# fawnliu/TRIS

Measured on AMD Instinct MI355X. Metric: Stage-1 training images/sec @320px bs48 (TRIS clip-RN50, 3 negatives), higher is better.
Workload: dtype f32 storage/accumulate; products h2 = 2 x f16 pieces; 1 GPU; Stage-1 train step, RefCOCOg-shaped synthetic batch: 48 img/GPU 320x320, 20-token query + 3 negative queries per image, clip-RN50 trunk + frozen aux CLIP ViT-B/32, AdamW (BASELINE.json configs[2]/[3]); per_gpu_batch=48, global_batch=48, size=320, query_len=20, negative_samples=3, parallelism=dp1, sync_bn=False

## Files before the change

include/tris_hip.h:

```cpp
#ifndef TRIS_HIP_H
#define TRIS_HIP_H

#ifdef __cplusplus
extern "C" {
#endif

int tris_gemm_f32(const float* A, const float* B, float* C, int M, int N, int K, long lda, long ldb, long ldc,
                  int transA, int transB, int batch, long strideA, long strideB, long strideC, const float* bias,
                  int bias_mode, const float* resid, long ldr, long strideR, int act, float alpha, float* workspace,
                  long workspace_bytes, void* stream);

int tris_gemm_epilogue_next(float* pre_out, const float* dact_x);

int tris_splitk_tickets_next(int* tickets, int count);
long tris_splitk_fused_launches(void);

int tris_set_gemm_mode(int mode);
int tris_set_gemm_mode_thread(int mode);
int tris_set_option(const char* name, const char* value);
int tris_set_conv_direct_thread(int value);

int tris_set_autotune(int on);
int tris_get_autotune(void);
int tris_get_gemm_mode(void);
long tris_direct_launches(int kind);

int tris_conv3x3_fwd_f32(const float* X, const float* Wt, float* Y, int B, int H, int W, int Cin, int Cout, int stride,
                         void* stream);
int tris_conv3x3_dgrad_f32(const float* dY, const float* Wt, float* dX, int B, int H, int W, int Cin, int Cout,
                           void* stream);
int tris_conv3x3_wgrad_f32(const float* X, const float* dY, float* dW, int B, int H, int W, int Cin, int Cout,
                           int stride, float* workspace, long workspace_bytes, void* stream);

int tris_conv3x3_bnin_ok(int B, int H, int W, int Cin, int Cout);
int tris_conv3x3_fwd_bnin_f32(const float* X, const float* mean, const float* invstd, const float* gamma, const float* beta,
                              const float* Wt, float* Y, int B, int H, int W, int Cin, int Cout, double* stat_part,
                              int* stat_rows, void* stream);
int tris_conv3x3_wgrad_bnin_f32(const float* X, const float* mean, const float* invstd, const float* gamma, const float* beta,
                                const float* dY, float* dW, int B, int H, int W, int Cin, int Cout, float* workspace,
                                long workspace_bytes, void* stream);

int tris_gemm_bnstat_f32(const float* A, const float* B, float* C, int M, int N, int K, double* stat_part,
                         int* stat_rows, void* stream);
int tris_conv3x3_fwd_bnstat_f32(const float* X, const float* Wt, float* Y, int B, int H, int W, int Cin, int Cout,
                                int stride, double* stat_part, int* stat_rows, void* stream);
int tris_bn_finalize_f32(const double* part, int rows, long M, int C, float eps, float momentum, float* stats,
                         float* running_mean, float* running_var, void* stream);

long tris_col_workspace_bytes(long M, int C);
int tris_bn_stats_f32(const float* X, long M, int C, float eps, float momentum, float* stats, float* running_mean,
                      float* running_var, float* workspace, void* stream);
int tris_bn_sync_combine_f32(const float* gathered, int world, int C, long count_per_rank, float eps, float momentum,
                             float* stats, float* running_mean, float* running_var, void* stream);
int tris_bn_apply_f32(const float* X, const float* mean, const float* invstd, const float* gamma, const float* beta,
                      const float* resid, float* Y, long M, int C, int relu, void* stream);
int tris_gemm_bnbwd_f32(const float* dY, const float* Wt, float* dZ, int M, int N, int K, const float* resid, long ldr,
                        const float* bn_x, const float* bn_y, const float* mean, const float* invstd, const float* gamma,
                        const float* beta, double* part, int* part_rows, void* stream);
int tris_conv3x3_dgrad_bnbwd_f32(const float* dY, const float* Wt, float* dZ, int B, int H, int W, int Cin, int Cout,
                                 const float* bn_x, const float* mean, const float* invstd, const float* gamma,
                                 const float* beta, double* part, int* part_rows, void* stream);
int tris_part_finalize_f32(const double* part, int rows, int C, float* out0, float* out1, void* stream);

int tris_amax_bits_f32(const float* x, long n, unsigned* out, void* stream);
int tris_amax_segments_f32(const float* base, const long* offs, const long* sizes, int nseg, unsigned* slots, void* stream);
int tris_amax_next(unsigned* out);
int tris_h2_next(const unsigned* amaxA, const unsigned* amaxB, float scaleA, float scaleB);
int tris_bn_mask_next(unsigned char* mask);
int tris_h2_planes_f32(const float* x, float* planes_out, long n, const unsigned* word, void* stream);
int tris_h2_planes_segments_f32(const float* base, const long* offs, const long* sizes, const long* slot_index, int nseg,
                                const unsigned* slots, float* out_base, void* stream);
int tris_h2_planes_t_segments_f32(const float* base, const long* offs, const long* rows, const long* cols, const long* slot_index,
                                  int nseg, const unsigned* slots, float* out_base, void* stream);
int tris_h2_unplanes_f32(const float* planes, float* out, long n, const unsigned* word, void* stream);
int tris_h2_next_planes(const unsigned* amaxA, const unsigned* amaxB, int flags);
int tris_bn_apply_pl_f32(const float* X, const float* mean, const float* invstd, const float* gamma, const float* beta,
                         const float* resid, int resid_kind, const unsigned* resid_word, float* Ypl, const unsigned* out_word, long M,
                         int C, int relu, void* stream);
int tris_bn_bwd_reduce_pl_f32(const float* dY, const float* Ypl, const float* X, const float* mean, const float* invstd, long M, int C,
                              float* sum_dz, float* sum_dzx, float* workspace, float* dz_out, void* stream);
int tris_bn_apply_pool_pl_f32(const float* X, const float* mean, const float* invstd, const float* gamma, const float* beta,
                              float* Ypl, const unsigned* out_word, int B, int H, int W, int C, void* stream);
int tris_avgpool2_fwd_pl_f32(const float* Xpl, float* Ypl, const unsigned* word, int B, int H, int W, int C, void* stream);
int tris_bn_bwd_apply_pl_f32(const float* dY, const float* Ypl, const float* X, const float* mean, const float* invstd,
                             const float* gamma, const float* sum_dz, const float* sum_dzx, float inv_count, float* dXpl,
                             const unsigned* out_word, float* dZ, long M, int C, const float* beta_mask, void* stream);
int tris_bn_bwd_apply_pool_pl_f32(const float* dYp, const float* X, const float* mean, const float* invstd, const float* gamma,
                                  const float* beta, const float* sum_dz, const float* sum_dzx, float inv_count, float* dXpl,
                                  const unsigned* out_word, int B, int H, int W, int C, void* stream);
int tris_bn_out_bound2_f32(const float* gamma, const float* beta, int C, float xhat_max, const unsigned* add_word, unsigned* out,
                           void* stream);
int tris_bn_finalize_bound_f32(const double* part, int rows, long M, int C, float eps, float momentum, float* stats,
                               float* running_mean, float* running_var, const float* gamma, const float* beta, float xhat_max,
                               const unsigned* add_word, unsigned* bound_out, void* stream);
int tris_part_finalize_bound_f32(const double* part, int rows, int C, float* out0, float* out1, const float* gamma, const float* invstd,
                                 float inv_count, float xhat_max, const unsigned* dz_word, unsigned* bound_out, void* stream);
int tris_bn_bwd_bound_f32(const float* gamma, const float* invstd, const float* sum_dz, const float* sum_dzx, int C, float inv_count,
                          float xhat_max, const unsigned* dz_word, unsigned* out, void* stream);
int tris_bn_out_bound_f32(const float* gamma, const float* beta, int C, float xhat_max, unsigned* out, void* stream);
int tris_bn_bwd_reduce_f32(const float* dY, const float* Y, const float* X, const float* mean, const float* invstd,
                           long M, int C, float* sum_dz, float* sum_dzx, float* workspace, const float* gamma_mask,
                           const float* beta_mask, float* dz_out, void* stream);
int tris_bn_bwd_apply_f32(const float* dY, const float* Y, const float* X, const float* mean, const float* invstd,
                          const float* gamma, const float* sum_dz, const float* sum_dzx, float inv_count, float* dX,
                          float* dZ, long M, int C, const float* beta_mask, void* stream);
int tris_colsum_f32(const float* X, long M, int N, long ld, float* out, float* workspace, void* stream);

int tris_instnorm_fwd_f32(const float* X, const float* gamma, const float* beta, float* Y, float* mean, float* invstd,
                          int B, int P, int C, float eps, int relu, void* stream);
int tris_instnorm_bwd_f32(const float* dY, const float* Y, const float* X, const float* gamma, const float* mean,
                          const float* invstd, float* dX, float* dgamma_part , float* dbeta_part ,
                          int B, int P, int C, int relu, void* stream);

int tris_layernorm_fwd_f32(const float* X, const float* gamma, const float* beta, float* Y, float* mean, float* rstd,
                           long rows, int W, float eps, void* stream);
long tris_layernorm_bwd_workspace_bytes(long rows, int W);
int tris_layernorm_bwd_f32(const float* dY, const float* X, const float* gamma, const float* mean, const float* rstd,
                           float* dX, float* dgamma, float* dbeta, long rows, int W, float* workspace, const float* extra , void* stream);

int tris_bn_apply_pool_f32(const float* X, const float* mean, const float* invstd, const float* gamma, const float* beta,
                           float* Yp, int B, int H, int W, int C, void* stream);
int tris_bn_bwd_reduce_pool_f32(const float* dYp, const float* X, const float* mean, const float* invstd, int B, int H, int W,
                                int C, float* sum_dz, float* sum_dzx, float* workspace, const float* gamma, const float* beta,
                                void* stream);
int tris_bn_bwd_apply_pool_f32(const float* dYp, const float* X, const float* mean, const float* invstd, const float* gamma,
                               const float* beta, const float* sum_dz, const float* sum_dzx, float inv_count, float* dX, int B,
                               int H, int W, int C, void* stream);
int tris_avgpool2_fwd_f32(const float* X, float* Y, int B, int H, int W, int C, void* stream);
int tris_avgpool2_bwd_f32(const float* dY, float* dX, int B, int H, int W, int C, void* stream);
#define TRIS_EW_ADD 0
#define TRIS_EW_AXPY 1
#define TRIS_EW_RELU_BWD 2
#define TRIS_EW_QGELU 3
#define TRIS_EW_QGELU_BWD 4
#define TRIS_EW_MUL 5
#define TRIS_EW_SCALE 6
#define TRIS_EW_RELU 7
int tris_elementwise_f32(int op, const float* A, const float* B, float* O, long n, float s, void* stream);
int tris_elementwise_bcast_f32(int op, const float* A, const float* B, float* O, long n, long nb, float s, void* stream);
int tris_scale_exp_fwd_f32(const float* X, const float* ls, float* O, float* e_out, long n, void* stream);
long tris_scale_exp_workspace_bytes(void);
int tris_scale_exp_bwd_f32(const float* dO, const float* O, const float* ls, float* dX, float* dls, float* workspace, long n,
                           void* stream);
int tris_nchw_to_nhwc_f32(const float* X, float* Y, int B, int C, int H, int W, void* stream);

int tris_mha_fwd_f32(const float* qkv, float* out, int N, int L, int W, int heads, int causal, void* stream);
int tris_mha_bwd_f32(const float* qkv, const float* dout, float* dqkv, int N, int L, int W, int heads, int causal,
                     void* stream);
int tris_mha_mfma_fwd_f32(const float* qkv, float* out, float* lse, int N, int L, int W, int heads, int causal,
                          void* stream);
int tris_mha_mfma_bwd_f32(const float* qkv, const float* out, const float* dout, const float* lse, float* delta,
                          float* dqkv, int N, int L, int W, int heads, int causal, void* stream);
int tris_mha_h2_fwd_f32(const float* qkv, float* out, float* lse, const unsigned* amax_qkv, int N, int L, int W, int heads,
                        int causal, void* stream);
int tris_mha_h2_bwd_f32(const float* qkv, const float* out, const float* dout, const float* lse, float* delta, float* dqkv,
                        const unsigned* amax_qkv, const unsigned* amax_dout, int N, int L, int W, int heads, int causal,
                        void* stream);
int tris_text_pack_plan_i64(const long* ids, int N, int L, int* plan, void* stream);
int tris_embed_packed_fwd_f32(const long* ids, const float* tok, const float* pos, const int* plan, float* out, int N, int L, int W,
                              void* stream);
int tris_mha_packed_fwd_f32(const float* qkv, float* out, const int* plan, int N, int Lmax, int W, int heads, int causal, void* stream);
int tris_eot_gather_packed_f32(const float* x, const int* plan, float* out, int N, int W, void* stream);
int tris_rows_limit_thread(const int* limit);
int tris_embed_fwd_f32(const long* ids, const float* tok, const float* pos, float* out, int N, int L, int W,
                       void* stream);
int tris_embed_bwd_f32(const long* ids, const float* dout, float* dtok, float* dpos, int N, int L, int W, void* stream);
int tris_embed_rows_bwd_f32(const long* ids, const float* rows, float* dtok, int R, int W, float scale, void* stream);
int tris_concat_i64(const long* a, long na, const long* b, long nb, long* out, void* stream);
int tris_eot_gather_fwd_f32(const long* ids, const float* x, float* out, int N, int L, int W, void* stream);
int tris_eot_gather_bwd_f32(const long* ids, const float* dout, float* dx, int N, int L, int W, void* stream);

int tris_l2norm_fwd_f32(const float* X, float* Y, float* inv_norm, long rows, int C, void* stream);
int tris_l2norm_bwd_f32(const float* dY, const float* Y, const float* inv_norm, float* dX, long rows, int C,
                        void* stream);
int tris_softmax_fwd_f32(const float* X, float* Y, long rows, int n, float scale, void* stream);
int tris_softmax_bwd_f32(const float* dY, const float* Y, float* dX, long rows, int n, float scale, void* stream);
int tris_xattn_fwd_f32(const float* Qv, const float* Kv, const float* Vv, const float* Qt, const float* Kt,
                       const float* Vt, float* new_vis, float* new_lan, float* probs, int B, int P, int N, int C,
                       void* stream);
#define TRIS_DECLINED (-2)
long tris_xattn_fused_ws_bytes(int B, int N, int C);
long tris_xattn_fused_sync_words(int B);
int tris_xattn_fused_fwd_f32(const float* Qv, const float* Kv, const float* Vv, const float* Qt, const float* Kt,
                             const float* Vt, float* new_vis, float* new_lan, float* probs, int B, int P, int N, int C,
                             float* ws, long ws_bytes, unsigned* sync, void* stream);
long tris_xattn_px_ws_bytes(int B, int N, int C);
long tris_xattn_px_sync_words(int B);
long tris_xattn_px_bwd_ws_bytes(int B, int N, int C);
int tris_xattn_px_bwd_f32(const float* d_vis, const float* d_lan, const float* Vv, const float* Qt, const float* Kt,
                          const float* Vt, const float* probs, float* dQv, float* dKv, float* dVv, float* dS, int B, int P,
                          int N, int C, float* ws, long ws_bytes, unsigned* sync, unsigned* amax_dQv, unsigned* amax_dKv,
                          unsigned* amax_dVv, void* stream);
long tris_xattn_px_last_form(void);
int tris_xattn_amax_next(const unsigned* qv, const unsigned* kv, const unsigned* vv, const unsigned* qt, const unsigned* kt,
                         const unsigned* vt);
long tris_xattn_px_slots(int B, int P, int C, int cus);
int tris_xattn_px_fwd_f32(const float* Qv, const float* Kv, const float* Vv, const float* Qt, const float* Kt,
                          const float* Vt, float* new_vis, float* new_lan, float* probs, int B, int P, int N, int C,
                          float* ws, long ws_bytes, unsigned* sync, void* stream);
int tris_softmax_col_bwd_f32(const float* dY, const float* Y, float* dX, int B, int P, int N, float scale,
                             void* stream);
int tris_cls_head_fwd_f32(const float* score, float* cls_out, float* cls_fg, int B, int P, int N, float focal_p,
                          float focal_c, void* stream);
int tris_cls_head_bwd_f32(const float* score, const float* g_cls_out, float* dscore, int B, int P, int N, float focal_p,
                          float focal_c, void* stream);
int tris_maps_fwd_f32(const float* score, float* relu_map, float* sig_map, int B, int h, int w, int N, int S,
                      void* stream);
int tris_maps_bwd_f32(const float* score, const float* d_relu, const float* d_sig, float* dscore, int B, int h, int w,
                      int N, int S, void* stream);
int tris_resize_bilinear_fwd_f32(const float* X, float* Y, int planes, int Hi, int Wi, int Ho, int Wo,
                                 int align_corners, void* stream);
int tris_resize_bilinear_bwd_f32(const float* dY, float* dX, int planes, int Hi, int Wi, int Ho, int Wo,
                                 int align_corners, void* stream);
int tris_fg_patch_fwd_f32(const float* cam, const float* img, float* patches, int B, int C, int R, int ps,
                          void* stream);
int tris_fg_patch_bwd_f32(const float* dpatches, const float* img, float* dcam, int B, int C, int R, int ps,
                          void* stream);
int tris_vit_assemble_fwd_f32(const float* emb, const float* cls, const float* pos, float* x, int B, int T, int W,
                              void* stream);
int tris_vit_assemble_bwd_f32(const float* dx, float* demb, int B, int T, int W, void* stream);
int tris_stage1_loss_fwd_f32(const float* cls, const float* fi, const float* ft, const float* fneg, int B, int N, int E,
                             int K, float w1, float w4, float w5, float* per_img, float* rowloss, float* losses,
                             void* stream);
int tris_stage1_loss_bwd_f32(const float* cls, const float* fi, const float* ft, const float* fneg, const float* g,
                             float w1, float w4, float w5, int B, int N, int E, int K, float* dcls, float* dfi, void* stream);

int tris_adamw_f32(float* p, const float* g, float* m, float* v, long n, float lr, float beta1, float beta2, float eps,
                   float weight_decay, int step_count, void* stream);
int tris_adamw_dev_f32(float* p, const float* g, float* m, float* v, long n, const float* hyper, float beta1, float beta2,
                       float eps, float weight_decay, void* stream);

int tris_eval_post_f32(const float* relu_map, int S, const unsigned char* target, int oH, int oW, float* cam,
                       long* out_iu, float* workspace , void* stream);

int tris_resample_u8(const unsigned char* in, int Hin, int Win, int C, const int* bounds_h, const int* kk_h, int ksize_h,
                     const int* bounds_v, const int* kk_v, int ksize_v, int Hout, int Wout, unsigned char* tmp,
                     unsigned char* out, void* stream);
int tris_gather2d_u8(const unsigned char* in, int Hin, int Win, int C, const int* yidx, const int* xidx, int Hout,
                     int Wout, unsigned char* out, void* stream);
int tris_mask_sum_nearest_u8(const unsigned char* masks, int K, int Hin, int Win, const int* yidx, const int* xidx,
                             int Hout, int Wout, unsigned char* out, void* stream);
int tris_u8_gather_normalize_f32(const unsigned char* cache, const long* index, int B, long HW, const float* lut,
                                 float* out, int planar, void* stream);
int tris_gather_rows(const void* table, const long* index, long rows, long row_bytes, void* out, void* stream);

#define TRIS_MBOX_MAX_WORLD 16
long tris_mbox_bytes(int cap_floats);
int tris_mbox_alloc(void** ptr, int cap_floats);
int tris_mbox_free(void* ptr);
int tris_mbox_ipc_handle(void* ptr, void* handle64);
int tris_mbox_ipc_open(const void* handle64, void** ptr);
int tris_mbox_ipc_close(void* ptr);
int tris_mbox_exchange_f32(const float* src0, int n0, const float* src1, int n1, float* out, void* const* boxes, int world,
                           int rank, unsigned* seq, int cap_floats, int mode, long spin_limit, int* err, void* stream);
int tris_mbox_bn_combine_f32(const float* local_stats, int C, long count_per_rank, float eps, float momentum, float* stats,
                             float* running_mean, float* running_var, void* const* boxes, int world, int rank, unsigned* seq,
                             int cap_floats, long spin_limit, int* err, void* stream);
int tris_mbox_bn_combine_bound_f32(const float* local_stats, int C, long count_per_rank, float eps, float momentum, float* stats,
                                   float* running_mean, float* running_var, void* const* boxes, int world, int rank, unsigned* seq,
                                   int cap_floats, long spin_limit, int* err, const float* gamma, const float* beta, float xhat_max,
                                   const unsigned* resid_word, unsigned* bound_word, void* stream);
int tris_mbox_bn_bwd_exchange_f32(const float* sum_dz, const float* sum_dzx, int C, float* out, void* const* boxes, int world, int rank,
                                  unsigned* seq, int cap_floats, long spin_limit, int* err, const float* gamma, const float* invstd,
                                  float inv_count, float xhat_max, const unsigned* dz_word, unsigned* bound_word, void* stream);

long tris_seg_workspace_bytes(long M, int C);
int tris_bn_prelu_fwd_f32(const float* X, const float* mean, const float* invstd, const float* gamma, const float* beta,
                          const float* slope, float* Y, long M, int C, void* stream);
int tris_bn_prelu_bwd_reduce_f32(const float* dY, const float* X, const float* mean, const float* invstd, const float* gamma,
                                 const float* beta, const float* slope, long M, int C, float* sum_dz, float* sum_dzx, float* dslope,
                                 double* workspace, void* stream);
int tris_bn_prelu_bwd_apply_f32(const float* dY, const float* X, const float* mean, const float* invstd, const float* gamma,
                                const float* beta, const float* slope, const float* sum_dz, const float* sum_dzx, float inv_count,
                                float* dX, long M, int C, void* stream);
int tris_upsample_nhwc_fwd_f32(const float* X, const float* skip, float* up, float* sum, int B, int Hi, int Wi, int Ho, int Wo,
                               int C, void* stream);
int tris_upsample_nhwc_bwd_f32(const float* d_up, const float* d_sum, float* dX, int B, int Hi, int Wi, int Ho, int Wo, int C,
                               void* stream);
int tris_head1_fwd_f32(const float* X, const float* w, float* Y, long M, int C, void* stream);
int tris_head1_bwd_f32(const float* g, const float* X, const float* w, float* dX, float* dw, long M, int C, double* workspace,
                       void* stream);
long tris_bce4_workspace_bytes(long n);
int tris_bce4_fwd_f32(const float* x1, const float* x2, const float* x3, const float* x4, const void* target, int target_f32, long n,
                      float* losses, double* workspace, void* stream);
int tris_bce4_bwd_f32(const float* x1, const float* x2, const float* x3, const float* x4, const void* target, int target_f32,
                      const float* g, float* d1, float* d2, float* d3, float* d4, long n, void* stream);
int tris_eval_post_signed_f32(const float* map, int S, const unsigned char* target, int oH, int oW, float* cam, long* out_iu,
                              float* workspace, void* stream);

int tris_irn_centroids_f32(const float* dp, int h, int w, int iterations, int* centroids, void* stream);
int tris_irn_weak_mask_f32(const float* dp, int h, int w, float thres, unsigned char* mask, void* stream);
long tris_cc_workspace_bytes(int B, int H, int W);
int tris_cc_label_u8(const unsigned char* img, int B, int H, int W, int* labels, int* counts, int* workspace, void* stream);
int tris_irn_cluster_i32(const int* centroids, const int* dp_label, int n_label, int h, int w, int* inst_map, int* n_inst,
                         int* workspace, void* stream);
int tris_irn_instance_cam_f32(const float* cam, const int* inst_map, int K, int n, float* out, void* stream);
int tris_irn_affinity_f32(const float* edge, int h, int w, const int* dirs, const int* path_off, const int* path_cells, int n_dirs,
                          float beta, float* Wt, float* colsum, void* stream);
int tris_irn_walk_f32(const float* x, const float* edge, const float* Wt, const float* colsum, const int* dirs, int n_dirs, int K,
                      int h, int w, int steps, float* out, float* tmp, void* stream);
int tris_irn_finish_f32(const float* rw, int K, int h, int w, int H, int W, float bg_thres, float* rw_up, int* labels,
                        float* workspace, void* stream);
int tris_irn_label_masks_u8(const int* labels, int K, long n, int base, unsigned char* masks, void* stream);
int tris_irn_fragments_f32(const int* frag_labels, const float* rw_up, const int* offsets, int K, long n, long min_area, int F,
                           float* score, int* area, unsigned char* frag_masks, int* workspace, void* stream);

int tris_irn_stem_f32(const unsigned char* img, const float* lut, const float* Wk, const float* mean, const float* invstd,
// ... 58 lines not shown
```

tris_amd/CLIP/clip/model.py:

```python
from collections import OrderedDict


import numpy as np
import torch
from torch import nn

from ... import ops
from ...config import cfg


class Conv2d(nn.Module):

    def __init__(self, cin, cout, k, stride=1, bias=False):
        super().__init__()
        self.cin, self.cout, self.k, self.stride = cin, cout, k, stride
        w = torch.empty(cout, cin, k, k).contiguous(memory_format=torch.channels_last)
        nn.init.kaiming_uniform_(w, a=5 ** 0.5)
        self.weight = nn.Parameter(w)
        self.bias = nn.Parameter(torch.zeros(cout)) if bias else None

    def forward(self, x, stats=False, grad_box=None, grad_box_out=None):
        if self.k == 1:
            return ops.linear(x, self.weight, self.bias, stats=stats and self.bias is None, grad_box=grad_box,
                              grad_box_out=grad_box_out)
# ... 34 lines not shown
        super().__init__()
        assert k == 2
        self.k = k

    def forward(self, x, grad_box_out=None):
        return ops.avgpool2(x, grad_box_out)


class Bottleneck(nn.Module):
    expansion = 4

    def __init__(self, inplanes, planes, stride=1):
        super().__init__()
        self.conv1 = Conv2d(inplanes, planes, 1)
        self.bn1 = BatchNorm2d(planes)
        self.conv2 = Conv2d(planes, planes, 3)
        self.bn2 = BatchNorm2d(planes)
        self.avgpool = AvgPool2d(stride) if stride > 1 else nn.Identity()
        self.conv3 = Conv2d(planes, planes * self.expansion, 1)
        self.bn3 = BatchNorm2d(planes * self.expansion)
        self.downsample = None
        self.stride = stride
        if stride > 1 or inplanes != planes * Bottleneck.expansion:
            self.downsample = nn.Sequential(OrderedDict([
                ("-1", AvgPool2d(stride) if stride > 1 else nn.Identity()),
                ("0", Conv2d(inplanes, planes * self.expansion, 1)),
                ("1", BatchNorm2d(planes * self.expansion)),
            ]))

    def forward(self, x, link_out=False):
        tr = self.training
        link_out = link_out and cfg.grad_box
        box = ops.GradBox() if (tr and torch.is_grad_enabled() and x.requires_grad
                               and cfg.grad_box) else None
        out = self.conv1(x, stats=tr, grad_box=box)
        pl = tr and ops.planes_on()
        out = self.bn1(out, relu=True, lazy=tr and not pl and ops.conv3x3_bnin_ok(out.shape, self.conv2.cout), bwd_link=True,
                       planes=pl, dx_planes=pl)
        if self.stride > 1:
            out = self.bn2(self.conv2(out, stats=tr), relu=True, pool=True, planes=pl, dx_planes=pl)
        else:
            out = self.bn2(self.conv2(out, stats=tr), relu=True, bwd_link=True, planes=pl, dx_planes=pl)
        out = self.conv3(out, stats=tr)
        if self.downsample is not None:
            if isinstance(self.downsample[0], AvgPool2d):
                idn = self.downsample[1](self.downsample[0](x, grad_box_out=box), stats=tr)
            else:
                idn = self.downsample[1](self.downsample[0](x), stats=tr, grad_box_out=box)
            idn = self.downsample[2](idn, dx_planes=pl)
            return self.bn3(out, resid=idn, relu=True, bwd_link=link_out, planes=pl, dx_planes=pl)
        return self.bn3(out, resid=x, relu=True, grad_box=box, bwd_link=link_out, planes=pl, dx_planes=pl)


class Linear(nn.Module):
    def __init__(self, cin, cout):
        super().__init__()
        self.in_features, self.out_features = cin, cout
        self.weight = nn.Parameter(torch.empty(cout, cin))
        self.bias = nn.Parameter(torch.zeros(cout))
        nn.init.kaiming_uniform_(self.weight, a=5 ** 0.5)

    def forward(self, x, resid=None, act=0, grad_box_res=None):
        return ops.linear(x, self.weight, self.bias, resid, act, grad_box_res=grad_box_res)


class AttentionPool2d(nn.Module):

    def __init__(self, spacial_dim, embed_dim, num_heads, output_dim=None):
        super().__init__()
        self.positional_embedding = nn.Parameter(torch.randn(spacial_dim ** 2 + 1, embed_dim) / embed_dim ** 0.5)
        self.k_proj = Linear(embed_dim, embed_dim)
        self.q_proj = Linear(embed_dim, embed_dim)
        self.v_proj = Linear(embed_dim, embed_dim)
        self.c_proj = Linear(embed_dim, output_dim or embed_dim)
        self.num_heads, self.embed_dim, self.spacial_dim = num_heads, embed_dim, spacial_dim
        for p in self.parameters():
            p._tris_no_grad_path = True

    def forward(self, x):
        raise NotImplementedError("AttentionPool2d output is unused by TRIS Stage-1 and is not part of the MI355X path")


class ModifiedResNet(nn.Module):
    def __init__(self, layers, output_dim, heads, input_resolution=224, width=64):
        super().__init__()
        self.output_dim, self.input_resolution = output_dim, input_resolution
        self.conv1 = Conv2d(3, width // 2, 3, stride=2)
        self.bn1 = BatchNorm2d(width // 2)
        self.conv2 = Conv2d(width // 2, width // 2, 3)
        self.bn2 = BatchNorm2d(width // 2)
        self.conv3 = Conv2d(width // 2, width, 3)
        self.bn3 = BatchNorm2d(width)
        self.avgpool = AvgPool2d(2)
        self._inplanes = width
        self.layer1 = self._make_layer(width, layers[0])
        self.layer2 = self._make_layer(width * 2, layers[1], stride=2)
        self.layer3 = self._make_layer(width * 4, layers[2], stride=2)
        self.layer4 = self._make_layer(width * 8, layers[3], stride=2)
        self.attnpool = AttentionPool2d(input_resolution // 32, width * 32, heads, output_dim)

    def _make_layer(self, planes, blocks, stride=1):
        layers = [Bottleneck(self._inplanes, planes, stride)]
        self._inplanes = planes * Bottleneck.expansion
        for _ in range(1, blocks):
            layers.append(Bottleneck(self._inplanes, planes))
        return nn.Sequential(*layers)

    def forward_cl(self, x, hooks=None, taps=True):
        tr = self.training
        if tr:
            ops.h2_auto_step()
        x = ops.nchw_to_nhwc(x.float())
        pl = tr and ops.planes_on()
        x = self.conv1(x, stats=tr)
        x = self.bn1(x, relu=True, lazy=tr and not pl and ops.conv3x3_bnin_ok(x.shape, self.conv2.cout), bwd_link=True,
                     planes=pl)
        x = self.conv2(ops.cut(x), stats=tr)
        x = self.bn2(x, relu=True, lazy=tr and not pl and ops.conv3x3_bnin_ok(x.shape, self.conv3.cout), bwd_link=True,
                     planes=pl, dx_planes=pl)
        x = ops.cut(x)
        x = self.bn3(self.conv3(x, stats=tr), relu=True, pool=True, planes=pl, dx_planes=pl)
        x = ops.cut(x)
        if hooks and "stem" in hooks:
            hooks["stem"]()
        outs = []
        red = getattr(self, "grad_reducer", None)
        if red is not None:
            x = red.boundary(x, "layer1")
        for name, layer in (("layer2", self.layer1), ("layer3", self.layer2), ("layer4", self.layer3),
                            ("heads", self.layer4)):
            for k, blk in enumerate(layer):
                x = ops.cut(blk(x, link_out=(not taps) or k + 1 < len(layer)))
            if red is not None:
                x = red.boundary(x, name)
            outs.append(x)
            stage = {"layer2": "layer1", "layer3": "layer2", "layer4": "layer3", "heads": "layer4"}.get(name)
            if hooks and stage in hooks:
                hooks[stage]()
        return tuple(outs)

    def forward(self, x):
        outs = [ops.unplanes(o).permute(0, 3, 1, 2) for o in self.forward_cl(x)]
        outs.append(None)
        return tuple(outs)


class LayerNorm(nn.Module):
    def __init__(self, w, eps=1e-5):
        super().__init__()
        self.eps = eps
        self.weight = nn.Parameter(torch.ones(w))
        self.bias = nn.Parameter(torch.zeros(w))

    def forward(self, x, grad_box=None):
        return ops.layer_norm(x, self.weight, self.bias, self.eps, grad_box)


class QuickGELU(nn.Module):
    def forward(self, x):
        return ops.quick_gelu(x)


class MultiheadAttention(nn.Module):

    def __init__(self, d_model, n_head):
        super().__init__()
        self.embed_dim, self.num_heads = d_model, n_head
        self.in_proj_weight = nn.Parameter(torch.empty(3 * d_model, d_model))
        self.in_proj_bias = nn.Parameter(torch.zeros(3 * d_model))
        self.out_proj = Linear(d_model, d_model)
        nn.init.xavier_uniform_(self.in_proj_weight)


class ResidualAttentionBlock(nn.Module):
    def __init__(self, d_model, n_head, attn_mask=None):
        super().__init__()
        self.attn = MultiheadAttention(d_model, n_head)
        self.ln_1 = LayerNorm(d_model)
        self.mlp = nn.Sequential(OrderedDict([
            ("c_fc", Linear(d_model, d_model * 4)),
            ("gelu", QuickGELU()),
            ("c_proj", Linear(d_model * 4, d_model)),
        ]))
        self.ln_2 = LayerNorm(d_model)
        self.causal = attn_mask is not None

    def forward(self, x):
        use_box = torch.is_grad_enabled() and x.requires_grad and cfg.grad_box
        b1 = ops.GradBox() if use_box else None
        b2 = ops.GradBox() if use_box else None
        h = self.ln_1(x, b1)
        qkv = ops.linear(h, self.attn.in_proj_weight, self.attn.in_proj_bias)
        a = ops.mha(qkv, self.attn.num_heads, self.causal)
        x = self.attn.out_proj(a, resid=x, grad_box_res=b1)
        h = self.ln_2(x, b2)
        if torch.is_grad_enabled() and cfg.mlp_fuse:
            f = ops.linear_qgelu(h, self.mlp.c_fc.weight, self.mlp.c_fc.bias)
            return ops.linear(f, self.mlp.c_proj.weight, self.mlp.c_proj.bias, x, 0, grad_box_res=b2, act_link=True)
        if torch.is_grad_enabled():
            return self.mlp.c_proj(self.mlp.gelu(self.mlp.c_fc(h)), resid=x, grad_box_res=b2)
        f = self.mlp.c_fc(h, act=2)
        return self.mlp.c_proj(f, resid=x, grad_box_res=b2)


    def forward_packed(self, x, plan, N, L):
        h = self.ln_1(x)
        qkv = ops.linear(h, self.attn.in_proj_weight, self.attn.in_proj_bias)
        a = ops.mha_packed(qkv, plan, N, L, self.attn.num_heads, self.causal)
        x = self.attn.out_proj(a, resid=x)
        h = self.ln_2(x)
        return self.mlp.c_proj(self.mlp.c_fc(h, act=2), resid=x)

    def forward_token0(self, x):
        h = self.ln_1(x)
        qkv = ops.linear(h, self.attn.in_proj_weight, self.attn.in_proj_bias)
        a = ops.token0(ops.mha(qkv, self.attn.num_heads, self.causal))
        x0 = self.attn.out_proj(a, resid=ops.token0(x))
        h = self.ln_2(x0)
        if torch.is_grad_enabled() and cfg.mlp_fuse:
            f = ops.linear_qgelu(h, self.mlp.c_fc.weight, self.mlp.c_fc.bias)
            return ops.linear(f, self.mlp.c_proj.weight, self.mlp.c_proj.bias, x0, 0, act_link=True)
        if torch.is_grad_enabled():
            return self.mlp.c_proj(self.mlp.gelu(self.mlp.c_fc(h)), resid=x0)
        return self.mlp.c_proj(self.mlp.c_fc(h, act=2), resid=x0)


class Transformer(nn.Module):
    def __init__(self, width, layers, heads, attn_mask=None):
        super().__init__()
        self.width, self.layers = width, layers
        self.resblocks = nn.Sequential(*[ResidualAttentionBlock(width, heads, attn_mask) for _ in range(layers)])

    def forward(self, x):
        for blk in self.resblocks:
            x = ops.cut(blk(x))
        return x

    def forward_token0(self, x):
        blocks = list(self.resblocks)
        for blk in blocks[:-1]:
            x = ops.cut(blk(x))
        return blocks[-1].forward_token0(x)


class VisionTransformer(nn.Module):
    def __init__(self, input_resolution, patch_size, width, layers, heads, output_dim):
        super().__init__()
        self.input_resolution, self.output_dim, self.patch_size = input_resolution, output_dim, patch_size
        self.conv1 = nn.Module()
        self.conv1.weight = nn.Parameter(torch.randn(width, 3, patch_size, patch_size) * 0.02)
        scale = width ** -0.5
        self.class_embedding = nn.Parameter(scale * torch.randn(width))
        self.positional_embedding = nn.Parameter(scale * torch.randn((input_resolution // patch_size) ** 2 + 1, width))
        self.ln_pre = LayerNorm(width)
        self.transformer = Transformer(width, layers, heads)
        for blk in self.transformer.resblocks:
            for w in (blk.attn.in_proj_weight, blk.attn.out_proj.weight, blk.mlp.c_fc.weight, blk.mlp.c_proj.weight):
                w._tris_linear_w = True
        self.ln_post = LayerNorm(width)
        self.proj = nn.Parameter(scale * torch.randn(width, output_dim))
        self.spacial_dim = 7
        self.class_embedding._tris_accumulates = True
        self.positional_embedding._tris_accumulates = True

    def forward_patches(self, patches):
        emb = ops.linear(patches, self.conv1.weight)
        x = ops.vit_assemble(emb, self.class_embedding, self.positional_embedding)
        x = self.ln_pre(x)
        if cfg.vit_token0:
            cls = self.ln_post(self.transformer.forward_token0(x))
        else:
            cls = self.ln_post(ops.token0(self.transformer(x)))
        return ops.matmul(cls, self.proj)

    def forward_spatial(self, x):
        B, C, H, Wd = x.shape
        ps = self.patch_size
        ones = torch.ones(B, 1, H, Wd, device=x.device, dtype=torch.float32)
        emb = ops.linear(ops.fg_patches(ones, x.float(), ps), self.conv1.weight)
        gh, gw = H // ps, Wd // ps
        sd = self.input_resolution // ps
        width = self.positional_embedding.shape[1]
        pos = self.positional_embedding
        if (gh, gw) != (sd, sd):
            grid = pos[1:].reshape(1, sd, sd, width).permute(0, 3, 1, 2)
            grid = ops.resize_bilinear(grid, (gh, gw), False)
            pos = torch.cat([pos[0:1], grid.reshape(width, gh * gw).permute(1, 0)], dim=0)
        x = ops.vit_assemble(emb, self.class_embedding, pos.contiguous())
        x = self.ln_pre(x)
        x = self.transformer(x)
        return x[:, 0, :], x[:, 1:, :].reshape(B, gh, gw, width)

    def forward(self, x):
        B, C, R, _ = x.shape
        ones = torch.ones(B, 1, R, R, device=x.device, dtype=torch.float32)
        return self.forward_patches(ops.fg_patches(ones, x.float(), self.patch_size))


class CLIP(nn.Module):
    def __init__(self, embed_dim, image_resolution, vision_layers, vision_width, vision_patch_size, context_length,
                 txt_length, vocab_size, transformer_width, transformer_heads, transformer_layers):
        super().__init__()
        self.context_length = context_length
        if isinstance(vision_layers, (tuple, list)):
            self.visual = ModifiedResNet(layers=vision_layers, output_dim=embed_dim, heads=vision_width * 32 // 64,
                                         input_resolution=image_resolution, width=vision_width)
        else:
            self.visual = VisionTransformer(input_resolution=image_resolution, patch_size=vision_patch_size,
                                            width=vision_width, layers=vision_layers, heads=vision_width // 64,
                                            output_dim=embed_dim)
        self.txt_length = txt_length
        self.transformer = Transformer(width=transformer_width, layers=transformer_layers, heads=transformer_heads,
                                       attn_mask=True)
        self.vocab_size = vocab_size
        self.token_embedding = nn.Embedding(vocab_size, transformer_width)
        self.positional_embedding = nn.Parameter(torch.empty(self.context_length, transformer_width))
        self.ln_final = LayerNorm(transformer_width)
        self.text_projection = nn.Parameter(torch.empty(transformer_width, embed_dim))
        self.logit_scale = nn.Parameter(torch.ones([]) * np.log(1 / 0.07))
        self.logit_scale._tris_no_grad_path = True
        self.initialize_parameters()

    def initialize_parameters(self):
        nn.init.normal_(self.token_embedding.weight, std=0.02)
        nn.init.normal_(self.positional_embedding, std=0.01)
        if isinstance(self.visual, ModifiedResNet):
            std = self.visual.attnpool.c_proj.in_features ** -0.5
            for m in (self.visual.attnpool.q_proj, self.visual.attnpool.k_proj, self.visual.attnpool.v_proj,
                      self.visual.attnpool.c_proj):
                nn.init.normal_(m.weight, std=std)
            for layer in (self.visual.layer1, self.visual.layer2, self.visual.layer3, self.visual.layer4):
                for name, param in layer.named_parameters():
                    if name.endswith("bn3.weight"):
                        nn.init.zeros_(param)
        proj_std = (self.transformer.width ** -0.5) * ((2 * self.transformer.layers) ** -0.5)
        attn_std = self.transformer.width ** -0.5
        fc_std = (2 * self.transformer.width) ** -0.5
        for block in self.transformer.resblocks:
            nn.init.normal_(block.attn.in_proj_weight, std=attn_std)
            nn.init.normal_(block.attn.out_proj.weight, std=proj_std)
            nn.init.normal_(block.mlp.c_fc.weight, std=fc_std)
            nn.init.normal_(block.mlp.c_proj.weight, std=proj_std)
        nn.init.normal_(self.text_projection, std=self.transformer.width ** -0.5)

    @property
    def dtype(self):
        return self.visual.conv1.weight.dtype

    def encode_image(self, image):
        return self.visual(image)

    def encode_text(self, text):
        ids = text.long()
        if ids.shape[1] > self.txt_length:
            raise ValueError(f"token length {ids.shape[1]} exceeds txt_length {self.txt_length}")
        red = getattr(self, "grad_reducer", None)
        x = ops.embed(ids, self.token_embedding.weight, self.positional_embedding, reducer=red)
        if red is not None:
            x = red.boundary(x, "text")
            from ...parallel import TEXT_BOUNDARIES
            for i, blk in enumerate(self.transformer.resblocks):
                x = blk(x)
                if i in TEXT_BOUNDARIES:
                    x = red.boundary(x, TEXT_BOUNDARIES[i])
        else:
            x = self.transformer(x)
        x = self.ln_final(x)
        hidden = ops.matmul(ops.eot_gather(ids, x), self.text_projection)
        return x, hidden

    def encode_text_hidden(self, text):
        ids = text.long()
        if (not cfg.text_pack or torch.is_grad_enabled() or not ops.text_packable(ids.shape[1]) or ids.shape[1] > self.txt_length
                or not ids.is_cuda):
            return self.encode_text(text)[1]
        ids = ids.contiguous()
        N, L = ids.shape
        plan = ops.text_pack_plan(ids)
        x = ops.embed_packed(ids, self.token_embedding.weight, self.positional_embedding, plan)
        with ops.rows_limit(plan):
            for blk in self.transformer.resblocks:
                x = blk.forward_packed(x, plan, N, L)
            x = self.ln_final(x)
        return ops.matmul(ops.eot_gather_packed(x, plan, N), self.text_projection)

    def forward(self, image, text):
        raise NotImplementedError("CLIP.forward (zero-shot logits) is not on the Stage-1 path")


def convert_weights(model):
    return model


def build_model(state_dict, txt_length=40):
    vit = "visual.proj" in state_dict
    if vit:
        vision_width = state_dict["visual.conv1.weight"].shape[0]
        vision_layers = len([k for k in state_dict if k.startswith("visual.") and k.endswith(".attn.in_proj_weight")])
        vision_patch_size = state_dict["visual.conv1.weight"].shape[-1]
        grid = round((state_dict["visual.positional_embedding"].shape[0] - 1) ** 0.5)
        image_resolution = vision_patch_size * grid
    else:
        counts = [len(set(k.split(".")[2] for k in state_dict if k.startswith(f"visual.layer{b}"))) for b in (1, 2, 3, 4)]
        vision_layers = tuple(counts)
        vision_width = state_dict["visual.layer1.0.conv1.weight"].shape[0]
        out_w = round((state_dict["visual.attnpool.positional_embedding"].shape[0] - 1) ** 0.5)
        vision_patch_size = None
        assert out_w ** 2 + 1 == state_dict["visual.attnpool.positional_embedding"].shape[0]
        image_resolution = out_w * 32
    embed_dim = state_dict["text_projection"].shape[1]
    context_length = state_dict["positional_embedding"].shape[0]
# ... 26 lines not shown
```

tris_amd/config.py:

```python
import contextlib
import os


def _flag(name, default):
    v = os.environ.get(name)
    return default if v is None or v == "" else v != "0"


class _Config:
    def __setattr__(self, name, value):
        if name == "step_graph" and "step_graph" in self.__dict__:
            self.__dict__["step_graph_chosen"] = True
        self.__dict__[name] = value

    def __init__(self):
        e = os.environ.get
        self.step_graph = e("TRIS_STEP_GRAPH", "0")
        self.step_graph_chosen = "TRIS_STEP_GRAPH" in os.environ
        self.hipgraph = _flag("TRIS_HIPGRAPH", True)
        self.text_stream = _flag("TRIS_TEXT_STREAM", True)
        self.wgrad_stream = _flag("TRIS_WGRAD_STREAM", True)
        self.stream_probe = _flag("TRIS_STREAM_PROBE", True)
        self.stream_probe_log = e("TRIS_STREAM_PROBE_LOG") == "1"
        self.text_at = e("TRIS_TEXT_AT", "layer4")
        self.bn_bwd_fuse = _flag("TRIS_BN_BWD_FUSE", True)
        self.bn_pool = _flag("TRIS_BN_POOL", True)
        self.grad_box = _flag("TRIS_GRAD_BOX", True)
        self.mlp_fuse = _flag("TRIS_MLP_FUSE", True)
        self.mha = e("TRIS_MHA", "auto")
        self.mha_h2 = _flag("TRIS_MHA_H2", True)
        self.ddp_seg_opt = _flag("TRIS_DDP_SEG_OPT", True)
        self.ddp_seg_poison = _flag("TRIS_DDP_SEG_POISON", False)
        self.syncbn_bound = _flag("TRIS_SYNCBN_BOUND", True)
        self.xattn_fused = _flag("TRIS_XATTN_FUSED", True)
        self.xattn_px = _flag("TRIS_XATTN_PX", True)
        self.xattn_h2 = _flag("TRIS_XATTN_H2", True)
        self.xattn_bwd_px = _flag("TRIS_XATTN_BWD_PX", True)
        self.hbm_loader = _flag("TRIS_HBM_LOADER", True)
        self.eval_group = max(1, int(e("TRIS_EVAL_GROUP", "16")))
        self.mbox_spin = int(e("TRIS_MBOX_SPIN", "40000000"))
        self.syncbn_comm = e("TRIS_SYNCBN_COMM", "mailbox")
        self.ddp_check = e("TRIS_DDP_CHECK") == "1"
        self.ddp_sparse_embed = _flag("TRIS_DDP_SPARSE_EMBED", True)
        self.random_init = e("TRIS_RANDOM_INIT") == "1"
        self.h2_planes = _flag("TRIS_H2_PLANES", True)
        self.own_stream = _flag("TRIS_OWN_STREAM", True)
        self.fuse_splitk = _flag("TRIS_FUSE_SPLITK_PY", False)
        self.aux_text_early = _flag("TRIS_AUX_TEXT_EARLY", True)
        self.text_pack = _flag("TRIS_TEXT_PACK", True)
        self.bn_bitmask = _flag("TRIS_BN_BITMASK", True)
        self.gemm_convert = int(e("TRIS_GEMM_CONVERT", "0"))
        self.step_graph_rerecord = int(e("TRIS_STEP_GRAPH_RERECORD", "3"))
        self.side_param_grads = _flag("TRIS_SIDE_PARAM_GRADS", True)
        self.vit_token0 = _flag("TRIS_VIT_TOKEN0", True)

    @contextlib.contextmanager
    def override(self, **kw):
        old = {k: getattr(self, k) for k in kw}
        try:
            for k, v in kw.items():
                setattr(self, k, v)
            yield self
        finally:
            for k, v in old.items():
                setattr(self, k, v)

    def key(self):
        return tuple(sorted((k, v) for k, v in self.__dict__.items() if k not in ("step_graph_chosen", "step_graph_rerecord")))


cfg = _Config()
```

tris_amd/csrc/attn_h2.hip:

```cpp
#include "common.h"
#include "tris_hip.h"
#include "x3_split.h"

namespace {

#include "amax.h"

constexpr int HD = 64;
constexpr int RS = 144;
constexpr int PLB = 64 * RS;
constexpr float PS = 8192.f;

typedef float f4v __attribute__((ext_vector_type(4)));
typedef short s16x4 __attribute__((ext_vector_type(4)));
typedef short s16x8 __attribute__((ext_vector_type(8)));
typedef unsigned u32x4v __attribute__((ext_vector_type(4)));

struct H8 { f16x8 hi, lo; };

__device__ __forceinline__ float4 ldg4(const float* p) { return *reinterpret_cast<const float4*>(p); }
__device__ __forceinline__ H8 split8(const float4 u, const float4 w, const float s) {
  const Split4 p = split4h(u, s), q = split4h(w, s);
  H8 o;
  o.hi = __builtin_bit_cast(f16x8, (u32x4v){p.hi.x, p.hi.y, q.hi.x, q.hi.y});
  o.lo = __builtin_bit_cast(f16x8, (u32x4v){p.mid.x, p.mid.y, q.mid.x, q.mid.y});
  return o;
}
__device__ __forceinline__ void mm3(const H8& a, const H8& b, f4v& c, f4v& cx) {
  cx = __builtin_amdgcn_mfma_f32_16x16x32_f16(a.lo, b.hi, cx, 0, 0, 0);
  cx = __builtin_amdgcn_mfma_f32_16x16x32_f16(a.hi, b.lo, cx, 0, 0, 0);
  c = __builtin_amdgcn_mfma_f32_16x16x32_f16(a.hi, b.hi, c, 0, 0, 0);
}
__device__ __forceinline__ f4v join(const f4v c, const f4v cx) { return c + cx * (1.0f / 2048.0f); }

__device__ __forceinline__ void stage64(char* planes, const float* base, long row_stride, int row0, int L, int tid, float s) {
#pragma unroll
  for (int q = 0; q < 4; ++q) {
    const int idx = q * 256 + tid, row = idx >> 4, c4 = (idx & 15) * 4;
    const Split4 sp = split4h(ldg4(base + (long)min(row0 + row, L - 1) * row_stride + c4), s);
    *reinterpret_cast<uint2*>(planes + row * RS + c4 * 2) = sp.hi;
    *reinterpret_cast<uint2*>(planes + PLB + row * RS + c4 * 2) = sp.mid;
  }
}
__device__ __forceinline__ H8 afrag(const char* planes, int row, int ks, int kg) {
  H8 o;
  o.hi = *reinterpret_cast<const f16x8*>(planes + row * RS + (32 * ks + 8 * kg) * 2);
  o.lo = *reinterpret_cast<const f16x8*>(planes + PLB + row * RS + (32 * ks + 8 * kg) * 2);
  return o;
}
__device__ __forceinline__ f16x8 trf1(const char* plane, int rb, int ct, int r16, int kg) {
  typedef __attribute__((address_space(3))) s16x4 lds_s16x4;
  const char* a = plane + (rb + kg * 8 + (r16 >> 2)) * RS + ct * 32 + 8 * (r16 & 3);
  const s16x4 lo = __builtin_amdgcn_ds_read_tr16_b64_v4i16((lds_s16x4*)a);
  const s16x4 hi = __builtin_amdgcn_ds_read_tr16_b64_v4i16((lds_s16x4*)(a + 4 * RS));
  const s16x8 v = {lo[0], lo[1], lo[2], lo[3], hi[0], hi[1], hi[2], hi[3]};
  return __builtin_bit_cast(f16x8, v);
}
__device__ __forceinline__ H8 bfrag(const char* planes, int rb, int ct, int r16, int kg) {
  H8 o;
  o.hi = trf1(planes, rb, ct, r16, kg);
  o.lo = trf1(planes + PLB, rb, ct, r16, kg);
  return o;
}
__device__ __forceinline__ void resident(H8 (&f)[2], const float* row_kg, float s) {
#pragma unroll
  for (int ks = 0; ks < 2; ++ks) f[ks] = split8(ldg4(row_kg + 32 * ks), ldg4(row_kg + 32 * ks + 4), s);
}
__device__ __forceinline__ int trow(int r, int j) { return 8 * (r >> 2) + 4 * j + (r & 3); }
__device__ __forceinline__ float wave_scale_of(float m) {
  unsigned u = __builtin_bit_cast(unsigned, m);
#pragma unroll
  for (int sft = 32; sft > 0; sft >>= 1) u = max(u, (unsigned)__shfl_xor((int)u, sft, 64));
  return h2_scale_from_bits(u);
}

__global__ __launch_bounds__(256) void mha_h2_fwd_kernel(const float* __restrict__ qkv, float* __restrict__ out, float* __restrict__ lse,
                                                         int L, int W, int causal, float scale, const unsigned* __restrict__ am_qkv,
                                                         unsigned* __restrict__ amax) {
  __shared__ __attribute__((aligned(16))) char Kp[2 * PLB];
  __shared__ __attribute__((aligned(16))) char Vp[2 * PLB];
  const int tid = threadIdx.x, lane = tid & 63, wave = tid >> 6, r = lane & 15, kg = lane >> 4;
  const int h = blockIdx.y, n = blockIdx.z, H = gridDim.y;
  const int qb = blockIdx.x * 64, q0 = qb + wave * 16;
  const float s = h2_scale_from_bits(h2_amax_of(am_qkv, lane));
  const float inv_s = scale / (s * s), inv_o = 1.0f / (PS * s);
  const float* base = qkv + (long)n * L * 3 * W + h * HD;
  const int qrow = min(q0 + r, L - 1);
  H8 qf[2];
  resident(qf, base + (long)qrow * 3 * W + 8 * kg, s);
  float m = -INFINITY, l = 0.f;
  f4v oc[4], ox[4];
#pragma unroll
  for (int j = 0; j < 4; ++j) oc[j] = ox[j] = (f4v){0.f, 0.f, 0.f, 0.f};
  const int kend = causal ? min(L, qb + 64) : L;
  for (int kb = 0; kb < kend; kb += 64) {
    __syncthreads();
    stage64(Kp, base + W, 3L * W, kb, L, tid, s);
    stage64(Vp, base + 2 * W, 3L * W, kb, L, tid, s);
    __syncthreads();
    if (q0 < L) {
#pragma unroll
      for (int pr = 0; pr < 2; ++pr) {
        const int key0 = kb + 32 * pr;
        if (key0 < kend && !(causal && key0 > q0 + 15)) {
          f4v sc[2], sx[2];
#pragma unroll
          for (int j = 0; j < 2; ++j) {
            sc[j] = sx[j] = (f4v){0.f, 0.f, 0.f, 0.f};
            const int row = 32 * pr + trow(r, j);
#pragma unroll
            for (int ks = 0; ks < 2; ++ks) mm3(afrag(Kp, row, ks, kg), qf[ks], sc[j], sx[j]);
          }
          float sv[8], mx = -INFINITY;
          const bool full = key0 + 32 <= L && !(causal && key0 + 31 > q0);
#pragma unroll
          for (int i = 0; i < 8; ++i) {
            const int key = key0 + 8 * kg + i;
            const float v = (sc[i >> 2][i & 3] + sx[i >> 2][i & 3] * (1.0f / 2048.0f)) * inv_s;
            sv[i] = (full || (key < L && !(causal && key > q0 + r))) ? v : -INFINITY;
            mx = fmaxf(mx, sv[i]);
          }
          mx = fmaxf(mx, __shfl_xor(mx, 16, 64));
          mx = fmaxf(mx, __shfl_xor(mx, 32, 64));
          const float mn = fmaxf(m, mx);
          float p[8], rs = 0.f;
#pragma unroll
          for (int i = 0; i < 8; ++i) { p[i] = mn == -INFINITY ? 0.f : __expf(sv[i] - mn); rs += p[i]; }
          rs += __shfl_xor(rs, 16, 64);
          rs += __shfl_xor(rs, 32, 64);
          const float alpha = mn == -INFINITY ? 1.f : __expf(m - mn);
          l = l * alpha + rs;
          m = mn;
          if (__builtin_amdgcn_ballot_w64(alpha != 1.f) != 0ull) {
#pragma unroll
            for (int t = 0; t < 4; ++t) {
              const float ar = __shfl(alpha, 4 * kg + t, 64);
#pragma unroll
              for (int j = 0; j < 4; ++j) { oc[j][t] *= ar; ox[j][t] *= ar; }
            }
          }
          const H8 pf = split8(make_float4(p[0], p[1], p[2], p[3]), make_float4(p[4], p[5], p[6], p[7]), PS);
#pragma unroll
          for (int ct = 0; ct < 4; ++ct) mm3(pf, bfrag(Vp, 32 * pr, ct, r, kg), oc[ct], ox[ct]);
        }
      }
    }
  }
  unsigned am = 0u;
  if (q0 < L) {
    const float linv = 1.f / l;
    float* ob = out + (long)n * L * W + h * HD;
#pragma unroll
    for (int t = 0; t < 4; ++t) {
      const float li = __shfl(linv, 4 * kg + t, 64) * inv_o;
      const int q = q0 + 4 * kg + t;
      if (q < L) {
#pragma unroll
        for (int j = 0; j < 4; ++j) {
          const float o = (oc[j][t] + ox[j][t] * (1.0f / 2048.0f)) * li;
          ob[(long)q * W + 16 * j + r] = o;
          am = max(am, __builtin_bit_cast(unsigned, o) & 0x7fffffffu);
        }
      }
    }
    if (kg == 0 && q0 + r < L) lse[((long)n * H + h) * L + q0 + r] = m + __logf(l);
  }
  if (amax != nullptr) amax_commit(am, amax);
}

__global__ __launch_bounds__(256) void mha_h2_dq_kernel(const float* __restrict__ qkv, const float* __restrict__ out,
                                                        const float* __restrict__ dout, const float* __restrict__ lse,
                                                        float* __restrict__ delta, float* __restrict__ dqkv, int L, int W, int causal,
                                                        float scale, const unsigned* __restrict__ am_qkv,
                                                        const unsigned* __restrict__ am_do, unsigned* __restrict__ amax) {
  __shared__ __attribute__((aligned(16))) char Kp[2 * PLB];
  __shared__ __attribute__((aligned(16))) char Vp[2 * PLB];
  const int tid = threadIdx.x, lane = tid & 63, wave = tid >> 6, r = lane & 15, kg = lane >> 4;
  const int h = blockIdx.y, n = blockIdx.z, H = gridDim.y;
  const int qb = blockIdx.x * 64, q0 = qb + wave * 16;
  const float s = h2_scale_from_bits(h2_amax_of(am_qkv, lane)), sg = h2_scale_from_bits(h2_amax_of(am_do, lane));
  const float inv_s = scale / (s * s), inv_p = 1.0f / (s * sg);
  const float* base = qkv + (long)n * L * 3 * W + h * HD;
  const int qrow = min(q0 + r, L - 1);
  H8 qf[2], gf[2];
  resident(qf, base + (long)qrow * 3 * W + 8 * kg, s);
  float dl = 0.f;
  {
    const float* gp = dout + ((long)n * L + qrow) * W + h * HD + 8 * kg;
    const float* op = out + ((long)n * L + qrow) * W + h * HD + 8 * kg;
#pragma unroll
    for (int ks = 0; ks < 2; ++ks) {
      const float4 g0 = ldg4(gp + 32 * ks), g1 = ldg4(gp + 32 * ks + 4), o0 = ldg4(op + 32 * ks), o1 = ldg4(op + 32 * ks + 4);
      gf[ks] = split8(g0, g1, sg);
      dl += g0.x * o0.x + g0.y * o0.y + g0.z * o0.z + g0.w * o0.w + g1.x * o1.x + g1.y * o1.y + g1.z * o1.z + g1.w * o1.w;
    }
    dl += __shfl_xor(dl, 16, 64);
    dl += __shfl_xor(dl, 32, 64);
    if (kg == 0 && q0 + r < L) delta[((long)n * H + h) * L + q0 + r] = dl;
  }
  const float ls = lse[((long)n * H + h) * L + qrow];
  f4v acc[4];
#pragma unroll
  for (int j = 0; j < 4; ++j) acc[j] = (f4v){0.f, 0.f, 0.f, 0.f};
  const int kend = causal ? min(L, qb + 64) : L;
  for (int kb = 0; kb < kend; kb += 64) {
    __syncthreads();
    stage64(Kp, base + W, 3L * W, kb, L, tid, s);
    stage64(Vp, base + 2 * W, 3L * W, kb, L, tid, s);
    __syncthreads();
    if (q0 < L) {
#pragma unroll
      for (int pr = 0; pr < 2; ++pr) {
        const int key0 = kb + 32 * pr;
        if (key0 < kend && !(causal && key0 > q0 + 15)) {
          f4v sc[2], sx[2], pc[2], px[2];
#pragma unroll
          for (int j = 0; j < 2; ++j) {
            sc[j] = sx[j] = pc[j] = px[j] = (f4v){0.f, 0.f, 0.f, 0.f};
            const int row = 32 * pr + trow(r, j);
#pragma unroll
            for (int ks = 0; ks < 2; ++ks) {
              mm3(afrag(Kp, row, ks, kg), qf[ks], sc[j], sx[j]);
              mm3(afrag(Vp, row, ks, kg), gf[ks], pc[j], px[j]);
            }
          }
          float ds[8], mx = 0.f;
          const bool full = key0 + 32 <= L && !(causal && key0 + 31 > q0);
#pragma unroll
          for (int i = 0; i < 8; ++i) {
            const int key = key0 + 8 * kg + i;
            const bool ok = full || (key < L && !(causal && key > q0 + r));
            const float sv = (sc[i >> 2][i & 3] + sx[i >> 2][i & 3] * (1.0f / 2048.0f)) * inv_s;
            const float dp = (pc[i >> 2][i & 3] + px[i >> 2][i & 3] * (1.0f / 2048.0f)) * inv_p;
            ds[i] = ok ? __expf(sv - ls) * (dp - dl) * scale : 0.f;
            mx = fmaxf(mx, fabsf(ds[i]));
          }
          const float sd = wave_scale_of(mx);
          const H8 df = split8(make_float4(ds[0], ds[1], ds[2], ds[3]), make_float4(ds[4], ds[5], ds[6], ds[7]), sd);
          const float inv_d = 1.0f / (sd * s);
#pragma unroll
          for (int ct = 0; ct < 4; ++ct) {
            f4v tc = {0.f, 0.f, 0.f, 0.f}, tx = {0.f, 0.f, 0.f, 0.f};
            mm3(df, bfrag(Kp, 32 * pr, ct, r, kg), tc, tx);
            acc[ct] += join(tc, tx) * inv_d;
          }
        }
      }
    }
  }
  unsigned am = 0u;
  if (q0 < L) {
    float* ob = dqkv + (long)n * L * 3 * W + h * HD;
#pragma unroll
    for (int t = 0; t < 4; ++t) {
      const int q = q0 + 4 * kg + t;
      if (q < L) {
#pragma unroll
        for (int j = 0; j < 4; ++j) {
          ob[(long)q * 3 * W + 16 * j + r] = acc[j][t];
          am = max(am, __builtin_bit_cast(unsigned, acc[j][t]) & 0x7fffffffu);
        }
      }
    }
  }
  if (amax != nullptr) amax_commit(am, amax);
}

__global__ __launch_bounds__(256) void mha_h2_dkv_kernel(const float* __restrict__ qkv, const float* __restrict__ dout,
                                                         const float* __restrict__ lse, const float* __restrict__ delta,
                                                         float* __restrict__ dqkv, int L, int W, int causal, float scale,
                                                         const unsigned* __restrict__ am_qkv, const unsigned* __restrict__ am_do,
                                                         unsigned* __restrict__ amax) {
  __shared__ __attribute__((aligned(16))) char Qp[2 * PLB];
  __shared__ __attribute__((aligned(16))) char Gp[2 * PLB];
  __shared__ float Ls[64], Ds[64];
  const int tid = threadIdx.x, lane = tid & 63, wave = tid >> 6, r = lane & 15, kg = lane >> 4;
  const int h = blockIdx.y, n = blockIdx.z, H = gridDim.y;
  const int kb0 = blockIdx.x * 64, k0 = kb0 + wave * 16;
  const float s = h2_scale_from_bits(h2_amax_of(am_qkv, lane)), sg = h2_scale_from_bits(h2_amax_of(am_do, lane));
  const float inv_s = scale / (s * s), inv_p = 1.0f / (s * sg), inv_v = 1.0f / (PS * sg);
  const float* base = qkv + (long)n * L * 3 * W + h * HD;
  const int krow = min(k0 + r, L - 1);
  H8 kf[2], vf[2];
  resident(kf, base + W + (long)krow * 3 * W + 8 * kg, s);
  resident(vf, base + 2 * W + (long)krow * 3 * W + 8 * kg, s);
  f4v dk[4], vc[4], vx[4];
#pragma unroll
  for (int j = 0; j < 4; ++j) dk[j] = vc[j] = vx[j] = (f4v){0.f, 0.f, 0.f, 0.f};
  const int qstart = causal ? kb0 : 0;
  for (int qb = qstart; qb < L; qb += 64) {
    __syncthreads();
    stage64(Qp, base, 3L * W, qb, L, tid, s);
    stage64(Gp, dout + (long)n * L * W + h * HD, (long)W, qb, L, tid, sg);
    if (tid < 64) {
      const int q = min(qb + tid, L - 1);
      Ls[tid] = lse[((long)n * H + h) * L + q];
      Ds[tid] = delta[((long)n * H + h) * L + q];
    }
    __syncthreads();
    if (k0 < L) {
#pragma unroll
      for (int pr = 0; pr < 2; ++pr) {
        const int qs0 = qb + 32 * pr;
        if (qs0 < L && !(causal && qs0 + 31 < k0)) {
          f4v sc[2], sx[2], pc[2], px[2];
#pragma unroll
          for (int j = 0; j < 2; ++j) {
            sc[j] = sx[j] = pc[j] = px[j] = (f4v){0.f, 0.f, 0.f, 0.f};
            const int row = 32 * pr + trow(r, j);
#pragma unroll
            for (int ks = 0; ks < 2; ++ks) {
              mm3(afrag(Qp, row, ks, kg), kf[ks], sc[j], sx[j]);
              mm3(afrag(Gp, row, ks, kg), vf[ks], pc[j], px[j]);
            }
          }
          float p[8], ds[8], mx = 0.f;
          const bool full = qs0 + 32 <= L && !(causal && k0 + 15 > qs0);
#pragma unroll
          for (int i = 0; i < 8; ++i) {
            const int ql = 32 * pr + 8 * kg + i, q = qb + ql;
            const bool ok = full || (q < L && !(causal && k0 + r > q));
            const float sv = (sc[i >> 2][i & 3] + sx[i >> 2][i & 3] * (1.0f / 2048.0f)) * inv_s;
            const float dp = (pc[i >> 2][i & 3] + px[i >> 2][i & 3] * (1.0f / 2048.0f)) * inv_p;
            p[i] = ok ? __expf(sv - Ls[ql]) : 0.f;
            ds[i] = p[i] * (dp - Ds[ql]) * scale;
            mx = fmaxf(mx, fabsf(ds[i]));
          }
          const float sd = wave_scale_of(mx);
          const H8 pf = split8(make_float4(p[0], p[1], p[2], p[3]), make_float4(p[4], p[5], p[6], p[7]), PS);
          const H8 df = split8(make_float4(ds[0], ds[1], ds[2], ds[3]), make_float4(ds[4], ds[5], ds[6], ds[7]), sd);
          const float inv_d = 1.0f / (sd * s);
#pragma unroll
          for (int ct = 0; ct < 4; ++ct) {
            mm3(pf, bfrag(Gp, 32 * pr, ct, r, kg), vc[ct], vx[ct]);
            f4v tc = {0.f, 0.f, 0.f, 0.f}, tx = {0.f, 0.f, 0.f, 0.f};
            mm3(df, bfrag(Qp, 32 * pr, ct, r, kg), tc, tx);
            dk[ct] += join(tc, tx) * inv_d;
          }
        }
      }
    }
  }
  unsigned am = 0u;
  if (k0 < L) {
    float* ob = dqkv + (long)n * L * 3 * W + h * HD;
#pragma unroll
    for (int t = 0; t < 4; ++t) {
      const int k = k0 + 4 * kg + t;
      if (k < L) {
#pragma unroll
        for (int j = 0; j < 4; ++j) {
          const float dv = (vc[j][t] + vx[j][t] * (1.0f / 2048.0f)) * inv_v;
          ob[(long)k * 3 * W + W + 16 * j + r] = dk[j][t];
          ob[(long)k * 3 * W + 2 * W + 16 * j + r] = dv;
          am = max(am, max(__builtin_bit_cast(unsigned, dk[j][t]) & 0x7fffffffu, __builtin_bit_cast(unsigned, dv) & 0x7fffffffu));
        }
      }
    }
  }
  if (amax != nullptr) amax_commit(am, amax);
}

}

extern "C" __attribute__((visibility("hidden"))) unsigned* tris_internal_take_amax_next();

extern "C" int tris_mha_h2_fwd_f32(const float* qkv, float* out, float* lse, const unsigned* amax_qkv, int N, int L, int W, int heads,
                                   int causal, void* stream) {
  if (W != heads * HD || L < 1 || N < 1 || (((uintptr_t)qkv) & 15) || amax_qkv == nullptr) return (int)hipErrorInvalidValue;
  hipLaunchKernelGGL(mha_h2_fwd_kernel, dim3(cdiv(L, 64), heads, N), dim3(256), 0, (hipStream_t)stream, qkv, out, lse, L, W, causal,
                     1.0f / sqrtf((float)HD), amax_qkv, tris_internal_take_amax_next());
  TRIS_LAUNCH_CHECK();
  return 0;
}

extern "C" int tris_mha_h2_bwd_f32(const float* qkv, const float* out, const float* dout, const float* lse, float* delta, float* dqkv,
                                   const unsigned* amax_qkv, const unsigned* amax_dout, int N, int L, int W, int heads, int causal,
                                   void* stream) {
  if (W != heads * HD || L < 1 || N < 1 || amax_qkv == nullptr || amax_dout == nullptr || (((uintptr_t)qkv) & 15) ||
      (((uintptr_t)dout) & 15) || (((uintptr_t)out) & 15))
    return (int)hipErrorInvalidValue;
  const float scale = 1.0f / sqrtf((float)HD);
  const dim3 grid(cdiv(L, 64), heads, N);
  unsigned* amax = tris_internal_take_amax_next();
  hipLaunchKernelGGL(mha_h2_dq_kernel, grid, dim3(256), 0, (hipStream_t)stream, qkv, out, dout, lse, delta, dqkv, L, W, causal, scale,
                     amax_qkv, amax_dout, amax);
  TRIS_LAUNCH_CHECK();
  hipLaunchKernelGGL(mha_h2_dkv_kernel, grid, dim3(256), 0, (hipStream_t)stream, qkv, dout, lse, delta, dqkv, L, W, causal, scale,
                     amax_qkv, amax_dout, amax);
  TRIS_LAUNCH_CHECK();
  return 0;
}
```

tris_amd/csrc/gemm_core.h:

```cpp
#pragma once
#include <algorithm>
#include <cstdlib>
#include <cstring>

#include "common.h"
#include "tris_hip.h"

namespace {

#include "gemm_params.h"
#include "amax.h"

constexpr int BK = 16;
constexpr int PAD = 4;

template <int BM, int BN, int AK, int BKIND, int EPI>
__global__ __launch_bounds__(256) void gemm_kernel(GemmParams p) {
  constexpr int WM = BM / 2, WN = BN / 2;
  constexpr int FM = WM / 32, FN = WN / 32;
  constexpr int PA = BM / 64, PB = BN / 64;
  __shared__ float As[BK][BM + PAD];
  __shared__ float Bs[BK][BN + PAD];

  const int tid = threadIdx.x;
// ... 267 lines not shown
        __syncthreads();
      }
    }
  }

  const int li = lane & 31, kh = lane >> 5;
  unsigned g_am = 0u;
#pragma unroll
  for (int i = 0; i < FM; ++i)
#pragma unroll
    for (int j = 0; j < FN; ++j) {
      const int col = n0 + wn * WN + j * 32 + li;
#pragma unroll
      for (int r = 0; r < 16; ++r) {
        const int row = m0 + wm * WM + i * 32 + (r & 3) + 8 * (r >> 2) + 4 * kh;
        if (row < p.M && col < p.N) {
          float v = acc[i][j][r];
          if (EPI == EPI_SLAB) {
            p.C[((long)blockIdx.z * p.M + row) * p.N + col] = v;
          } else {
            v *= p.alpha;
            if (p.bias_mode == 1) v += p.bias[col];
            else if (p.bias_mode == 2) v += p.bias[row];
            if (p.act == 1) v = fmaxf(v, 0.f);
            else if (p.act == 2) v = v / (1.0f + expf(-1.702f * v));
            if (p.resid) v += p.resid[(long)zb * p.sR + (long)row * p.ldr + col];
            p.C[(long)zb * p.sC + (long)row * p.ldc + col] = v;
            g_am = max(g_am, __builtin_bit_cast(unsigned, v) & 0x7fffffffu);
          }
        }
      }
    }
  if (EPI != EPI_SLAB && p.amax_out != nullptr) amax_commit(g_am, p.amax_out);
}

template <int VEC>
__global__ __launch_bounds__(256) void splitk_reduce_kernel(const float* __restrict__ ws, int S, GemmParams p) {
  const long total = (long)p.M * p.N;
  const long stride = (long)gridDim.x * blockDim.x * VEC;
  unsigned am = 0u;
  for (long idx = ((long)blockIdx.x * blockDim.x + threadIdx.x) * VEC; idx < total; idx += stride) {
    if (p.m_limit != nullptr && idx / p.N >= (long)*p.m_limit) break;
    float v[VEC];
#pragma unroll
    for (int t = 0; t < VEC; ++t) v[t] = 0.f;
    if (VEC == 4) {
      int s = 0;
      for (; s + 3 < S; s += 4) {
        const float4 a = ld4(ws + (long)s * total + idx), b = ld4(ws + (long)(s + 1) * total + idx);
        const float4 c = ld4(ws + (long)(s + 2) * total + idx), d = ld4(ws + (long)(s + 3) * total + idx);
        v[0] = (((v[0] + a.x) + b.x) + c.x) + d.x;
        v[1] = (((v[1] + a.y) + b.y) + c.y) + d.y;
        v[2] = (((v[2] + a.z) + b.z) + c.z) + d.z;
        v[3] = (((v[3] + a.w) + b.w) + c.w) + d.w;
      }
      for (; s < S; ++s) {
        const float4 a = ld4(ws + (long)s * total + idx);
        v[0] += a.x; v[1] += a.y; v[2] += a.z; v[3] += a.w;
      }
    } else {
      for (int s = 0; s < S; ++s) v[0] += ws[(long)s * total + idx];
    }
    const int row = (int)(idx / p.N), col0 = (int)(idx - (long)row * p.N);
#pragma unroll
    for (int t = 0; t < VEC; ++t) {
      const int col = col0 + t;
      float x = v[t] * p.alpha;
      if (p.bias_mode == 1) x += p.bias[col];
      else if (p.bias_mode == 2) x += p.bias[row];
      if (p.act == 1) x = fmaxf(x, 0.f);
      else if (p.act == 2) x = x / (1.0f + expf(-1.702f * x));
      if (p.resid) x += p.resid[(long)row * p.ldr + col];
      v[t] = x;
    }
    if (VEC == 4 && (p.ldc & 3) == 0)
      *reinterpret_cast<float4*>(p.C + (long)row * p.ldc + col0) = make_float4(v[0], v[1], v[2], v[3]);
    else
#pragma unroll
      for (int t = 0; t < VEC; ++t) p.C[(long)row * p.ldc + col0 + t] = v[t];
#pragma unroll
    for (int t = 0; t < VEC; ++t) am = max(am, __builtin_bit_cast(unsigned, v[t]) & 0x7fffffffu);
  }
  if (p.amax_out != nullptr) amax_commit(am, p.amax_out);
}

extern "C" { extern __attribute__((visibility("hidden"))) int tris_internal_red_grid; }
extern "C" { extern __attribute__((visibility("hidden"))) int tris_internal_reduce_wide; }
extern "C" { extern __attribute__((visibility("hidden"))) int tris_internal_xcd_order; }
extern "C" { extern __attribute__((visibility("hidden"))) int tris_internal_fuse_splitk; }
extern "C" { extern __attribute__((visibility("hidden"))) long tris_internal_fused_count; }
template <int G>
__global__ __launch_bounds__(64 * G) void splitk_reduce_wide_kernel(const float* __restrict__ ws, int S, GemmParams p) {
  __shared__ float4 part[G][64];
  const int c = threadIdx.x & 63, g = threadIdx.x >> 6;
  const long total = (long)p.M * p.N;
  const long idx = ((long)blockIdx.x * 64 + c) * 4;
  const bool in = idx < total && !(p.m_limit != nullptr && idx / p.N >= (long)*p.m_limit);
  float4 a = make_float4(0.f, 0.f, 0.f, 0.f);
  if (in) {
    int s = g;
    for (; s + 3 * G < S; s += 4 * G) {
      const float4 x0 = ld4(ws + (long)s * total + idx), x1 = ld4(ws + (long)(s + G) * total + idx);
      const float4 x2 = ld4(ws + (long)(s + 2 * G) * total + idx), x3 = ld4(ws + (long)(s + 3 * G) * total + idx);
      a.x = (((a.x + x0.x) + x1.x) + x2.x) + x3.x; a.y = (((a.y + x0.y) + x1.y) + x2.y) + x3.y;
      a.z = (((a.z + x0.z) + x1.z) + x2.z) + x3.z; a.w = (((a.w + x0.w) + x1.w) + x2.w) + x3.w;
    }
    for (; s < S; s += G) {
      const float4 x0 = ld4(ws + (long)s * total + idx);
      a.x += x0.x; a.y += x0.y; a.z += x0.z; a.w += x0.w;
    }
  }
  part[g][c] = a;
  __syncthreads();
  if (g != 0) return;
  float v[4] = {part[0][c].x, part[0][c].y, part[0][c].z, part[0][c].w};
#pragma unroll
  for (int w = 1; w < G; ++w) { v[0] += part[w][c].x; v[1] += part[w][c].y; v[2] += part[w][c].z; v[3] += part[w][c].w; }
  unsigned am = 0u;
  if (in) {
    const int row = (int)(idx / p.N), col0 = (int)(idx - (long)row * p.N);
#pragma unroll
    for (int t = 0; t < 4; ++t) {
      const int col = col0 + t;
      float x = v[t] * p.alpha;
      if (p.bias_mode == 1) x += p.bias[col];
      else if (p.bias_mode == 2) x += p.bias[row];
      if (p.act == 1) x = fmaxf(x, 0.f);
      else if (p.act == 2) x = x / (1.0f + expf(-1.702f * x));
      if (p.resid) x += p.resid[(long)row * p.ldr + col];
      v[t] = x;
      am = max(am, __builtin_bit_cast(unsigned, x) & 0x7fffffffu);
    }
    if ((p.ldc & 3) == 0)
      *reinterpret_cast<float4*>(p.C + (long)row * p.ldc + col0) = make_float4(v[0], v[1], v[2], v[3]);
    else
#pragma unroll
      for (int t = 0; t < 4; ++t) p.C[(long)row * p.ldc + col0 + t] = v[t];
  }
  if (p.amax_out != nullptr) amax_commit(am, p.amax_out);
}

#include "gemm_fast.h"

static inline long red_blocks(long want) { return tris_internal_red_grid > 0 && want > tris_internal_red_grid ? tris_internal_red_grid : want; }

template <int AK, int BKIND>
int run_cfg(GemmParams p, int batch, float* ws, hipStream_t st, Cfg cfg, int mode) {
  int bm = cfg.bm, bn = cfg.bn, splitk = ws != nullptr ? cfg.splitk : 1;
  const bool fast = gemm_fast_ok(p);
  if (bn == 32 && !fast) bm = bn = 64;
  const bool xtra = p.pre_out != nullptr || p.dact_x != nullptr;
  if (mode == 4 && !fast) return (int)hipErrorInvalidValue;
  const bool pipe = cfg.pipe == 1 && (mode == 1 || mode == 3 || mode == 4) && fast && bn != 32 && !xtra;
  const bool glds = cfg.pipe >= 2 && mode == 4 && fast && !xtra && bn != 32 && AK == A_ROWK && BKIND == B_NK;
  const int gform = glds ? (cfg.pipe >= 4 ? cfg.pipe - 2 : cfg.pipe) : 0;
  if (bm == 256 && !pipe && !glds) bm = 128;
  int tiles_m = cdiv(p.M, bm), tiles_n = cdiv(p.N, bn);
  p.tiles_n = tiles_n;
  const int kalign = fast ? 32 : BK;
  p.splitk = splitk;
  p.kchunk = cdiv(cdiv(p.K, splitk), kalign) * kalign;
  if (splitk > 1) splitk = cdiv(p.K, p.kchunk), p.splitk = splitk;
  dim3 grid((unsigned)(tiles_m * tiles_n), 1, (unsigned)(batch * splitk));
  p.xcd_remap = (fast && BKIND == B_KN_IM2COL && batch == 1 && splitk >= 8 && splitk % 8 == 0 && tiles_m * tiles_n > 1) ? 1 : 0;
  if (glds && cfg.pipe >= 4) p.xcd_remap = 2;
  if (tris_internal_xcd_order >= 0 && fast && p.xcd_remap != 1 && !(tris_internal_xcd_order == 2 && mode == 4))
    p.xcd_remap = (tris_internal_xcd_order && tiles_m * tiles_n >= 16 && tiles_n > 1) ? 2 : 0;
  float* Cfinal = p.C;
  int* const tk = p.tickets;
  p.tickets = nullptr;
  const bool wide = (p.N & 3) == 0 && al16(ws) && al16(Cfinal) && splitk >= 8 && (long)p.M * p.N / 4 < 128 * 256 && tris_internal_reduce_wide;
  const bool vec_fin = (p.N % 4 == 0) && al16(Cfinal) && (p.ldc % 4 == 0) && (!p.resid || (al16(p.resid) && p.ldr % 4 == 0)) &&
                       (p.bias_mode != 1 || al16(p.bias));
  const bool fuse = splitk > 1 && splitk <= tris_internal_fuse_splitk && splitk <= TRIS_FUSE_SPLITK_MAX && tk != nullptr && fast &&
                    batch == 1 && tiles_m * tiles_n <= p.tickets_n && (!wide || vec_fin);
  p.fin_groups = 0;
  if (fuse) {
    __atomic_fetch_add(&tris_internal_fused_count, 1L, __ATOMIC_RELAXED);
    p.tickets = tk;
    p.Cfin = Cfinal;
    p.vecCfin = vec_fin;
    if (wide) p.fin_groups = tris_internal_reduce_wide >= 16 ? 16 : tris_internal_reduce_wide >= 8 ? 8 : 4;
  }
  if (splitk > 1)
    p.vecC = (p.N % 4 == 0) && al16(ws);
  else
    p.vecC = (p.N % 4 == 0) && al16(p.C) && (p.ldc % 4 == 0) && (p.sC % 4 == 0) &&
             (!p.resid || (al16(p.resid) && p.ldr % 4 == 0 && p.sR % 4 == 0)) && (p.bias_mode != 1 || al16(p.bias));
#define TRIS_NW(BM_, BN_, PREC_) ((BM_) == 128 && (BN_) == 128 && (PREC_) != 0 ? 8 : (BN_) == 32 ? 2 : 4)
#define TRIS_FAST(BM_, BN_, EPI_, PREC_)                                                                       \
  hipLaunchKernelGGL((gemm_fast_kernel<BM_, BN_, AK, BKIND, EPI_, PREC_, TRIS_NW(BM_, BN_, PREC_)>), grid,    \
                     dim3(64 * TRIS_NW(BM_, BN_, PREC_)), 0, st, p)
#define TRIS_FAST_EPI(BM_, BN_, EPI_)                                       \
  do {                                                                      \
    if (mode == 1) TRIS_FAST(BM_, BN_, EPI_, 1);                            \
    else if (mode == 3) TRIS_FAST(BM_, BN_, EPI_, 3);                       \
    else if (mode == 4) TRIS_FAST(BM_, BN_, EPI_, 4);                       \
    else TRIS_FAST(BM_, BN_, EPI_, 0);                                      \
  } while (0)
#define TRIS_GO(BM_, BN_, GENERIC_OK_)                                                             \
  do {                                                                                             \
    if (fast) {                                                                                    \
      if (splitk > 1) {                                                                            \
        p.C = ws;                                                                                  \
        TRIS_FAST_EPI(BM_, BN_, EPI_SLAB);                                                         \
      } else if (xtra) {                                                                           \
        if constexpr (AK == A_ROWK && (BKIND == B_NK || BKIND == B_KN)) TRIS_FAST_EPI(BM_, BN_, EPI_XTRA); \
        else return (int)hipErrorInvalidValue;                                                     \
      } else {                                                                                     \
        TRIS_FAST_EPI(BM_, BN_, EPI_STD);                                                          \
      }                                                                                            \
    } else if (GENERIC_OK_) {                                                                      \
      if (splitk > 1) {                                                                            \
        p.C = ws;                                                                                  \
        hipLaunchKernelGGL((gemm_kernel<(GENERIC_OK_ ? BM_ : 64), (GENERIC_OK_ ? BN_ : 64), AK, BKIND, EPI_SLAB>), grid, dim3(256), 0, st, p); \
      } else {                                                                                     \
        hipLaunchKernelGGL((gemm_kernel<(GENERIC_OK_ ? BM_ : 64), (GENERIC_OK_ ? BN_ : 64), AK, BKIND, EPI_STD>), grid, dim3(256), 0, st, p);  \
      }                                                                                            \
    }                                                                                              \
  } while (0)
#define TRIS_PIPE_ONE(BM_, BN_, NW_, NWM_, EPI_)                                                                                   \
  do {                                                                                                                             \
    if (mode == 3)                                                                                                                 \
      hipLaunchKernelGGL((gemm_fast_kernel<BM_, BN_, AK, BKIND, EPI_, 3, NW_, 16, 2, NWM_>), grid, dim3(NW_ * 64), 0, st, p);      \
    else if (mode == 4)                                                                                                            \
      hipLaunchKernelGGL((gemm_fast_kernel<BM_, BN_, AK, BKIND, EPI_, 4, NW_, 16, 2, NWM_>), grid, dim3(NW_ * 64), 0, st, p);      \
    else                                                                                                                           \
      hipLaunchKernelGGL((gemm_fast_kernel<BM_, BN_, AK, BKIND, EPI_, 1, NW_, 16, 2, NWM_>), grid, dim3(NW_ * 64), 0, st, p);      \
  } while (0)
#define TRIS_PIPE_GO(BM_, BN_, NW_, NWM_)                        \
  do {                                                           \
    if (splitk > 1) {                                            \
      p.C = ws;                                                  \
      TRIS_PIPE_ONE(BM_, BN_, NW_, NWM_, EPI_SLAB);              \
    } else {                                                     \
      TRIS_PIPE_ONE(BM_, BN_, NW_, NWM_, EPI_STD);               \
    }                                                            \
  } while (0)
#define TRIS_GLDS_GO(BM_, BN_, NW_, NWM_)                                                                                          \
  do {                                                                                                                           \
    if (splitk > 1) {                                                                                                            \
      p.C = ws;                                                                                                                  \
      hipLaunchKernelGGL((gemm_fast_kernel<BM_, BN_, AK, BKIND, EPI_SLAB, 4, NW_, 32, 4, NWM_>), grid, dim3(NW_ * 64), 0, st, p); \
    } else {                                                                                                                     \
      hipLaunchKernelGGL((gemm_fast_kernel<BM_, BN_, AK, BKIND, EPI_STD, 4, NW_, 32, 4, NWM_>), grid, dim3(NW_ * 64), 0, st, p);  \
    }                                                                                                                            \
  } while (0)
  bool launched = false;
  if constexpr (AK == A_ROWK && BKIND == B_NK) {
    if (glds) {
      launched = true;
      if (bm == 256 && bn == 128) TRIS_GLDS_GO(256, 128, 8, 4);
      else if (bm == 128 && bn == 128 && gform == 3) TRIS_GLDS_GO(128, 128, 4, 2);
      else if (bm == 128 && bn == 128) TRIS_GLDS_GO(128, 128, 8, 2);
      else if (bm == 128 && bn == 64) TRIS_GLDS_GO(128, 64, 4, 2);
      else TRIS_GLDS_GO(64, 64, 4, 2);
    }
  }
#undef TRIS_GLDS_GO
  if (launched) {
  } else
  if (pipe) {
    if (bm == 256 && bn == 128) TRIS_PIPE_GO(256, 128, 8, 4);
    else if (bm == 128 && bn == 128) TRIS_PIPE_GO(128, 128, 8, 2);
    else if (bm == 128 && bn == 64) TRIS_PIPE_GO(128, 64, 4, 2);
    else TRIS_PIPE_GO(64, 64, 4, 2);
  } else if (bm == 128 && bn == 128) TRIS_GO(128, 128, true);
  else if (bm == 128 && bn == 64) TRIS_GO(128, 64, true);
  else if (bm == 128 && bn == 32) TRIS_GO(128, 32, false);
  else TRIS_GO(64, 64, true);
#undef TRIS_GO
#undef TRIS_PIPE_GO
#undef TRIS_PIPE_ONE
#undef TRIS_FAST_EPI
#undef TRIS_FAST
#undef TRIS_NW
  TRIS_LAUNCH_CHECK();
  if (splitk > 1 && !fuse) {
    p.C = Cfinal;
    long total = (long)p.M * p.N;
    if ((p.N & 3) == 0 && al16(ws) && al16(p.C) && splitk >= 8 && total / 4 < 128 * 256 && tris_internal_reduce_wide)
    {
      if (tris_internal_reduce_wide >= 16)
        hipLaunchKernelGGL(splitk_reduce_wide_kernel<16>, dim3(cdiv(total / 4, 64)), dim3(1024), 0, st, ws, splitk, p);
      else if (tris_internal_reduce_wide >= 8)
        hipLaunchKernelGGL(splitk_reduce_wide_kernel<8>, dim3(cdiv(total / 4, 64)), dim3(512), 0, st, ws, splitk, p);
      else
        hipLaunchKernelGGL(splitk_reduce_wide_kernel<4>, dim3(cdiv(total / 4, 64)), dim3(256), 0, st, ws, splitk, p);
    }
    else if ((p.N & 3) == 0 && al16(ws) && al16(p.C))
      hipLaunchKernelGGL(splitk_reduce_kernel<4>, dim3(red_blocks(cdiv(total / 4, 256))), dim3(256), 0, st, ws, splitk, p);
    else
      hipLaunchKernelGGL(splitk_reduce_kernel<1>, dim3(red_blocks(cdiv(total, 256))), dim3(256), 0, st, ws, splitk, p);
    TRIS_LAUNCH_CHECK();
  }
  return 0;
}

}
```

tris_amd/csrc/norm.hip:

```cpp
#include <cstdlib>

#include "common.h"
#include "tris_hip.h"

extern "C" {
__attribute__((visibility("hidden"))) int tris_internal_stream_form = 256;
__attribute__((visibility("hidden"))) int tris_internal_col_blocks = 512;
}

namespace {

#include "amax.h"

__device__ __forceinline__ float4 ld4(const float* p) { return *reinterpret_cast<const float4*>(p); }
__device__ __forceinline__ void st4(float* p, float4 v) { *reinterpret_cast<float4*>(p) = v; }
typedef float f32x4_t __attribute__((ext_vector_type(4)));
__device__ __forceinline__ float4 ld4nt(const float* p) {
  const f32x4_t v = __builtin_nontemporal_load(reinterpret_cast<const f32x4_t*>(p));
  return make_float4(v.x, v.y, v.z, v.w);
}
__device__ __forceinline__ void st4nt(float* p, float4 v) {
  const f32x4_t w = {v.x, v.y, v.z, v.w};
  __builtin_nontemporal_store(w, reinterpret_cast<f32x4_t*>(p));
}
constexpr int BIG_U = 4;
constexpr long BIG_PIECE = 256L * BIG_U;
inline bool big_form(long n4, int C, int streams) { return tris_internal_stream_form && C >= 4 && 1024 % C == 0 && n4 * 16 * streams > ((long)tris_internal_stream_form << 20) && n4 >= 4 * BIG_PIECE; }
inline int big_grid(long n4) { return (int)((n4 + BIG_PIECE - 1) / BIG_PIECE); }

struct d4 { double x, y, z, w; };
__device__ __forceinline__ d4 d4zero() { d4 r; r.x = r.y = r.z = r.w = 0.0; return r; }
__device__ __forceinline__ void st4d(double* p, d4 v) { p[0] = v.x; p[1] = v.y; p[2] = v.z; p[3] = v.w; }

__device__ __forceinline__ long pooled_row(long r, int H, int W) {
  const int w = (int)(r % W);
  const long t = r / W;
  const int h = (int)(t % H);
  const long b = t / H;
  return (b * (H >> 1) + (h >> 1)) * (W >> 1) + (w >> 1);
}

template <int MODE, bool POOL = false>
__global__ __launch_bounds__(256) void col_partial_kernel(const float* __restrict__ X, const float* __restrict__ dY,
                                                          const float* __restrict__ Y, const float* __restrict__ mean,
                                                          const float* __restrict__ invstd, long M, int C, long ld,
                                                          long rows_per_block, double* __restrict__ part,
                                                          const float* __restrict__ gamma = nullptr,
                                                          const float* __restrict__ beta = nullptr,
                                                          float* __restrict__ dZ = nullptr, int pool_h = 0, int pool_w = 0,
                                                          int y_pl = 0, unsigned* __restrict__ amax = nullptr) {
  unsigned am = 0u;
  auto ldy = [&](long o) -> float4 {
    if (!y_pl) return ld4(Y + o);
    const char* yb = reinterpret_cast<const char*>(Y + (o & ~7L)) + (o & 4) * 2;
    const uint2 h = *reinterpret_cast<const uint2*>(yb), l = *reinterpret_cast<const uint2*>(yb + 16);
    const unsigned m0 = (h.x | l.x) & 0x7fff7fffu, m1 = (h.y | l.y) & 0x7fff7fffu;
    return make_float4((m0 & 0xffffu) ? 1.f : 0.f, (m0 >> 16) ? 1.f : 0.f, (m1 & 0xffffu) ? 1.f : 0.f, (m1 >> 16) ? 1.f : 0.f);
  };
  __shared__ d4 l0[256];
  __shared__ d4 l1[256];
  const int CV = C >> 2;
  const int CVB = CV < 256 ? CV : 256;
  const int RS = 256 / CVB;
  const int tid = threadIdx.x;
  const int cvl = tid % CVB, ro = tid / CVB;
  const long rbeg = (long)blockIdx.x * rows_per_block;
  const long rend = min(M, rbeg + rows_per_block);
  for (int cv0 = 0; cv0 < CV; cv0 += CVB) {
    const int c = (cv0 + cvl) * 4;
    d4 s0 = d4zero(), s1 = d4zero();
    float4 mu = make_float4(0, 0, 0, 0), is = mu, sc = mu, be = mu;
    const bool act = (ro < RS) && (cv0 + cvl < CV);
    const bool mask_x = (MODE == 1) && (gamma != nullptr);
    if (act) {
      if (MODE == 1) { mu = ld4(mean + c); is = ld4(invstd + c); }
      if (mask_x) {
        const float4 ga = ld4(gamma + c);
        be = ld4(beta + c);
        sc = make_float4(is.x * ga.x, is.y * ga.y, is.z * ga.z, is.w * ga.w);
      }
      auto accum = [&](const float4 x, float4 g, const float4 y, long o) {
        if (MODE == 0) {
          s0.x += x.x; s0.y += x.y; s0.z += x.z; s0.w += x.w;
          s1.x += (double)x.x * x.x; s1.y += (double)x.y * x.y; s1.z += (double)x.z * x.z; s1.w += (double)x.w * x.w;
        } else if (MODE == 1) {
          if (mask_x) {
            if (!((x.x - mu.x) * sc.x + be.x > 0.f)) g.x = 0.f;
            if (!((x.y - mu.y) * sc.y + be.y > 0.f)) g.y = 0.f;
            if (!((x.z - mu.z) * sc.z + be.z > 0.f)) g.z = 0.f;
            if (!((x.w - mu.w) * sc.w + be.w > 0.f)) g.w = 0.f;
          } else if (Y) {
            if (!(y.x > 0.f)) g.x = 0.f;
            if (!(y.y > 0.f)) g.y = 0.f;
            if (!(y.z > 0.f)) g.z = 0.f;
            if (!(y.w > 0.f)) g.w = 0.f;
          }
          if (dZ) st4(dZ + o, g);
          am = max(am, abits4(g));
          s0.x += g.x; s0.y += g.y; s0.z += g.z; s0.w += g.w;
          s1.x += (double)(g.x * ((x.x - mu.x) * is.x)); s1.y += (double)(g.y * ((x.y - mu.y) * is.y));
          s1.z += (double)(g.z * ((x.z - mu.z) * is.z)); s1.w += (double)(g.w * ((x.w - mu.w) * is.w));
        } else {
          s0.x += x.x; s0.y += x.y; s0.z += x.z; s0.w += x.w;
        }
      };
      const float4 z4 = make_float4(0, 0, 0, 0);
      long r = rbeg + ro;
      for (; r + 3 * RS < rend; r += 4 * RS) {
        float4 x[4], g[4], y[4];
#pragma unroll
        for (int u = 0; u < 4; ++u) {
          const long o = (r + (long)u * RS) * ld + c;
          x[u] = ld4(X + o);
          if (POOL) {
            g[u] = ld4(dY + pooled_row(r + (long)u * RS, pool_h, pool_w) * ld + c);
            g[u].x *= 0.25f; g[u].y *= 0.25f; g[u].z *= 0.25f; g[u].w *= 0.25f;
          } else {
            g[u] = (MODE == 1) ? ld4(dY + o) : z4;
          }
          y[u] = (MODE == 1 && Y) ? ldy(o) : z4;
        }
#pragma unroll
        for (int u = 0; u < 4; ++u) accum(x[u], g[u], y[u], (r + (long)u * RS) * ld + c);
      }
      for (; r < rend; r += RS) {
        const long o = r * ld + c;
        float4 g1 = z4;
        if (POOL) {
          g1 = ld4(dY + pooled_row(r, pool_h, pool_w) * ld + c);
          g1.x *= 0.25f; g1.y *= 0.25f; g1.z *= 0.25f; g1.w *= 0.25f;
        } else if (MODE == 1) {
          g1 = ld4(dY + o);
        }
        accum(ld4(X + o), g1, (MODE == 1 && Y) ? ldy(o) : z4, o);
      }
    }
    __syncthreads();
    l0[tid] = s0;
    l1[tid] = s1;
    __syncthreads();
    if (ro == 0 && cv0 + cvl < CV) {
      for (int q = 1; q < RS; ++q) {
        d4 a = l0[q * CVB + cvl], b = l1[q * CVB + cvl];
        s0.x += a.x; s0.y += a.y; s0.z += a.z; s0.w += a.w;
        s1.x += b.x; s1.y += b.y; s1.z += b.z; s1.w += b.w;
      }
      double* o = part + (long)blockIdx.x * 2 * C;
      st4d(o + c, s0);
      if (MODE != 2) st4d(o + C + c, s1);
    }
  }
  if (MODE == 1 && amax != nullptr) amax_commit(am, amax);
}

constexpr int FIN_CH = 4;
template <typename T>
__device__ __forceinline__ void reduce_parts(const T* __restrict__ part, int nb, int C, bool two, double& s, double& ss,
                                             int& c, bool& lead) {
  __shared__ double sh0[1024];
  __shared__ double sh1[1024];
  const int SL = blockDim.x / FIN_CH;
  const int cl = threadIdx.x % FIN_CH, j = threadIdx.x / FIN_CH;
  c = blockIdx.x * FIN_CH + cl;
  s = 0.0;
  ss = 0.0;
  if (c < C) {
    constexpr int U = 8;
// ... 195 lines not shown
                                                           const float* __restrict__ invstd,
                                                           const float* __restrict__ gamma,
                                                           const float* __restrict__ sum_dz,
                                                           const float* __restrict__ sum_dzx, float inv_cnt,
                                                           float* __restrict__ dX, float* __restrict__ dZ, long n4,
                                                           int C, const float* __restrict__ beta_mask, int pool_h = 0,
                                                           int pool_w = 0, unsigned* __restrict__ amax = nullptr) {
  unsigned am = 0u;
  const long stride = (long)gridDim.x * blockDim.x;
  long i = BIG ? (long)blockIdx.x * BIG_PIECE + threadIdx.x : (long)blockIdx.x * blockDim.x + threadIdx.x;
  const int c = (int)((i * 4) % C);
  const float4 mu = ld4(mean + c), is = ld4(invstd + c), ga = ld4(gamma + c), a = ld4(sum_dz + c), b = ld4(sum_dzx + c);
  const float4 be = beta_mask ? ld4(beta_mask + c) : make_float4(0, 0, 0, 0);
  const float4 k1 = make_float4(ga.x * is.x, ga.y * is.y, ga.z * is.z, ga.w * is.w);
  const float4 k2 = make_float4(a.x * inv_cnt, a.y * inv_cnt, a.z * inv_cnt, a.w * inv_cnt);
  const float4 k3 = make_float4(is.x * b.x * inv_cnt, is.y * b.y * inv_cnt, is.z * b.z * inv_cnt, is.w * b.w * inv_cnt);
  const bool use_y = !beta_mask && Y != nullptr;
  auto load_g = [&](long j) {
    float4 g;
    if (POOL) {
      g = ld4(dY + pooled_row(j * 4 / C, pool_h, pool_w) * C + c);
      g.x *= 0.25f; g.y *= 0.25f; g.z *= 0.25f; g.w *= 0.25f;
    } else {
      g = BIG ? ld4nt(dY + j * 4) : ld4(dY + j * 4);
    }
    return g;
  };
  auto finish = [&](long j, float4 g, const float4 x, const float4 y) {
    if (beta_mask) {
      if (!((x.x - mu.x) * k1.x + be.x > 0.f)) g.x = 0.f;
      if (!((x.y - mu.y) * k1.y + be.y > 0.f)) g.y = 0.f;
      if (!((x.z - mu.z) * k1.z + be.z > 0.f)) g.z = 0.f;
      if (!((x.w - mu.w) * k1.w + be.w > 0.f)) g.w = 0.f;
    } else if (use_y) {
      if (!(y.x > 0.f)) g.x = 0.f;
      if (!(y.y > 0.f)) g.y = 0.f;
      if (!(y.z > 0.f)) g.z = 0.f;
      if (!(y.w > 0.f)) g.w = 0.f;
    }
    if (dZ) { if (BIG) st4nt(dZ + j * 4, g); else st4(dZ + j * 4, g); }
    float4 o;
    o.x = k1.x * (g.x - k2.x - (x.x - mu.x) * k3.x);
    o.y = k1.y * (g.y - k2.y - (x.y - mu.y) * k3.y);
    o.z = k1.z * (g.z - k2.z - (x.z - mu.z) * k3.z);
    o.w = k1.w * (g.w - k2.w - (x.w - mu.w) * k3.w);
    if (BIG) st4nt(dX + j * 4, o); else st4(dX + j * 4, o);
    am = max(am, abits4(o));
  };
  const float4 z4 = make_float4(0, 0, 0, 0);
  if (BIG) {
    float4 g[BIG_U], x[BIG_U], y[BIG_U];
#pragma unroll
    for (int u = 0; u < BIG_U; ++u) {
      const long j = i + u * 256;
      const bool ok = j < n4;
      g[u] = ok ? load_g(j) : z4;
      x[u] = ok ? ld4nt(X + j * 4) : z4;
      y[u] = (ok && use_y) ? ld4nt(Y + j * 4) : z4;
    }
#pragma unroll
    for (int u = 0; u < BIG_U; ++u) {
      const long j = i + u * 256;
      if (j < n4) finish(j, g[u], x[u], y[u]);
    }
  } else {
    auto one = [&](long j) { finish(j, load_g(j), ld4(X + j * 4), use_y ? ld4(Y + j * 4) : z4); };
    for (; i + stride < n4; i += 2 * stride) {
      one(i);
      one(i + stride);
    }
    if (i < n4) one(i);
  }
  if (amax != nullptr) amax_commit_block(am, amax);
}

__global__ __launch_bounds__(256) void instnorm_fwd_kernel(const float* __restrict__ X, const float* __restrict__ gamma,
                                                           const float* __restrict__ beta, float* __restrict__ Y,
                                                           float* __restrict__ mean_out, float* __restrict__ invstd_out,
                                                           int P, int C, float eps, int relu,
                                                           unsigned* __restrict__ amax = nullptr) {
  __shared__ float red[4][64];
  const int b = blockIdx.y, c = blockIdx.x * 64 + (threadIdx.x & 63), pg = threadIdx.x >> 6;
  const bool ok = c < C;
  const float* x = X + (long)b * P * C + c;
  float s = 0.f;
  if (ok) for (int p = pg; p < P; p += 4) s += x[(long)p * C];
  red[pg][threadIdx.x & 63] = s;
  __syncthreads();
  const int cl = threadIdx.x & 63;
  float mean = (red[0][cl] + red[1][cl] + red[2][cl] + red[3][cl]) / (float)P;
  __syncthreads();
  float v = 0.f;
  if (ok) for (int p = pg; p < P; p += 4) { float d = x[(long)p * C] - mean; v += d * d; }
  red[pg][cl] = v;
  __syncthreads();
  float var = (red[0][cl] + red[1][cl] + red[2][cl] + red[3][cl]) / (float)P;
  float is = rsqrtf(var + eps);
  unsigned am = 0u;
  if (ok) {
    float g = gamma[c], be = beta[c];
    float* y = Y + (long)b * P * C + c;
    for (int p = pg; p < P; p += 4) {
      float o = (x[(long)p * C] - mean) * is * g + be;
      if (relu) o = fmaxf(o, 0.f);
      y[(long)p * C] = o;
      am = max(am, __builtin_bit_cast(unsigned, o) & 0x7fffffffu);
    }
    if (pg == 0) { mean_out[(long)b * C + c] = mean; invstd_out[(long)b * C + c] = is; }
  }
  if (amax != nullptr) amax_commit(am, amax);
}

__global__ __launch_bounds__(256) void instnorm_bwd_kernel(const float* __restrict__ dY, const float* __restrict__ Y,
                                                           const float* __restrict__ X, const float* __restrict__ gamma,
                                                           const float* __restrict__ mean_in,
                                                           const float* __restrict__ invstd_in, float* __restrict__ dX,
                                                           float* __restrict__ dgamma_part, float* __restrict__ dbeta_part,
                                                           int P, int C, int relu, unsigned* __restrict__ amax = nullptr) {
  __shared__ float r0[4][64];
  __shared__ float r1[4][64];
  const int b = blockIdx.y, cl = threadIdx.x & 63, c = blockIdx.x * 64 + cl, pg = threadIdx.x >> 6;
  const bool ok = c < C;
  const long base = (long)b * P * C + c;
  float mean = ok ? mean_in[(long)b * C + c] : 0.f, is = ok ? invstd_in[(long)b * C + c] : 0.f;
  float s0 = 0.f, s1 = 0.f;
  if (ok)
    for (int p = pg; p < P; p += 4) {
      float g = dY[base + (long)p * C];
      if (relu && !(Y[base + (long)p * C] > 0.f)) g = 0.f;
      s0 += g;
      s1 += g * (X[base + (long)p * C] - mean) * is;
    }
  r0[pg][cl] = s0;
  r1[pg][cl] = s1;
  __syncthreads();
  s0 = r0[0][cl] + r0[1][cl] + r0[2][cl] + r0[3][cl];
  s1 = r1[0][cl] + r1[1][cl] + r1[2][cl] + r1[3][cl];
  unsigned am = 0u;
  if (ok) {
    float ga = gamma[c], ip = 1.0f / (float)P;
    for (int p = pg; p < P; p += 4) {
      float g = dY[base + (long)p * C];
      if (relu && !(Y[base + (long)p * C] > 0.f)) g = 0.f;
      float xh = (X[base + (long)p * C] - mean) * is;
      const float d = ga * is * (g - s0 * ip - xh * s1 * ip);
      dX[base + (long)p * C] = d;
      am = max(am, __builtin_bit_cast(unsigned, d) & 0x7fffffffu);
    }
    if (pg == 0) { dgamma_part[(long)b * C + c] = s1; dbeta_part[(long)b * C + c] = s0; }
  }
  if (amax != nullptr) amax_commit(am, amax);
}

__global__ __launch_bounds__(256) void layernorm_fwd_kernel(const float* __restrict__ X, const float* __restrict__ gamma,
                                                            const float* __restrict__ beta, float* __restrict__ Y,
                                                            float* __restrict__ mean_out, float* __restrict__ rstd_out,
                                                            long rows, int W, float eps, unsigned* __restrict__ amax = nullptr,
                                                            const int* __restrict__ limit = nullptr) {
  const int lane = threadIdx.x & 63;
  const long row = (long)blockIdx.x * 4 + (threadIdx.x >> 6);
  if (row >= rows) return;
  if (limit != nullptr && row >= (long)*limit) return;
  unsigned am = 0u;
  const int W4 = W >> 2;
  float4 v[4];
  float s = 0.f;
#pragma unroll
  for (int q = 0; q < 4; ++q) {
    int i = lane + q * 64;
    v[q] = make_float4(0, 0, 0, 0);
    if (i < W4) { v[q] = ld4(X + row * W + i * 4); s += v[q].x + v[q].y + v[q].z + v[q].w; }
  }
  float mean = wave_sum(s) / (float)W;
  float s2 = 0.f;
#pragma unroll
  for (int q = 0; q < 4; ++q) {
    int i = lane + q * 64;
    if (i < W4) {
      float a = v[q].x - mean, b = v[q].y - mean, c = v[q].z - mean, d = v[q].w - mean;
      s2 += a * a + b * b + c * c + d * d;
    }
  }
  float rstd = rsqrtf(wave_sum(s2) / (float)W + eps);
#pragma unroll
  for (int q = 0; q < 4; ++q) {
    int i = lane + q * 64;
    if (i < W4) {
      float4 g = ld4(gamma + i * 4), b = ld4(beta + i * 4), o;
      o.x = (v[q].x - mean) * rstd * g.x + b.x;
      o.y = (v[q].y - mean) * rstd * g.y + b.y;
      o.z = (v[q].z - mean) * rstd * g.z + b.z;
      o.w = (v[q].w - mean) * rstd * g.w + b.w;
      st4(Y + row * W + i * 4, o);
      am = max(am, abits4(o));
    }
  }
  if (amax != nullptr) amax_commit(am, amax);
  if (lane == 0 && mean_out) { mean_out[row] = mean; rstd_out[row] = rstd; }
}

__global__ __launch_bounds__(256) void layernorm_bwd_kernel(const float* __restrict__ dY, const float* __restrict__ X,
                                                            const float* __restrict__ gamma,
                                                            const float* __restrict__ mean_in,
                                                            const float* __restrict__ rstd_in, float* __restrict__ dX,
                                                            float* __restrict__ part, long rows, int W,
                                                            long rows_per_block, const float* __restrict__ extra,
                                                            unsigned* __restrict__ amax = nullptr) {
  unsigned am = 0u;
  __shared__ float4 lg[4][256];
  __shared__ float4 lb[4][256];
  const int lane = threadIdx.x & 63, wv = threadIdx.x >> 6;
  const int W4 = W >> 2;
  float4 ag[4], ab[4];
#pragma unroll
  for (int q = 0; q < 4; ++q) ag[q] = ab[q] = make_float4(0, 0, 0, 0);
  const long rbeg = (long)blockIdx.x * rows_per_block, rend = min(rows, rbeg + rows_per_block);
  for (long row = rbeg + wv; row < rend; row += 4) {
    const float mean = mean_in[row], rstd = rstd_in[row];
    float4 xh[4], dh[4];
    float c1 = 0.f, c2 = 0.f;
#pragma unroll
    for (int q = 0; q < 4; ++q) {
      int i = lane + q * 64;
      xh[q] = dh[q] = make_float4(0, 0, 0, 0);
      if (i < W4) {
        float4 x = ld4(X + row * W + i * 4), dy = ld4(dY + row * W + i * 4), g = ld4(gamma + i * 4);
        xh[q] = make_float4((x.x - mean) * rstd, (x.y - mean) * rstd, (x.z - mean) * rstd, (x.w - mean) * rstd);
        dh[q] = make_float4(dy.x * g.x, dy.y * g.y, dy.z * g.z, dy.w * g.w);
        c1 += dh[q].x + dh[q].y + dh[q].z + dh[q].w;
        c2 += dh[q].x * xh[q].x + dh[q].y * xh[q].y + dh[q].z * xh[q].z + dh[q].w * xh[q].w;
        ag[q].x += dy.x * xh[q].x; ag[q].y += dy.y * xh[q].y; ag[q].z += dy.z * xh[q].z; ag[q].w += dy.w * xh[q].w;
        ab[q].x += dy.x; ab[q].y += dy.y; ab[q].z += dy.z; ab[q].w += dy.w;
      }
    }
    c1 = wave_sum(c1) / (float)W;
    c2 = wave_sum(c2) / (float)W;
    if (dX) {
#pragma unroll
      for (int q = 0; q < 4; ++q) {
        int i = lane + q * 64;
        if (i < W4) {
          float4 o;
          o.x = rstd * (dh[q].x - c1 - xh[q].x * c2);
          o.y = rstd * (dh[q].y - c1 - xh[q].y * c2);
          o.z = rstd * (dh[q].z - c1 - xh[q].z * c2);
          o.w = rstd * (dh[q].w - c1 - xh[q].w * c2);
          if (extra) {
            const float4 e = ld4(extra + row * W + i * 4);
            o.x += e.x; o.y += e.y; o.z += e.z; o.w += e.w;
          }
          st4(dX + row * W + i * 4, o);
          am = max(am, abits4(o));
        }
      }
    }
  }
  if (amax != nullptr) amax_commit_block(am, amax);
  if (!part) return;
#pragma unroll
  for (int q = 0; q < 4; ++q) { lg[wv][lane + q * 64] = ag[q]; lb[wv][lane + q * 64] = ab[q]; }
  __syncthreads();
  if (wv == 0) {
    float* o = part + (long)blockIdx.x * 2 * W;
#pragma unroll
    for (int q = 0; q < 4; ++q) {
      int i = lane + q * 64;
      if (i < W4) {
        float4 g = lg[0][i], b = lb[0][i];
        for (int w = 1; w < 4; ++w) {
          float4 g2 = lg[w][i], b2 = lb[w][i];
          g.x += g2.x; g.y += g2.y; g.z += g2.z; g.w += g2.w;
          b.x += b2.x; b.y += b2.y; b.z += b2.z; b.w += b2.w;
        }
        st4(o + i * 4, g);
        st4(o + W + i * 4, b);
      }
    }
  }
}

__global__ void avgpool2_fwd_kernel(const float* __restrict__ X, float* __restrict__ Y, int B, int H, int W, int C) {
  const int Ho = H >> 1, Wo = W >> 1, C4 = C >> 2;
  long n = (long)B * Ho * Wo * C4;
  long i = (long)blockIdx.x * blockDim.x + threadIdx.x;
  const long stride = (long)gridDim.x * blockDim.x;
  for (; i < n; i += stride) {
    int c4 = (int)(i % C4);
    long t = i / C4;
    int ox = (int)(t % Wo);
    t /= Wo;
    int oy = (int)(t % Ho);
    int b = (int)(t / Ho);
    const float* p = X + (((long)b * H + oy * 2) * W + ox * 2) * C + c4 * 4;
    float4 a = ld4(p), b4 = ld4(p + C), c = ld4(p + (long)W * C), d = ld4(p + (long)W * C + C);
    st4(Y + i * 4, make_float4(0.25f * (a.x + b4.x + c.x + d.x), 0.25f * (a.y + b4.y + c.y + d.y),
                               0.25f * (a.z + b4.z + c.z + d.z), 0.25f * (a.w + b4.w + c.w + d.w)));
  }
}

__global__ void avgpool2_bwd_kernel(const float* __restrict__ dY, float* __restrict__ dX, int B, int H, int W, int C) {
  const int Ho = H >> 1, Wo = W >> 1, C4 = C >> 2;
  long n = (long)B * H * W * C4;
  long i = (long)blockIdx.x * blockDim.x + threadIdx.x;
  const long stride = (long)gridDim.x * blockDim.x;
  for (; i < n; i += stride) {
    int c4 = (int)(i % C4);
    long t = i / C4;
    int x = (int)(t % W);
    t /= W;
    int y = (int)(t % H);
    int b = (int)(t / H);
    float4 g = make_float4(0, 0, 0, 0);
    if ((y >> 1) < Ho && (x >> 1) < Wo) {
      g = ld4(dY + (((long)b * Ho + (y >> 1)) * Wo + (x >> 1)) * C + c4 * 4);
      g.x *= 0.25f; g.y *= 0.25f; g.z *= 0.25f; g.w *= 0.25f;
    }
    st4(dX + i * 4, g);
  }
}

__device__ __forceinline__ float ew1(int op, float a, float b, float s) {
  switch (op) {
    case TRIS_EW_ADD: return a + b;
    case TRIS_EW_AXPY: return s * a + b;
    case TRIS_EW_RELU_BWD: return b > 0.f ? a : 0.f;
    case TRIS_EW_QGELU: return a / (1.0f + expf(-1.702f * a));
    case TRIS_EW_QGELU_BWD: {
      float sg = 1.0f / (1.0f + expf(-1.702f * b));
      return a * (sg + 1.702f * b * sg * (1.f - sg));
    }
    case TRIS_EW_MUL: return a * b;
    case TRIS_EW_SCALE: return s * a;
    case TRIS_EW_RELU: return fmaxf(a, 0.f);
    default: return a;
  }
}
__global__ void ew_kernel(int op, const float* __restrict__ A, const float* __restrict__ Bp, float* __restrict__ O,
                          long n, float s, unsigned* __restrict__ amax = nullptr, long nb = 0) {
  long i = (long)blockIdx.x * blockDim.x + threadIdx.x;
  const long stride = (long)gridDim.x * blockDim.x;
  const long n4 = n >> 2;
  unsigned am = 0u;
  for (long j = i; j < n4; j += stride) {
    float4 a = ld4(A + j * 4), b = Bp ? ld4(Bp + (nb > 0 ? (j * 4) % nb : j * 4)) : make_float4(0, 0, 0, 0);
    const float4 o = make_float4(ew1(op, a.x, b.x, s), ew1(op, a.y, b.y, s), ew1(op, a.z, b.z, s), ew1(op, a.w, b.w, s));
    st4(O + j * 4, o);
    am = max(am, abits4(o));
  }
  for (long j = n4 * 4 + i; j < n; j += stride) {
    const float o = ew1(op, A[j], Bp ? Bp[j] : 0.f, s);
// ... 187 lines not shown
  const long M = (long)B * H * W;
  ColPlan p = col_plan(M, C);
  hipLaunchKernelGGL((col_partial_kernel<1, true>), dim3(p.nb), dim3(256), 0, st, X, dYp, (const float*)nullptr, mean, invstd, M, C,
                     (long)C, p.rpb, (double*)workspace, gamma, beta, (float*)nullptr, H, W, 0, take_amax_next());
  TRIS_LAUNCH_CHECK();
  hipLaunchKernelGGL(part_finalize_kernel<double>, dim3(fin_grid(C, p.nb)), dim3(fin_block(p.nb)), 0, st, (const double*)workspace,
                     p.nb, C, sum_dz, sum_dzx);
  TRIS_LAUNCH_CHECK();
  return 0;
}

extern "C" int tris_bn_bwd_apply_pool_f32(const float* dYp, const float* X, const float* mean, const float* invstd,
                                          const float* gamma, const float* beta, const float* sum_dz, const float* sum_dzx,
                                          float inv_count, float* dX, int B, int H, int W, int C, void* stream) {
  if (C % 4 || (H & 1) || (W & 1)) return (int)hipErrorInvalidValue;
  const long n4 = (long)B * H * W * C / 4;
  hipLaunchKernelGGL(bn_bwd_apply_kernel<true>, dim3(bn_grid(n4, C)), dim3(256), 0, (hipStream_t)stream, dYp, (const float*)nullptr, X,
                     mean, invstd, gamma, sum_dz, sum_dzx, inv_count, dX, (float*)nullptr, n4, C, beta, H, W, take_amax_next());
  TRIS_LAUNCH_CHECK();
  return 0;
}

__global__ __launch_bounds__(256) void bn_out_bound_kernel(const float* __restrict__ gamma, const float* __restrict__ beta, int C,
                                                           float xhat_max, unsigned* __restrict__ out) {
  __shared__ float red[4];
  float m = 0.f;
  for (int c = threadIdx.x; c < C; c += 256) m = fmaxf(m, fabsf(gamma[c]) * xhat_max + fabsf(beta[c]));
  m = block_max_256(m, red);
  if (threadIdx.x == 0) out[0] = __builtin_bit_cast(unsigned, m);
}
extern "C" int tris_bn_out_bound_f32(const float* gamma, const float* beta, int C, float xhat_max, unsigned* out, void* stream) {
  if (C <= 0 || out == nullptr) return (int)hipErrorInvalidValue;
  hipLaunchKernelGGL(bn_out_bound_kernel, dim3(1), dim3(256), 0, (hipStream_t)stream, gamma, beta, C, xhat_max, out);
  TRIS_LAUNCH_CHECK();
  return 0;
}

__global__ __launch_bounds__(256) void amax_bits_kernel(const float* __restrict__ x, long n, unsigned* __restrict__ out) {
  const long n4 = n >> 2;
  const long stride = (long)gridDim.x * blockDim.x;
  unsigned m = 0u;
  for (long i = (long)blockIdx.x * blockDim.x + threadIdx.x; i < n4; i += stride) {
    const float4 v = ld4(x + i * 4);
    m = max(max(m, __builtin_bit_cast(unsigned, v.x) & 0x7fffffffu), __builtin_bit_cast(unsigned, v.y) & 0x7fffffffu);
    m = max(max(m, __builtin_bit_cast(unsigned, v.z) & 0x7fffffffu), __builtin_bit_cast(unsigned, v.w) & 0x7fffffffu);
  }
  for (long i = n4 * 4 + (long)blockIdx.x * blockDim.x + threadIdx.x; i < n; i += stride)
    m = max(m, __builtin_bit_cast(unsigned, x[i]) & 0x7fffffffu);
  amax_commit_block(m, out);
}

__global__ __launch_bounds__(256) void amax_segments_kernel(const float* __restrict__ base, const long* __restrict__ offs,
                                                            const long* __restrict__ sizes, unsigned* __restrict__ slots) {
  const long n = sizes[blockIdx.y];
  const float* x = base + offs[blockIdx.y];
  const long n4 = n >> 2;
  const long stride = (long)gridDim.x * blockDim.x;
  unsigned m = 0u;
  for (long i = (long)blockIdx.x * blockDim.x + threadIdx.x; i < n4; i += stride) m = max(m, abits4(ld4(x + i * 4)));
  for (long i = n4 * 4 + (long)blockIdx.x * blockDim.x + threadIdx.x; i < n; i += stride)
    m = max(m, __builtin_bit_cast(unsigned, x[i]) & 0x7fffffffu);
  amax_commit_block(m, slots + (long)blockIdx.y * 2048);
}

extern "C" int tris_amax_segments_f32(const float* base, const long* offs, const long* sizes, int nseg, unsigned* slots,
                                      void* stream) {
  if (nseg < 1 || (((uintptr_t)base) & 15)) return (int)hipErrorInvalidValue;
  hipLaunchKernelGGL(amax_segments_kernel, dim3(128, (unsigned)nseg), dim3(256), 0, (hipStream_t)stream, base, offs, sizes, slots);
  TRIS_LAUNCH_CHECK();
  return 0;
}

extern "C" int tris_amax_bits_f32(const float* x, long n, unsigned* out, void* stream) {
  if (n < 1 || (((uintptr_t)x) & 15)) return (int)hipErrorInvalidValue;
  long g = (n / 4 + 255) / 256;
  g = g > 2048 ? 2048 : (g < 1 ? 1 : g);
  hipLaunchKernelGGL(amax_bits_kernel, dim3((unsigned)g), dim3(256), 0, (hipStream_t)stream, x, n, out);
  TRIS_LAUNCH_CHECK();
  return 0;
}

extern "C" int tris_part_finalize_f32(const double* part, int rows, int C, float* out0, float* out1, void* stream) {
  if (rows < 1 || C < 1) return (int)hipErrorInvalidValue;
  hipLaunchKernelGGL(part_finalize_kernel<double>, dim3(fin_grid(C, rows)), dim3(fin_block(rows)), 0, (hipStream_t)stream, part, rows,
                     C, out0, out1);
  TRIS_LAUNCH_CHECK();
  return 0;
}

extern "C" int tris_part_finalize_bound_f32(const double* part, int rows, int C, float* out0, float* out1, const float* gamma,
                                            const float* invstd, float inv_count, float xhat_max, const unsigned* dz_word,
                                            unsigned* bound_out, void* stream) {
  if (rows < 1 || C < 1 || out1 == nullptr || gamma == nullptr || invstd == nullptr || dz_word == nullptr || bound_out == nullptr)
    return (int)hipErrorInvalidValue;
  hipLaunchKernelGGL(part_finalize_kernel<double>, dim3(fin_grid(C, rows)), dim3(fin_block(rows)), 0, (hipStream_t)stream, part, rows,
                     C, out0, out1, gamma, invstd, inv_count, xhat_max, dz_word, bound_out);
  TRIS_LAUNCH_CHECK();
  return 0;
}

extern "C" int tris_bn_bwd_apply_f32(const float* dY, const float* Y, const float* X, const float* mean,
                                     const float* invstd, const float* gamma, const float* sum_dz, const float* sum_dzx,
                                     float inv_count, float* dX, float* dZ, long M, int C, const float* beta_mask,
                                     void* stream) {
  long n4 = M * C / 4;
  const int streams = 3 + ((Y && !beta_mask) ? 1 : 0) + (dZ ? 1 : 0);
  if (big_form(n4, C, streams))
    hipLaunchKernelGGL((bn_bwd_apply_kernel<false, true>), dim3(big_grid(n4)), dim3(256), 0, (hipStream_t)stream, dY, Y, X, mean,
                       invstd, gamma, sum_dz, sum_dzx, inv_count, dX, dZ, n4, C, beta_mask, 0, 0, take_amax_next());
  else
    hipLaunchKernelGGL((bn_bwd_apply_kernel<false, false>), dim3(bn_grid(n4, C)), dim3(256), 0, (hipStream_t)stream, dY, Y, X, mean,
                       invstd, gamma, sum_dz, sum_dzx, inv_count, dX, dZ, n4, C, beta_mask, 0, 0, take_amax_next());
  TRIS_LAUNCH_CHECK();
  return 0;
}

extern "C" int tris_colsum_f32(const float* X, long M, int N, long ld, float* out, float* workspace, void* stream) {
  hipStream_t st = (hipStream_t)stream;
  if (N % 4 || ld % 4 || (((uintptr_t)X) & 15)) {
    hipLaunchKernelGGL(colsum_scalar_kernel, dim3(cdiv(N, 256)), dim3(256), 0, st, X, M, N, ld, out);
    TRIS_LAUNCH_CHECK();
    return 0;
  }
  ColPlan p = col_plan(M, N);
  hipLaunchKernelGGL(col_partial_kernel<2>, dim3(p.nb), dim3(256), 0, st, X, nullptr, nullptr, nullptr, nullptr, M, N,
                     ld, p.rpb, (double*)workspace);
  TRIS_LAUNCH_CHECK();
  hipLaunchKernelGGL(part_finalize_kernel<double>, dim3(fin_grid(N, p.nb)), dim3(fin_block(p.nb)), 0, st, (const double*)workspace, p.nb, N,
                     out, (float*)nullptr);
  TRIS_LAUNCH_CHECK();
  return 0;
}

extern "C" int tris_instnorm_fwd_f32(const float* X, const float* gamma, const float* beta, float* Y, float* mean,
                                     float* invstd, int B, int P, int C, float eps, int relu, void* stream) {
  hipLaunchKernelGGL(instnorm_fwd_kernel, dim3(cdiv(C, 64), B), dim3(256), 0, (hipStream_t)stream, X, gamma, beta, Y,
                     mean, invstd, P, C, eps, relu, take_amax_next());
  TRIS_LAUNCH_CHECK();
  return 0;
}

extern "C" int tris_instnorm_bwd_f32(const float* dY, const float* Y, const float* X, const float* gamma,
                                     const float* mean, const float* invstd, float* dX, float* dgamma_part,
                                     float* dbeta_part, int B, int P, int C, int relu, void* stream) {
  hipLaunchKernelGGL(instnorm_bwd_kernel, dim3(cdiv(C, 64), B), dim3(256), 0, (hipStream_t)stream, dY, Y, X, gamma,
                     mean, invstd, dX, dgamma_part, dbeta_part, P, C, relu, take_amax_next());
  TRIS_LAUNCH_CHECK();
  return 0;
}

extern "C" int tris_layernorm_fwd_f32(const float* X, const float* gamma, const float* beta, float* Y, float* mean,
                                      float* rstd, long rows, int W, float eps, void* stream) {
  if (W % 4 || W > 1024) return (int)hipErrorInvalidValue;
  hipLaunchKernelGGL(layernorm_fwd_kernel, dim3(cdiv(rows, 4)), dim3(256), 0, (hipStream_t)stream, X, gamma, beta, Y,
                     mean, rstd, rows, W, eps, take_amax_next(), g_rows_limit);
  TRIS_LAUNCH_CHECK();
  return 0;
}

extern "C" { __attribute__((visibility("hidden"))) int tris_internal_ln_bwd_blocks = 512; }
static long ln_bwd_rpb(long rows) {
  const long target = tris_internal_ln_bwd_blocks;
  long rpb = (rows + target - 1) / target;
  const long floor_ = target > 128 ? 4 : 8;
  return rpb < floor_ ? floor_ : rpb;
}
extern "C" long tris_layernorm_bwd_workspace_bytes(long rows, int W) {
  const long rpb = ln_bwd_rpb(rows);
  long nb = (rows + rpb - 1) / rpb;
  if (nb < 512) nb = 512;
  return nb * 2 * W * (long)sizeof(float);
}

extern "C" int tris_layernorm_bwd_f32(const float* dY, const float* X, const float* gamma, const float* mean,
                                      const float* rstd, float* dX, float* dgamma, float* dbeta, long rows, int W,
                                      float* workspace, const float* extra, void* stream) {
  if (W % 4 || W > 1024) return (int)hipErrorInvalidValue;
  hipStream_t st = (hipStream_t)stream;
  const long rpb = ln_bwd_rpb(rows);
  int nb = (int)((rows + rpb - 1) / rpb);
  float* part = dgamma ? workspace : nullptr;
  hipLaunchKernelGGL(layernorm_bwd_kernel, dim3(nb), dim3(256), 0, st, dY, X, gamma, mean, rstd, dX, part, rows, W,
                     rpb, extra, take_amax_next());
  TRIS_LAUNCH_CHECK();
  if (dgamma) {
    hipLaunchKernelGGL(part_finalize_kernel<float>, dim3(fin_grid(W, nb)), dim3(fin_block(nb)), 0, st, (const float*)workspace, nb, W, dgamma, dbeta);
    TRIS_LAUNCH_CHECK();
  }
  return 0;
}

extern "C" int tris_avgpool2_fwd_f32(const float* X, float* Y, int B, int H, int W, int C, void* stream) {
  if (C % 4) return (int)hipErrorInvalidValue;
  long n = (long)B * (H / 2) * (W / 2) * (C / 4);
  hipLaunchKernelGGL(avgpool2_fwd_kernel, dim3(grid_for(n)), dim3(256), 0, (hipStream_t)stream, X, Y, B, H, W, C);
  TRIS_LAUNCH_CHECK();
  return 0;
}

extern "C" int tris_avgpool2_bwd_f32(const float* dY, float* dX, int B, int H, int W, int C, void* stream) {
  if (C % 4) return (int)hipErrorInvalidValue;
  long n = (long)B * H * W * (C / 4);
  hipLaunchKernelGGL(avgpool2_bwd_kernel, dim3(grid_for(n)), dim3(256), 0, (hipStream_t)stream, dY, dX, B, H, W, C);
  TRIS_LAUNCH_CHECK();
  return 0;
}

extern "C" int tris_elementwise_f32(int op, const float* A, const float* B, float* O, long n, float s, void* stream) {
  hipLaunchKernelGGL(ew_kernel, dim3(grid_for((n + 3) / 4)), dim3(256), 0, (hipStream_t)stream, op, A, B, O, n, s,
                     take_amax_next());
  TRIS_LAUNCH_CHECK();
  return 0;
}

extern "C" int tris_elementwise_bcast_f32(int op, const float* A, const float* B, float* O, long n, long nb, float s,
                                          void* stream) {
  if (B == nullptr || nb < 4 || (nb & 3) || (n & 3) || n % nb) return (int)hipErrorInvalidValue;
  hipLaunchKernelGGL(ew_kernel, dim3(grid_for(n / 4)), dim3(256), 0, (hipStream_t)stream, op, A, B, O, n, s, take_amax_next(), nb);
  TRIS_LAUNCH_CHECK();
  return 0;
}

namespace {
__global__ __launch_bounds__(256) void scale_exp_fwd_kernel(const float* __restrict__ X, const float* __restrict__ ls,
                                                            float* __restrict__ O, float* __restrict__ e_out, long n) {
  const float e = expf(ls[0]);
  if (blockIdx.x == 0 && threadIdx.x == 0) e_out[0] = e;
  const long stride = (long)gridDim.x * blockDim.x;
  for (long i = (long)blockIdx.x * blockDim.x + threadIdx.x; i < n; i += stride) O[i] = X[i] * e;
}
__global__ __launch_bounds__(256) void scale_exp_bwd_kernel(const float* __restrict__ dO, const float* __restrict__ O,
                                                            const float* __restrict__ ls, float* __restrict__ dX,
                                                            double* __restrict__ part, long n) {
  __shared__ double red[256];
  const float e = expf(ls[0]);
  const long stride = (long)gridDim.x * blockDim.x;
  float acc = 0.f;
  for (long i = (long)blockIdx.x * blockDim.x + threadIdx.x; i < n; i += stride) {
    const float g = dO[i];
    if (dX) dX[i] = g * e;
    acc += g * O[i];
  }
  red[threadIdx.x] = (double)acc;
  __syncthreads();
  for (int h = 128; h > 0; h >>= 1) {
    if ((int)threadIdx.x < h) red[threadIdx.x] += red[threadIdx.x + h];
    __syncthreads();
  }
  if (threadIdx.x == 0) part[blockIdx.x] = red[0];
}
__global__ void scale_exp_bwd_finish_kernel(const double* __restrict__ part, int nb, float* __restrict__ dls) {
  double s = 0.0;
  for (int i = 0; i < nb; ++i) s += part[i];
  dls[0] = (float)s;
}
constexpr int SE_BLOCKS = 128;
}
extern "C" int tris_scale_exp_fwd_f32(const float* X, const float* ls, float* O, float* e_out, long n, void* stream) {
  hipLaunchKernelGGL(scale_exp_fwd_kernel, dim3(grid_for(n)), dim3(256), 0, (hipStream_t)stream, X, ls, O, e_out, n);
  TRIS_LAUNCH_CHECK();
  return 0;
}
extern "C" long tris_scale_exp_workspace_bytes() { return (long)SE_BLOCKS * sizeof(double); }
extern "C" int tris_scale_exp_bwd_f32(const float* dO, const float* O, const float* ls, float* dX, float* dls,
                                      float* workspace, long n, void* stream) {
  double* part = reinterpret_cast<double*>(workspace);
  hipLaunchKernelGGL(scale_exp_bwd_kernel, dim3(SE_BLOCKS), dim3(256), 0, (hipStream_t)stream, dO, O, ls, dX, part, n);
  TRIS_LAUNCH_CHECK();
  hipLaunchKernelGGL(scale_exp_bwd_finish_kernel, dim3(1), dim3(1), 0, (hipStream_t)stream, part, SE_BLOCKS, dls);
  TRIS_LAUNCH_CHECK();
  return 0;
}

extern "C" int tris_nchw_to_nhwc_f32(const float* X, float* Y, int B, int C, int H, int W, void* stream) {
  long n = (long)B * C * H * W;
  hipLaunchKernelGGL(nchw_to_nhwc_kernel, dim3(grid_for(n)), dim3(256), 0, (hipStream_t)stream, X, Y, B, C,
                     (long)H * W);
  TRIS_LAUNCH_CHECK();
  return 0;
}
```

tris_amd/ops.py:

```python
import math
import os

import torch

from . import _lib
from ._lib import CONSTS, call, query
from .config import cfg

EW = CONSTS


class NoGpuError(RuntimeError):
    pass


_RAW_STREAM = getattr(torch._C, "_cuda_getCurrentRawStream", None)


def _stream():
    if _RAW_STREAM is not None:
        return _RAW_STREAM(torch.cuda.current_device())
    return torch.cuda.current_stream().cuda_stream


# ... 222 lines not shown
            def coll():
                w = dist.all_reduce(buf, group=group, async_op=True)
                w.wait()
            dist.barrier(group=group)
            if not probe(r, issue, coll) and backend_cls is None and k < len(reps):
                backend_cls = k
    if cfg.stream_probe_log:
        print(f"[place_streams] queue classes of the candidates {cls}, collective backend on class {backend_cls}", flush=True)
    free = [k for k in range(len(reps)) if k != backend_cls]
    if len(free) < 3:
        return None
    order = ([cls[0]] if cls[0] in free else []) + [k for k in free if k != cls[0]]
    compute, text, wgrad = reps[order[0]], reps[order[1]], reps[order[2]]
    used = {cls[cands.index(compute)], cls[cands.index(text)], cls[cands.index(wgrad)]}
    issue = next((c for c, k in zip(cands, cls) if k == backend_cls), None)
    if issue is None:
        issue = next((c for c, k in zip(cands, cls) if k not in used), wgrad)
    _CAL[dev] = [text, wgrad, issue]
    _WG.pop(dev, None)
    for key in [k for k in _SIDE_STREAMS if k[0] == dev]:
        _SIDE_STREAMS.pop(key)
    return None if compute is null else compute


def _new_side_stream(dev, slot):
    pool = _calibrated_streams(dev)
    return pool[slot] if slot < len(pool) else torch.cuda.Stream(device=dev)


def _wgrad_stream():
    dev = torch.cuda.current_device()
    if dev not in _WG:
        _WG[dev] = _new_side_stream(dev, 1)
    return _WG[dev]


def on_wgrad_stream(fn, *tensors, sink=None):
    if _SEG is not None:
        return _SEG.defer(fn, tensors, sink)
    if not _wgrad_enabled():
        return fn()
    main, side = torch.cuda.current_stream(), _wgrad_stream()
    side.wait_stream(main)
    with torch.cuda.stream(side):
        r = fn()
    for t in tensors:
        if t is not None:
            t.record_stream(side)
    return r


_SIDE_STREAMS = {}


def side_stream(name):
    key = (torch.cuda.current_device(), name)
    if key not in _SIDE_STREAMS:
        slot = {"text": 0, "reduce": 2}.get(name)
        _SIDE_STREAMS[key] = _new_side_stream(key[0], slot) if slot is not None else torch.cuda.Stream(device=key[0])
    return _SIDE_STREAMS[key]


def wgrad_join(into=None):
    if _SEG is not None:
        return
    if not _WG and not _SIDE_STREAMS:
        return
    cur = torch.cuda.current_stream() if into is None else into
    dev = torch.cuda.current_device()
    if dev in _WG and _WG[dev] != cur:
        cur.wait_stream(_WG[dev])
    for (d, _), st in _SIDE_STREAMS.items():
        if d == dev and st != cur:
            cur.wait_stream(st)


def _sink(p):
    if p is not None and getattr(p, "_tris_sink", False):
        return p.grad
    return None


def _emit(p, make, needs, reads=None):
    if not needs:
        return None
    s = _sink(p)
    if s is not None:
        if reads is not None and cfg.side_param_grads:
            on_wgrad_stream(lambda: make(s), *reads, sink=s)
        else:
            make(s)
        return None
    out = torch.empty_like(p, memory_format=torch.preserve_format)
    make(out)
    return out


_PROF = None
_PROF_SHAPES = False


def profile_begin():
    global _PROF
    _PROF = []


def profile_end():
    global _PROF
    rec, _PROF = _PROF, None
    torch.cuda.synchronize()
    return [(k, f, a.elapsed_time(b), nb) for k, f, a, b, nb in rec]


def _shape_tag(text):
    return text if _PROF_SHAPES else None


def _timed(kind, flops, fn, tag=None, nbytes=0):
    if _PROF is None:
        return fn()
    a, b = torch.cuda.Event(enable_timing=True), torch.cuda.Event(enable_timing=True)
    a.record()
    r = fn()
    b.record()
    if r is not False:
        _PROF.append((kind if tag is None else f"{kind}:{tag}", flops, a, b, nbytes))
    return r


_BATCH_INVARIANT = 0


class batch_invariant:
    def __enter__(self):
        global _BATCH_INVARIANT
        _BATCH_INVARIANT += 1
        if _BATCH_INVARIANT == 1:
            call("tris_set_conv_direct_thread", 0)
        _H2["paused"] += 1
        return self

    def __exit__(self, *exc):
        global _BATCH_INVARIANT
        _BATCH_INVARIANT -= 1
        _H2["paused"] -= 1
        if _BATCH_INVARIANT == 0:
            call("tris_set_conv_direct_thread", -1)
        return False


def gemm(A, B, C, M, N, K, lda, ldb, ldc, tA, tB, batch=1, sA=0, sB=0, sC=0, bias=None, bias_mode=0, resid=None,
         ldr=0, sR=0, act=0, alpha=1.0, use_ws=True, pre_out=None, dact=None, w_a=False, w_b=False, w_bt=False, mark=True):
    _chk(A, B, C, bias, resid)
    if pre_out is not None or dact is not None or batch != 1 or _BATCH_INVARIANT:
        A, B = unplanes(A), unplanes(B)
    if pre_out is not None or dact is not None:
        if _BATCH_INVARIANT or batch != 1:
            return False
        h2_arm(A, B)
        h2_mark_next(C)
        call("tris_gemm_epilogue_next", P(pre_out), P(dact))
        return _timed("gemm", 2.0 * M * N * K, lambda: _declinable(
            "tris_gemm_f32", P(A), P(B), P(C), M, N, K, lda, ldb, ldc, int(tA), int(tB), 1, 0, 0, 0, P(bias), bias_mode, P(resid),
            ldr, sR, act, float(alpha), None, 0, _stream()),
            nbytes=4.0 * (M * K + K * N + M * N * (2 + int(resid is not None))))
    if _BATCH_INVARIANT and batch == 1 and not tA and M < 4 and lda == K and ldc == N and (resid is None or ldr == N) and bias_mode != 2:
        A4 = A.new_zeros(4, K)
        A4[:M].copy_(A.reshape(M, K))
        R4 = None
        if resid is not None:
            R4 = resid.new_zeros(4, N)
            R4[:M].copy_(resid.reshape(M, N))
        C4 = C.new_empty(4, N)
        gemm(A4, B, C4, 4, N, K, K, ldb, N, False, tB, bias=bias, bias_mode=bias_mode, resid=R4, ldr=N, act=act, alpha=alpha,
             use_ws=use_ws)
        C.reshape(M, N).copy_(C4[:M])
        return C
    ws = workspace(0) if (use_ws and batch == 1 and not _BATCH_INVARIANT) else None
    blind = _rows_limit_blind(A, tA, batch)
    if (w_b and batch == 1 and not tA and M >= cfg.gemm_convert and cfg.gemm_convert > 0 and K % 32 == 0 and lda == K and getattr(B, "_tris_linear_w", False)
            and planes_on() and pl_word(A) is None and A.is_contiguous() and A.data_ptr() % 16 == 0 and _pl_weight_ok(B) and not blind):
        A = _a_planes(A, M, K)
    if blind:
        PL_STATS["last"] = PL_STATS["last_t"] = False
        pA, pB = P(A), P(unplanes(B))
    else:
        pA, pB = h2_pp(A, B, w_a=w_a, w_b=w_b, k_red=K, w_bt=w_bt and not tB) if batch == 1 else (P(A), P(B))
    if batch == 1 and PL_STATS["last_t"]:
        tB, ldb = True, K
    if mark:
        h2_mark_next(C)
    if ws is not None and cfg.fuse_splitk:
        tk = splitk_tickets()
        if tk is not None:
            call("tris_splitk_tickets_next", tk.data_ptr(), tk.numel())
    _timed("gemm", 2.0 * M * N * K * batch, lambda: call(
        "tris_gemm_f32", pA, pB, P(C), M, N, K, lda, ldb, ldc, int(tA), int(tB), batch, sA, sB, sC, P(bias),
        bias_mode, P(resid), ldr, sR, act, float(alpha), P(ws), 0 if ws is None else ws.numel() * 4, _stream()),
        tag=(f"{'T' if tA else 'N'}{'T' if tB else 'N'} M{M} N{N} K{K} b{batch}" if _PROF_SHAPES else None),
        nbytes=4.0 * ((M * K if (sA == 0 and batch > 1) else batch * M * K) + batch * K * N
                      + batch * M * N * (2 if resid is not None else 1)))
    return C


def colsum(X, M, N, out):
    ws = workspace(query("tris_col_workspace_bytes", M, N))
    call("tris_colsum_f32", P(X), M, N, N, P(out), P(ws), _stream())
    return out


def ew(op, A, B=None, s=0.0, out=None):
    _chk(A, B)
    out = torch.empty_like(A) if out is None else out
    h2_mark_next(out)
    call("tris_elementwise_f32", EW[op], P(A), P(B), P(out), A.numel(), float(s), _stream())
    return out


def nchw_to_nhwc(x):
    _chk(x)
    if x.dim() == 4 and x.permute(0, 2, 3, 1).is_contiguous():
        return x.permute(0, 2, 3, 1)
    x = x.contiguous()
    B, C, H, W = x.shape
    y = torch.empty(B, H, W, C, device=x.device, dtype=x.dtype)
    call("tris_nchw_to_nhwc_f32", P(x), P(y), B, C, H, W, _stream())
    return y


def _launch_with_stats(y, M, N, launch):
    import ctypes
    part = torch.empty(((M + 127) // 128) * 2 * N, device=y.device, dtype=torch.float64)
    rows = ctypes.c_int(0)
    launch(part, ctypes.byref(rows))
    if rows.value > 0:
        y._bn_part = (part, rows.value)


def _declinable(name, *args):
    err = getattr(_lib.load(), name)(*args)
    if err == -2:
        return False
    if err != 0:
        raise _lib.TrisHipError(f"{name} failed with hipError_t {err}")
    return True


class GradBox:
    __slots__ = ("value", "consumed")

    def __init__(self):
        self.value = None
        self.consumed = False

    def deposit(self, g):
        if self.consumed or self.value is not None:
            return False
        self.value = g
        return True


_H2 = {"pool": None, "next": 0, "step": 0, "paused": 0, "arenas": [], "const": None, "const_next": 0, "const_tags": {}}
_H2_STEP_IDS = [0]
H2_SLOTS = 4096
H2_SUB = 2048
H2_CONST_SLOTS = 1024
H2_PREPASS_MAX = 1 << 25
H2_AUTO_KEEP = 4


def h2_on():
    return _ARITH == "h2" and not _H2["paused"] and not _thread_mode_is_set()


_H2_ARENAS = []


def h2_register_arena(arena):
    import weakref
    r = weakref.ref(arena)
    _H2_ARENAS.append(r)
    for p in arena.params:
        p._tris_arena = r


def _h2_live_arenas():
    out, words = [], 0
    for r in reversed(list(_H2_ARENAS)):
        a = r()
        if a is None or not a.params or getattr(a.params[0], "_tris_arena", None) is not r:
            _H2_ARENAS.remove(r)
        elif _H2["pool"] is not None and a.p.device == _H2["pool"].device and words + len(a.params) <= H2_SLOTS // 2:
            out.append(a)
            words += len(a.params)
    return out


def h2_weights_amax(arenas=None):
    base = 0
    for a in (_h2_live_arenas() if arenas is None else arenas):
        if not hasattr(a, "_h2_dev"):
            a._h2_dev = (torch.tensor(list(a.offsets), device=a.p.device, dtype=torch.int64),
                         torch.tensor([p.numel() for p in a.params], device=a.p.device, dtype=torch.int64))
        call("tris_amax_segments_f32", P(a.p), a._h2_dev[0].data_ptr(), a._h2_dev[1].data_ptr(), len(a.params),
             _H2["pool"].data_ptr() + 4 * H2_SUB * base, _stream())
        if cfg.h2_planes:
            if not hasattr(a, "_pl_dev"):
                idx = [i for i, p in enumerate(a.params) if _pl_weight_ok(p)]
                a._pl_idx = idx
                a._pl_dev = None if not idx else (
                    torch.tensor([a.offsets[i] for i in idx], device=a.p.device, dtype=torch.int64),
                    torch.tensor([a.params[i].numel() for i in idx], device=a.p.device, dtype=torch.int64),
                    torch.tensor(idx, device=a.p.device, dtype=torch.int64))
                a.pl = torch.zeros_like(a.p) if idx else None
            if a._pl_dev is not None:
                call("tris_h2_planes_segments_f32", P(a.p), a._pl_dev[0].data_ptr(), a._pl_dev[1].data_ptr(), a._pl_dev[2].data_ptr(),
                     len(a._pl_idx), _H2["pool"].data_ptr() + 4 * H2_SUB * base, P(a.pl), _stream())
            if not hasattr(a, "_plt_dev"):
                idt = [i for i in getattr(a, "_pl_idx", []) if _pl_weight_t_ok(a.params[i])]
                a._plt_idx = idt
                mk = lambda v: torch.tensor(v, device=a.p.device, dtype=torch.int64)
                a._plt_dev = None if not idt else (mk([a.offsets[i] for i in idt]), mk([a.params[i].shape[0] for i in idt]),
                                                   mk([a.params[i].shape[1] for i in idt]), mk(idt))
                a.plt = torch.zeros_like(a.p) if idt else None
            if a._plt_dev is not None:
                call("tris_h2_planes_t_segments_f32", P(a.p), a._plt_dev[0].data_ptr(), a._plt_dev[1].data_ptr(), a._plt_dev[2].data_ptr(),
                     a._plt_dev[3].data_ptr(), len(a._plt_idx), _H2["pool"].data_ptr() + 4 * H2_SUB * base, P(a.plt), _stream())
        base += len(a.params)
    return base


def _pl_weight_t_ok(p):
    if p.dim() == 2:
        return cfg.gemm_convert > 0 and getattr(p, "_tris_linear_w", False) and p.shape[0] % 64 == 0 and p.shape[1] % 64 == 0
    return p.dim() == 4 and p.shape[2] * p.shape[3] == 1 and p.shape[0] % 64 == 0 and p.shape[1] % 64 == 0


def _pl_weight_ok(p):
    if p.dim() == 2:
        return cfg.gemm_convert > 0 and getattr(p, "_tris_linear_w", False) and p.shape[1] % 8 == 0 and p.is_contiguous()
    return p.dim() == 4 and p.shape[1] % 8 == 0 and (p.is_contiguous(memory_format=torch.channels_last) or p.shape[2] * p.shape[3] == 1)


def _a_planes(A, M, K):
    slot = _h2_amax(A)
    if slot is None:
        return A
    t = torch.empty_like(A)
    call("tris_h2_planes_f32", P(A), P(t), A.numel(), slot, _stream())
    PL_STATS["converted"] = PL_STATS.get("converted", 0) + 1
    return pl_tag(t, slot)


def _h2_new_step_id():
    _H2_STEP_IDS[0] += 1
    return _H2_STEP_IDS[0]


def h2_begin_step(explicit=True):
    if _ARITH != "h2":
        return None
    _H2["in_step"] = bool(explicit)
    wgrad_join()
    dev = torch.device("cuda", torch.cuda.current_device())
    live = _H2.setdefault("auto_pools", {})
    if _H2["pool"] is None or _H2["pool"].device != dev:
        _H2["pool"] = torch.zeros(H2_SLOTS * H2_SUB, device=dev, dtype=torch.int32)
        live.clear()
    elif not explicit and _H2.get("auto_grad") and not _H2.get("private") and not torch.cuda.is_current_stream_capturing():
        live[_H2["step"]] = _H2["pool"]
        while len(live) > H2_AUTO_KEEP:
            live.pop(next(iter(live)))
        _H2["pool"] = torch.zeros(H2_SLOTS * H2_SUB, device=dev, dtype=torch.int32)
    else:
        if explicit:
            live.clear()
        _H2["pool"].zero_()
    _H2["auto_grad"] = (not explicit) and torch.is_grad_enabled() and not _H2.get("private")
    _H2["step"] = _h2_new_step_id()
    _H2["plane_numel"] = {}
    _PL_GRAD.clear()
    base = 0
    arenas = _h2_live_arenas() if not _H2.get("private") else []
    for a in arenas:
        for i, p in enumerate(a.params):
            p._h2 = (_H2["step"], _H2["pool"].data_ptr() + 4 * H2_SUB * (base + i), p._version)
        base += len(a.params)
    _H2["next"] = _H2["base"] = base
    _H2["arenas"] = arenas
    h2_weights_amax(arenas)
    if cfg.h2_planes:
        for a in arenas:
            for i in (a._pl_idx if getattr(a, "pl", None) is not None else ()):
                p = a.params[i]
                p._plw = (_H2["step"], a.pl.data_ptr() + 4 * a.offsets[i], p._h2[1])
                _H2["plane_numel"][p._h2[1]] = p.numel()
            for i in (a._plt_idx if getattr(a, "plt", None) is not None else ()):
                p = a.params[i]
                p._plwt = (_H2["step"], a.plt.data_ptr() + 4 * a.offsets[i], p._h2[1])
    return _H2["pool"]


def h2_end_step():
    _H2["in_step"] = False


def h2_auto_step():
    if not planes_on() or _H2.get("in_step") or _H2.get("auto_lock") or _H2.get("private"):
        return False
    if _H2["pool"] is not None and _H2["next"] == _H2.get("base", -1):
        return False
    h2_begin_step(explicit=False)
    return True


class h2_auto_lock:

    def __enter__(self):
        self.prev = _H2.get("auto_lock", False)
        _H2["auto_lock"] = True

    def __exit__(self, *a):
        _H2["auto_lock"] = self.prev


class h2_step:

    def __init__(self, explicit=True):
        self.explicit, self.mine = explicit, False

    def __enter__(self):
        self.mine = h2_on() and not _H2.get("in_step") and not _H2.get("private")
        if self.mine:
            h2_begin_step(explicit=self.explicit)
        return self

    def __exit__(self, *exc):
        if self.mine and self.explicit:
            h2_end_step()
        return False


class h2_private_pool:

    def __init__(self, slots=512):
        self.slots, self.pool = slots, None

    def __enter__(self):
        self.active = _ARITH == "h2"
        if not self.active:
            return self
        self.saved = {k: _H2.get(k) for k in ("pool", "next", "step", "arenas", "private", "limit")}
        dev = torch.device("cuda", torch.cuda.current_device())
        if self.pool is None or self.pool.device != dev:
            self.pool = torch.zeros(self.slots * H2_SUB, device=dev, dtype=torch.int32)
        _H2.update(pool=self.pool, arenas=[], private=True, limit=self.slots)
        self.reset()
        return self

    def reset(self):
        if self.active:
            self.pool.zero_()
            _H2.update(next=0, step=_h2_new_step_id())

    def __exit__(self, *exc):
        if self.active:
            _H2.update(self.saved)
        return False


class h2_paused:

    def __enter__(self):
        _H2["paused"] += 1

    def __exit__(self, *a):
        _H2["paused"] -= 1


def _h2_slot():
    limit = _H2.get("limit") or H2_SLOTS
    if _H2["pool"] is None or (_H2["next"] >= limit and not _H2.get("private")):
        h2_begin_step(explicit=bool(_H2.get("in_step")))
    i = _H2["next"]
    if i >= limit:
        return None
    _H2["next"] = i + 1
    return _H2["pool"].data_ptr() + 4 * H2_SUB * i


def h2_mark_next(t):
    if t is None or not h2_on():
        return
    slot = _h2_slot()
    if slot is None:
        return
    call("tris_amax_next", slot)
    t._h2 = (_H2["step"], slot, t._version)


def h2_bound_word(gamma, beta, C, xhat_max):
    if not h2_on():
        return None
    slot = _h2_slot()
    if slot is not None:
        call("tris_bn_out_bound_f32", P(gamma), P(beta), C, float(xhat_max), slot, _stream())
    return slot


def _h2_tag_slot(t):
    tag = getattr(t, "_h2", None)
    if tag is not None and tag[0] == _H2["step"] and tag[2] == t._version:
        return tag[1]
    return None


def _h2_const_slot(t):
    key = id(t)
    tag = _H2["const_tags"].get(key)
    if tag is not None and tag[1] == t.data_ptr() and tag[3]() is t and _H2["const"] is not None and _H2["const"].device == t.device:
        if tag[0] == t._version:
            return tag[2]
        i = (tag[2] - _H2["const"].data_ptr()) // (4 * H2_SUB)
        _H2["const"][i * H2_SUB:(i + 1) * H2_SUB].zero_()
        call("tris_amax_bits_f32", P(t), t.numel(), tag[2], _stream())
        _H2["const_tags"][key] = (t._version, t.data_ptr(), tag[2], tag[3])
        return tag[2]
    if _H2["const"] is None or _H2["const"].device != t.device:
        _H2["const"] = torch.zeros(H2_CONST_SLOTS * H2_SUB, device=t.device, dtype=torch.int32)
        _H2["const_next"] = 0
        _H2["const_tags"].clear()
    if _H2["const_next"] >= H2_CONST_SLOTS:
        return None
    import weakref
    slot = _H2["const"].data_ptr() + 4 * H2_SUB * _H2["const_next"]
    _H2["const_next"] += 1
    call("tris_amax_bits_f32", P(t), t.numel(), slot, _stream())
    _H2["const_tags"][key] = (t._version, t.data_ptr(), slot, weakref.ref(t))
    return slot


def _h2_amax(t):
    slot = _h2_tag_slot(t)
    if slot is not None:
        return slot
    dense = t.is_contiguous() or (t.dim() == 4 and t.is_contiguous(memory_format=torch.channels_last))
    if not (t.numel() <= H2_PREPASS_MAX and dense and t.data_ptr() % 16 == 0 and t.numel() > 0):
        return None
    if isinstance(t, torch.nn.Parameter) and not getattr(t, "_tris_arena", False):
        slot = _h2_const_slot(t)
        if slot is not None:
            return slot
    slot = _h2_slot()
    if slot is None:
        return None
    call("tris_amax_bits_f32", P(t), t.numel(), slot, _stream())
    try:
        t._h2 = (_H2["step"], slot, t._version)
    except AttributeError:
        pass
    return slot


def h2_arm(A, B, a_slot=None, b_slot=None):
    if not h2_on():
        return False
    a = a_slot if a_slot is not None else (_h2_amax(A) if A is not None else None)
    b = None
    if a is not None:
        b = b_slot if b_slot is not None else (_h2_amax(B) if B is not None else None)
    if a is None or b is None:
        return False
    call("tris_h2_next", a, b, 0.0, 0.0)
    return True


PL_STATS = {"unplanes": 0, "dx_planes": 0, "dy_planes": 0, "products": 0, "mixed": 0, "last": False, "last_t": False}


_HAS_GPU = None


def planes_on():
    global _HAS_GPU
    if _HAS_GPU is None:
        _HAS_GPU = torch.cuda.is_available()
    return _HAS_GPU and cfg.h2_planes and h2_on() and not _BATCH_INVARIANT


def pl_word(t):
    tag = getattr(t, "_pl", None) if t is not None else None
    if tag is None:
        return None
    if (tag[0] != _H2["step"] and tag[0] not in _H2.get("auto_pools", ())) or tag[2] != t.data_ptr():
        raise RuntimeError("a plane tensor outlived the step whose amax pool scales it")
    return tag[1]


def pl_tag(t, word):
    t._pl = (_H2["step"], word, t.data_ptr())
    t._h2 = (_H2["step"], word, t._version)
    _H2.setdefault("plane_numel", {})[word] = t.numel()
    return t


def h2_range_report(threshold=0.01):
    numel = _H2.get("plane_numel") or {}
    pool = _H2["pool"]
    if pool is None or not numel:
        return {"plane_tensors": 0, "elements": 0, "elements_below_floor": 0, "max_fraction_below_floor": 0.0, "out_of_range_operands": 0}
    torch.cuda.synchronize()
    base = pool.data_ptr()
    words = sorted(numel)
    idx = torch.tensor([(w - base) // (4 * H2_SUB) for w in words], device=pool.device, dtype=torch.int64)
    cnt = pool.view(-1, H2_SUB)[idx][:, 1::16].to(torch.int64).sum(1).cpu().tolist()
    fr = [c / max(numel[w], 1) for c, w in zip(cnt, words)]
    return {"plane_tensors": len(words), "elements": int(sum(numel.values())), "elements_below_floor": int(sum(cnt)),
            "max_fraction_below_floor": max(fr), "out_of_range_operands": sum(1 for f in fr if f > threshold)}


def _unplanes_raw(t, cache=True):
    w = pl_word(t)
    c = getattr(t, "_pl_f32", None) if cache else None
    if c is None:
        c = torch.empty_like(t)
        call("tris_h2_unplanes_f32", P(t), P(c), t.numel(), w, _stream())
        c._h2 = (_H2["step"], w, c._version)
        if cache:
            t._pl_f32 = c
        PL_STATS["unplanes"] += 1
    return c


class _UnplanesFn(torch.autograd.Function):

    @staticmethod
    def forward(ctx, t):
        return _unplanes_raw(t, cache=False)

    @staticmethod
    def backward(ctx, g):
        return g


def unplanes(t):
    if pl_word(t) is None:
        return t
    if t.requires_grad and torch.is_grad_enabled():
        return _UnplanesFn.apply(t)
    return _unplanes_raw(t)


_PL_CONST = {}


def _pl_weight(w):
    tag = getattr(w, "_plw", None)
    if tag is not None and tag[0] == _H2["step"]:
        return tag[1], tag[2]
    if not _pl_weight_ok(w):
        return None
    word = _h2_amax(w)
    if word is None:
        return None
    c = _PL_CONST.get(id(w))
    if c is not None and c[0] == w._version and c[1] == w.data_ptr() and c[2] == word and c[4]() is w:
        return c[3].data_ptr(), word
    import weakref
    wc = cl_weight(w)
    pl = torch.empty(wc.numel(), device=w.device, dtype=torch.float32)
    call("tris_h2_planes_f32", wc.data_ptr(), P(pl), wc.numel(), word, _stream())
    if len(_PL_CONST) > 4096:
        _PL_CONST.clear()
    _PL_CONST[id(w)] = (w._version, w.data_ptr(), word, pl, weakref.ref(w))
    return pl.data_ptr(), word


def _retag(t, tag):
    if tag is not None and t is not None and getattr(t, "_pl", None) is None:
        t._pl = tag
        t._h2 = (tag[0], tag[1], t._version)
    return t


_PL_GRAD = {}


_PL_GRAD_CB = [False]


def _pl_grad_end_of_backward():
    _PL_GRAD_CB[0] = False
    if _PL_GRAD:
        left = [(hex(k), v[2]) for k, v in _PL_GRAD.items()]
        _PL_GRAD.clear()
        raise RuntimeError(f"plane gradients without a plane-aware consumer at the end of backward: {left[:4]}")


def pl_grad_out(t, word):
    pl_tag(t, word)
    _PL_GRAD[t.data_ptr()] = (_H2["step"], word, tuple(t.shape))
    PL_STATS["dx_planes"] += 1
    if not _PL_GRAD_CB[0]:
        try:
            torch.autograd.Variable._execution_engine.queue_callback(_pl_grad_end_of_backward)
            _PL_GRAD_CB[0] = True
        except RuntimeError:
            pass
    return t


def pl_grad_in(dy):
    ent = _PL_GRAD.pop(dy.data_ptr(), None)
    if ent is not None and ent[0] == _H2["step"] and ent[2] == tuple(dy.shape):
        if getattr(dy, "_pl", None) is None:
            dy._pl = (ent[0], ent[1], dy.data_ptr())
            dy._h2 = (ent[0], ent[1], dy._version)
        PL_STATS["dy_planes"] += 1
    elif getattr(dy, "_pl", None) is not None:
        raise RuntimeError("a plane gradient reached a second consumer")
    return dy


def h2_pp(A, B, a_slot=None, b_slot=None, y_planes=False, w_a=False, w_b=False, k_red=32, w_bt=False, y_mask=False):
    PL_STATS["last"] = PL_STATS["last_t"] = False
    if A is None or B is None or a_slot is not None or b_slot is not None or not planes_on() or k_red % 32 != 0:
        if pl_word(A) is not None or pl_word(B) is not None:
            A, B = unplanes(A), unplanes(B)
        h2_arm(A, B, a_slot, b_slot)
        return P(A), P(B)
    wa, wb = pl_word(A), pl_word(B)
    if wa is not None or wb is not None:
        pa = (P(A), wa) if wa is not None else (_pl_weight(A) if w_a else None)
        pb = (P(B), wb) if wb is not None else (_pl_weight(B) if w_b else None)
        if w_bt and wb is None and pa is not None:
            tt = getattr(B, "_plwt", None)
            if tt is not None and tt[0] == _H2["step"]:
                pb = (tt[1], tt[2])
                PL_STATS["last_t"] = True
        if pa is not None and pb is not None:
            call("tris_h2_next_planes", pa[1], pb[1], (1 if y_planes else 0) | (2 if PL_STATS["last_t"] else 0) | (4 if y_mask else 0))
            PL_STATS["products"] += 1
            PL_STATS["last"] = True
            return pa[0], pb[0]
        PL_STATS["mixed"] += 1
        A, B = unplanes(A), unplanes(B)
    h2_arm(A, B)
    return P(A), P(B)


class _BnBwdLink:
    __slots__ = ("x", "mean", "invstd", "gamma", "beta", "from_y", "dz", "part", "rows", "dzw", "mask")

    def __init__(self, x, mean, invstd, gamma, beta, from_y):
        self.x, self.mean, self.invstd, self.gamma, self.beta, self.from_y = x, mean, invstd, gamma, beta, from_y
        self.dz = self.part = self.dzw = None
        self.rows = 0
        self.mask = None

    def fill(self, dz, part, rows, dzw=None):
        self.dz, self.part, self.rows, self.dzw = (dz.data_ptr(), dz._version, tuple(dz.shape)), part, rows, dzw

    def take(self, dy):
        dz, part, rows, dzw = self.dz, self.part, self.rows, self.dzw
        self.dz = self.part = self.dzw = None
        if dz is None or (dy.data_ptr(), dy._version, tuple(dy.shape)) != dz:
            return None
        return part, rows, dzw


def _bn_bwd_fuse_enabled():
    return cfg.bn_bwd_fuse


class LinearFn(torch.autograd.Function):

    @staticmethod
    def forward(ctx, x, w, b, resid, act, stats=False, grad_box=None, grad_box_out=None, grad_box_res=None, bn_link=None,
                act_link=None):
        _chk(x, w, b, resid)
        ctx.grad_box, ctx.grad_box_out, ctx.grad_box_res = grad_box, grad_box_out, grad_box_res
        ctx.act_link = act_link
        ctx.bn_link = bn_link if (bn_link is not None and x.is_contiguous() and bn_link.x.shape == x.shape) else None
        x = x.contiguous()
        K = x.shape[-1]
        N = w.numel() // K
        M = x.numel() // K
        y = torch.empty(*x.shape[:-1], N, device=x.device, dtype=torch.float32)
        if resid is not None:
            resid = resid.contiguous()
        want_stats = stats and b is None and resid is None and act == 0
        if want_stats:
            _launch_with_stats(y, M, N, lambda part, rows: _timed(
                "gemm", 2.0 * M * N * K, lambda: (lambda pp: call("tris_gemm_bnstat_f32", pp[0], pp[1], P(y), M, N, K,
                                                                  part.data_ptr(), rows, _stream()))(h2_pp(x, w, w_b=True, k_red=K)),
                nbytes=4.0 * (M * K + K * N + M * N), tag=_shape_tag(f"bnstat M{M} N{N} K{K}")))
        else:
            gemm(x, w, y, M, N, K, K, K, N, False, True, bias=b, bias_mode=1 if b is not None else 0, resid=resid,
                 ldr=N, act=act, w_b=True)
        ctx.act, ctx.dims = act, (M, N, K)
        ctx.has_b, ctx.has_r = b is not None, resid is not None
        ctx.params = (w, b)
        ctx.x_pl = getattr(x, "_pl", None)
        ctx.save_for_backward(x, w, b, y if act == 1 else None)
        return y

    @staticmethod
    def backward(ctx, dy):
        if ctx.act == 2:
            raise RuntimeError("fused QuickGELU epilogue is forward-only; use QGeluFn when gradients are needed")
        if ctx.act == 1 and ctx.has_r:
            raise RuntimeError("relu + residual epilogue is forward-only")
        x, w, b, y = ctx.saved_tensors
        pw, pb = ctx.params
        M, N, K = ctx.dims
        dy = pl_grad_in(dy.contiguous())
        _retag(x, ctx.x_pl)
        if pl_word(dy) is not None and (ctx.has_r or ctx.has_b or ctx.act == 1):
            dy = unplanes(dy)
        if pl_word(dy) is None:
            x = unplanes(x)
        d_res = dy if ctx.has_r and ctx.needs_input_grad[3] else None
        if d_res is not None and ctx.grad_box_res is not None and ctx.grad_box_res.deposit(d_res):
            d_res = None
        if d_res is not None and _wgrad_enabled() and ctx.needs_input_grad[1]:
            d_res = dy.clone()
        if ctx.act == 1:
            dy = ew("TRIS_EW_RELU_BWD", dy, y)
        dx = None
        box = ctx.grad_box
        extra = None
        if box is not None:
            box.consumed = True
            if box.value is not None:
                extra, box.value = box.value, None
        if ctx.needs_input_grad[0]:
            dx = torch.empty_like(x)
            link, fused = ctx.bn_link, False
            if link is not None and (box is None or extra is not None):
                import ctypes
                part = torch.empty(((M + 127) // 128) * 2 * K, device=x.device, dtype=torch.float64)
                rows = ctypes.c_int(0)
                ypl = link.from_y and pl_word(x) is not None
                if not ypl or pl_word(dy) is not None:
                    dzw = _h2_slot() if planes_on() else None

                    def launch():
                        bits = ypl and link.mask is not None
                        pp = h2_pp(dy, w, w_b=True, y_planes=ypl, k_red=N, w_bt=True, y_mask=bits)
                        if dzw is not None:
                            call("tris_amax_next", dzw)
                        by = (P(x) if (PL_STATS["last"] or not ypl) else P(unplanes(x))) if link.from_y else None
                        if bits and PL_STATS["last"]:
                            by = link.mask.data_ptr()
                        call("tris_gemm_bnbwd_f32", pp[0], pp[1], P(dx), M, K, N, P(extra), K, P(link.x), by,
                             P(link.mean), P(link.invstd), P(link.gamma), P(link.beta), part.data_ptr(), ctypes.byref(rows), _stream())
                        return rows.value > 0
                    _timed("gemm_bnbwd", 2.0 * M * N * K, launch, tag=_shape_tag(f"M{M} N{K} K{N}"),
                           nbytes=4.0 * (M * N + N * K + M * K * (2 + int(link.from_y) + int(extra is not None))))
                    if rows.value > 0:
                        fused = True
                        link.fill(dx, part, rows.value, dzw)
            alink = ctx.act_link
            if not fused and alink is not None and extra is None:
                if gemm(dy, w, dx, M, K, N, N, K, K, False, False, dact=alink.pre) is not False:
                    fused = alink.applied = True
            if not fused:
                gemm(dy, w, dx, M, K, N, N, K, K, False, False, resid=extra, ldr=K, w_b=True, w_bt=True)
        elif extra is not None:
            raise RuntimeError("a residual gradient was handed to a layer whose input needs no gradient")
        if dx is not None and ctx.grad_box_out is not None and ctx.grad_box_out.deposit(dx):
            dx = None
        dw = None
        if ctx.needs_input_grad[1]:
            if _sink(pw) is not None:
                on_wgrad_stream(lambda: gemm(dy, x, _sink(pw), N, K, M, N, K, K, True, False, mark=False), dy, x, sink=_sink(pw))
            else:
                dw = _emit(pw, lambda o: gemm(dy, x, o, N, K, M, N, K, K, True, False, mark=False), True)
        db = None
        if ctx.has_b:
            db = _emit(pb, lambda o: colsum(dy, M, N, o), ctx.needs_input_grad[2], reads=(dy,))
        return dx, dw, db, d_res, None, None, None, None, None, None, None


def linear(x, w, b=None, resid=None, act=0, stats=False, grad_box=None, grad_box_out=None, grad_box_res=None, act_link=False):
    link = getattr(x, "_bn_link", None)
    if link is not None and not (torch.is_grad_enabled() and x.requires_grad and _bn_bwd_fuse_enabled()):
        link = None
    alink = getattr(x, "_act_link", None) if (act_link and torch.is_grad_enabled() and x.requires_grad) else None
    return LinearFn.apply(x, w, b, resid, act, stats, grad_box, grad_box_out, grad_box_res, link, alink)


class _ActLink:
    __slots__ = ("pre", "applied")

    def __init__(self, pre):
        self.pre, self.applied = pre, False


class LinearQGeluFn(torch.autograd.Function):

    @staticmethod
    def forward(ctx, x, w, b):
        _chk(x, w, b)
        x = x.contiguous()
        K = x.shape[-1]
        N = w.numel() // K
        M = x.numel() // K
        y = torch.empty(*x.shape[:-1], N, device=x.device, dtype=torch.float32)
        pre = torch.empty_like(y)
        if gemm(x, w, y, M, N, K, K, K, N, False, True, bias=b, bias_mode=1 if b is not None else 0, act=2, pre_out=pre) is False:
            gemm(x, w, pre, M, N, K, K, K, N, False, True, bias=b, bias_mode=1 if b is not None else 0)
            ew("TRIS_EW_QGELU", pre, out=y)
        ctx.dims, ctx.has_b, ctx.params = (M, N, K), b is not None, (w, b)
        ctx.link = y._act_link = _ActLink(pre)
        ctx.save_for_backward(x, w, pre)
        return y

    @staticmethod
    def backward(ctx, dy):
        x, w, pre = ctx.saved_tensors
        pw, pb = ctx.params
        M, N, K = ctx.dims
        dy = dy.contiguous()
        dpre = dy if ctx.link.applied else ew("TRIS_EW_QGELU_BWD", dy, pre)
        dx = None
        if ctx.needs_input_grad[0]:
            dx = torch.empty_like(x)
            gemm(dpre, w, dx, M, K, N, N, K, K, False, False)
        dw = None
        if ctx.needs_input_grad[1]:
            if _sink(pw) is not None:
                on_wgrad_stream(lambda: gemm(dpre, x, _sink(pw), N, K, M, N, K, K, True, False, mark=False), dpre, x, sink=_sink(pw))
            else:
                dw = _emit(pw, lambda o: gemm(dpre, x, o, N, K, M, N, K, K, True, False, mark=False), True)
        db = None
        if ctx.has_b:
            db = _emit(pb, lambda o: colsum(dpre, M, N, o), ctx.needs_input_grad[2], reads=(dpre,))
        return dx, dw, db


def linear_qgelu(x, w, b=None):
    return LinearQGeluFn.apply(x, w, b)


class MatmulFn(torch.autograd.Function):

    @staticmethod
    def forward(ctx, A, B, tB):
        _chk(A, B)
        A, B = A.contiguous(), B.contiguous()
        K = A.shape[-1]
        M = A.numel() // K
        N = B.shape[0] if tB else B.shape[1]
        C = torch.empty(*A.shape[:-1], N, device=A.device, dtype=torch.float32)
        gemm(A, B, C, M, N, K, K, B.shape[1], N, False, tB)
        ctx.tB, ctx.dims = tB, (M, N, K)
        ctx.params = (B,)
        ctx.save_for_backward(A, B)
        return C

    @staticmethod
    def backward(ctx, dC):
        A, B = ctx.saved_tensors
        M, N, K = ctx.dims
        dC = dC.contiguous()
        dA = dB = None
        if ctx.needs_input_grad[0]:
            dA = torch.empty_like(A)
            if ctx.tB:
                gemm(dC, B, dA, M, K, N, N, K, K, False, False)
            else:
                gemm(dC, B, dA, M, K, N, N, N, K, False, True)
        if ctx.needs_input_grad[1]:
            if ctx.tB:
                dB = _emit(ctx.params[0], lambda o: gemm(dC, A, o, N, K, M, N, K, K, True, False, mark=False), True)
            else:
                dB = _emit(ctx.params[0], lambda o: gemm(A, dC, o, K, N, M, K, N, N, True, False, mark=False), True)
        return dA, dB, None


def matmul(A, B, tB=False):
    return MatmulFn.apply(A, B, tB)


class BmmFn(torch.autograd.Function):

    @staticmethod
    def forward(ctx, A, B, tB, alpha):
        _chk(A, B)
        A, B = A.contiguous(), B.contiguous()
        Bt = B.shape[0]
        shared = A.dim() == 2
        M, K = A.shape[-2], A.shape[-1]
        N = B.shape[1] if tB else B.shape[2]
        C = torch.empty(Bt, M, N, device=B.device, dtype=torch.float32)
        gemm(A, B, C, M, N, K, K, B.shape[2], N, False, tB, batch=Bt, sA=0 if shared else M * K,
             sB=B.shape[1] * B.shape[2], sC=M * N, alpha=alpha)
        ctx.cfg = (tB, alpha, shared, Bt, M, N, K)
        ctx.save_for_backward(A, B)
        return C

    @staticmethod
    def backward(ctx, dC):
        A, B = ctx.saved_tensors
        tB, alpha, shared, Bt, M, N, K = ctx.cfg
        dC = dC.contiguous()
        sA = 0 if shared else M * K
        dA = dB = None
        if ctx.needs_input_grad[0]:
            dAp = torch.empty(Bt, M, K, device=B.device, dtype=torch.float32)
            if tB:
                gemm(dC, B, dAp, M, K, N, N, K, K, False, False, batch=Bt, sA=M * N, sB=N * K, sC=M * K, alpha=alpha)
            else:
                gemm(dC, B, dAp, M, K, N, N, N, K, False, True, batch=Bt, sA=M * N, sB=K * N, sC=M * K, alpha=alpha)
            if shared:
                dA = torch.empty(M, K, device=B.device, dtype=torch.float32)
                colsum(dAp, Bt, M * K, dA)
            else:
                dA = dAp
        if ctx.needs_input_grad[1]:
            dB = torch.empty_like(B)
            if tB:
                gemm(dC, A, dB, N, K, M, N, K, K, True, False, batch=Bt, sA=M * N, sB=sA, sC=N * K, alpha=alpha)
            else:
                gemm(A, dC, dB, K, N, M, K, N, N, True, False, batch=Bt, sA=sA, sB=M * N, sC=K * N, alpha=alpha)
        return dA, dB, None, None


def bmm(A, B, tB=False, alpha=1.0):
    return BmmFn.apply(A, B, tB, alpha)


class Conv3x3Fn(torch.autograd.Function):

    @staticmethod
    def forward(ctx, x, w, stride, stats=False, lazy=None, bn_link=None):
        _chk(x, w)
        ctx.bn_link = bn_link if (bn_link is not None and stride == 1 and not bn_link.from_y and x.is_contiguous()
                                  and bn_link.x.shape == x.shape) else None
        x = x.contiguous()
        ctx.params = (w,)
        w = cl_weight(w)
        B, H, W, Cin = x.shape
        Cout = w.shape[0]
        ctx.lazy = None
        ctx.stride = stride
        if lazy is not None:
            xr, mean, invstd, gamma, beta, bound = lazy
            if stride == 1 and conv3x3_bnin_ok(x.shape, Cout):
                y = torch.empty(B, H, W, Cout, device=x.device, dtype=torch.float32)
                fl = 2.0 * B * H * W * Cout * 9 * Cin
                nb = 4.0 * (B * H * W * (Cin + Cout) + 9 * Cin * Cout)
                ctx.h2_in = bound

                def launch(part, rows):
                    return _timed("conv3x3_fwd", fl, lambda: (bound is not None and h2_arm(None, ctx.params[0], a_slot=bound), call(
                        "tris_conv3x3_fwd_bnin_f32", P(xr), P(mean), P(invstd), P(gamma), P(beta), P(w), P(y), B, H, W, Cin, Cout,
                        None if part is None else part.data_ptr(), rows, _stream()))[1], nbytes=nb,
                        tag=_shape_tag(f"bnin B{B} {H}x{W} {Cin}->{Cout}"))
                if stats:
                    _launch_with_stats(y, B * H * W, Cout, launch)
                else:
                    launch(None, None)
                ctx.lazy = True
# ... 259 lines not shown
        mb = None
        if group is not None and in_arena:
            from . import comm
            mb = comm.syncbn_mailbox(group, 2 * C)
        direct = in_arena and (group is None or mb is not None)
        if direct:
            p_dz, p_dzx = P(sb), P(sg)
            dg = db = None
        else:
            sums = torch.empty(2 * C, device=x.device, dtype=torch.float32)
            p_dz, p_dzx = P(sums), P(sums, C)
        mask_x = relu and not has_res and y is None
        got = ctx.link.take(dy) if ctx.link is not None else None
        if got is not None and dx_pl:
            dzw = got[2] if got[2] is not None else _h2_amax(dy)
        if ctx.pool:
            Bn, H, W = x.shape[0], x.shape[1], x.shape[2]
            if dzw is not None:
                call("tris_amax_next", dzw)
            call("tris_bn_bwd_reduce_pool_f32", P(dy), P(x), P(mean), P(invstd), Bn, H, W, C, p_dz, p_dzx, P(ws), P(gamma), P(beta),
                 _stream())
        dz_first = got is None and not ctx.pool and want_dz and relu and y is not None
        if dz_first:
            d_res = torch.empty_like(x)
        bound_word = None
        if got is not None and dx_pl and mb is None and (direct or group is None) and ctx.needs_input_grad[0]:
            bound_word = _h2_slot()
        if got is not None and bound_word is not None:
            call("tris_part_finalize_bound_f32", got[0].data_ptr(), got[1], C, p_dz, p_dzx, P(gamma), P(invstd), 1.0 / float(count),
                 math.sqrt(max(count - 1, 1)), dzw, bound_word, _stream())
        elif got is not None:
            call("tris_part_finalize_f32", got[0].data_ptr(), got[1], C, p_dz, p_dzx, _stream())
        elif not ctx.pool:
            if dzw is not None:
                call("tris_amax_next", dzw)
            if y_is_pl and not mask_x:
                call("tris_bn_bwd_reduce_pl_f32", P(dy), P(y), P(x), P(mean), P(invstd), M, C, p_dz, p_dzx, P(ws),
                     P(d_res) if dz_first else None, _stream())
            else:
                call("tris_bn_bwd_reduce_f32", P(dy), None if mask_x else P(y), P(x), P(mean), P(invstd), M, C, p_dz, p_dzx, P(ws),
                     P(gamma) if mask_x else None, P(beta) if mask_x else None, P(d_res) if dz_first else None, _stream())
        if mb is not None:
            sums = torch.empty(2 * C, device=x.device, dtype=torch.float32)
            if dx_pl and dzw is not None and ctx.needs_input_grad[0] and bound_word is None and cfg.syncbn_bound:
                bound_word = _h2_slot()
            if bound_word is not None and dx_pl and dzw is not None:
                mb.bn_bwd_exchange(sb, sg, sums, gamma, invstd, 1.0 / float(count), math.sqrt(max(count - 1, 1)), dzw, bound_word)
            else:
                mb.exchange(sb, sums, 1, src1=sg)
            p_dz, p_dzx = P(sums), P(sums, C)
        elif not direct:
            dg = _emit(ctx.params[0], lambda o: o.copy_(sums[C:]), ctx.needs_input_grad[1])
            db = _emit(ctx.params[1], lambda o: o.copy_(sums[:C]), ctx.needs_input_grad[2])
            if group is not None:
                from . import comm
                comm.syncbn_all_reduce_sum(sums, group=group)
        dx = None
        inv_cnt = 1.0 / float(count)

        def apply(g, ymask, dz_out, beta_m):
            if dx_pl:
                word = bound_word
                if word is None:
                    word = _h2_slot()
                    call("tris_bn_bwd_bound_f32", P(gamma), P(invstd), p_dz, p_dzx, C, inv_cnt, math.sqrt(max(count - 1, 1)), dzw, word,
                         _stream())
                if ctx.pool:
                    call("tris_bn_bwd_apply_pool_pl_f32", P(g), P(x), P(mean), P(invstd), P(gamma), P(beta), p_dz, p_dzx, inv_cnt, P(dx),
                         word, x.shape[0], x.shape[1], x.shape[2], C, _stream())
                else:
                    if ymask is not None and not y_is_pl:
                        raise RuntimeError("operand planes: the ReLU mask of a plane-output BatchNorm must come from plane y")
                    call("tris_bn_bwd_apply_pl_f32", P(g), P(ymask), P(x), P(mean), P(invstd), P(gamma), p_dz, p_dzx, inv_cnt, P(dx),
                         word, P(dz_out), M, C, P(beta_m), _stream())
                pl_grad_out(dx, word)
                return
            h2_mark_next(dx)
            if ctx.pool:
                call("tris_bn_bwd_apply_pool_f32", P(g), P(x), P(mean), P(invstd), P(gamma), P(beta), p_dz, p_dzx, inv_cnt, P(dx),
                     x.shape[0], x.shape[1], x.shape[2], C, _stream())
            else:
                call("tris_bn_bwd_apply_f32", P(g), P(unplanes(ymask)) if ymask is not None else None, P(x), P(mean), P(invstd),
                     P(gamma), p_dz, p_dzx, inv_cnt, P(dx), P(dz_out), M, C, P(beta_m), _stream())
        if ctx.pool:
            if ctx.needs_input_grad[0]:
                dx = torch.empty_like(x)
                apply(dy, None, None, None)
        elif got is not None:
            if want_dz:
                d_res = dy
            if ctx.needs_input_grad[0]:
                dx = torch.empty_like(x)
                apply(dy, None, None, None)
        elif dz_first:
            if ctx.needs_input_grad[0]:
                dx = torch.empty_like(x)
                apply(d_res, None, None, None)
        elif ctx.needs_input_grad[0] or want_dz:
            dx = torch.empty_like(x)
            if want_dz:
                d_res = torch.empty_like(x)
            apply(dy, None if mask_x else y, d_res if want_dz else None, beta if mask_x else None)
        if ctx.grad_box is not None and d_res is not None and ctx.grad_box.deposit(d_res):
            d_res = None
        return dx, dg, db, None, None, d_res, None, None, None, None, None, None, None, None, None, None, None, None


def batch_norm(x, gamma, beta, rmean, rvar, resid=None, relu=False, training=True, momentum=0.1, eps=1e-5, group=None,
               grad_box=None, lazy=False, bwd_link=False, pool=False, planes=False, dx_planes=False):
    part = getattr(x, "_bn_part", None) if training else None
    bwd_link = bool(bwd_link and training and torch.is_grad_enabled() and x.requires_grad and _bn_bwd_fuse_enabled())
    if pool and not (training and relu and resid is None and not lazy and x.dim() == 4 and x.shape[1] % 2 == 0
                     and x.shape[2] % 2 == 0 and cfg.bn_pool):
        return avgpool2(BatchNormFn.apply(x, gamma, beta, rmean, rvar, resid, relu, training, momentum, eps, group, part, grad_box,
                                          lazy, bwd_link, False, planes, dx_planes))
    return BatchNormFn.apply(x, gamma, beta, rmean, rvar, resid, relu, training, momentum, eps, group, part, grad_box, lazy,
                             bwd_link, pool, planes, dx_planes)


class AvgPool2Fn(torch.autograd.Function):
    @staticmethod
    def forward(ctx, x, grad_box_out=None):
        _chk(x)
        ctx.grad_box_out = grad_box_out
        x = x.contiguous()
        B, H, W, C = x.shape
        y = torch.empty(B, H // 2, W // 2, C, device=x.device, dtype=torch.float32)
        w = pl_word(x)
        if w is not None and C % 8 == 0:
            call("tris_avgpool2_fwd_pl_f32", P(x), P(y), w, B, H, W, C, _stream())
            pl_tag(y, w)
        else:
            call("tris_avgpool2_fwd_f32", P(unplanes(x)), P(y), B, H, W, C, _stream())
        ctx.shape = (B, H, W, C)
        return y

    @staticmethod
    def backward(ctx, dy):
        B, H, W, C = ctx.shape
        dy = unplanes(pl_grad_in(dy.contiguous()))
        dx = torch.empty(B, H, W, C, device=dy.device, dtype=torch.float32)
        call("tris_avgpool2_bwd_f32", P(dy), P(dx), B, H, W, C, _stream())
        if ctx.grad_box_out is not None and ctx.grad_box_out.deposit(dx):
            dx = None
        return dx, None


def avgpool2(x, grad_box_out=None):
    return AvgPool2Fn.apply(x, grad_box_out)


class LayerNormFn(torch.autograd.Function):
    @staticmethod
    def forward(ctx, x, g, b, eps, grad_box=None):
        _chk(x, g, b)
        ctx.grad_box = grad_box
        x = x.contiguous()
        W = x.shape[-1]
        rows = x.numel() // W
        y = torch.empty_like(x)
        st = torch.empty(2, rows, device=x.device, dtype=torch.float32)
        h2_mark_next(y)
        call("tris_layernorm_fwd_f32", P(x), P(g), P(b), P(y), P(st), P(st, rows), rows, W, eps, _stream())
        ctx.dims = (rows, W)
        ctx.params = (g, b)
        ctx.save_for_backward(x, g, b, st)
        return y

    @staticmethod
    def backward(ctx, dy):
        x, g, b, st = ctx.saved_tensors
        rows, W = ctx.dims
        dy = dy.contiguous()
        dx = torch.empty_like(x) if ctx.needs_input_grad[0] else None
        box, extra = ctx.grad_box, None
        if box is not None:
            box.consumed = True
            if box.value is not None:
                extra, box.value = box.value.contiguous(), None
                if dx is None:
                    raise RuntimeError("a residual gradient was handed to a LayerNorm whose input needs no gradient")
        need_p = ctx.needs_input_grad[1] or ctx.needs_input_grad[2]
        ws = workspace(query("tris_layernorm_bwd_workspace_bytes", rows, W))
        sg, sb = _sink(ctx.params[0]), _sink(ctx.params[1])
        if need_p and sg is not None and sb is not None and sg.is_contiguous() and sb.is_contiguous():
            h2_mark_next(dx)
            call("tris_layernorm_bwd_f32", P(dy), P(x), P(g), P(st), P(st, rows), P(dx), P(sg), P(sb), rows, W, P(ws),
                 P(extra), _stream())
            return dx, None, None, None, None
        dgb = torch.empty(2, W, device=x.device, dtype=torch.float32) if need_p else None
        h2_mark_next(dx)
        call("tris_layernorm_bwd_f32", P(dy), P(x), P(g), P(st), P(st, rows), P(dx), P(dgb), P(dgb, W),
             rows, W, P(ws), P(extra), _stream())
        dg = _emit(ctx.params[0], lambda o: o.copy_(dgb[0]), ctx.needs_input_grad[1])
        db = _emit(ctx.params[1], lambda o: o.copy_(dgb[1]), ctx.needs_input_grad[2])
        return dx, dg, db, None, None


def layer_norm(x, g, b, eps=1e-5, grad_box=None):
    return LayerNormFn.apply(x, g, b, eps, grad_box)


class MhaFn(torch.autograd.Function):

    @staticmethod
    def forward(ctx, qkv, heads, causal):
        _chk(qkv)
        qkv = qkv.contiguous()
        N, L, W3 = qkv.shape
        W = W3 // 3
        out = torch.empty(N, L, W, device=qkv.device, dtype=torch.float32)
        h2_mark_next(out)
        call("tris_mha_fwd_f32", P(qkv), P(out), N, L, W, heads, int(causal), _stream())
        ctx.cfg = (N, L, W, heads, int(causal))
        ctx.save_for_backward(qkv)
        return out

    @staticmethod
    def backward(ctx, do):
        (qkv,) = ctx.saved_tensors
        N, L, W, heads, causal = ctx.cfg
        do = do.contiguous()
        dqkv = torch.empty_like(qkv)
        h2_mark_next(dqkv)
        call("tris_mha_bwd_f32", P(qkv), P(do), P(dqkv), N, L, W, heads, causal, _stream())
        return dqkv, None, None


MHA_STATS = {"last": None}


class MhaMfmaFn(torch.autograd.Function):

    @staticmethod
    def forward(ctx, qkv, heads, causal):
        _chk(qkv)
        qkv = qkv.contiguous()
        N, L, W3 = qkv.shape
        W = W3 // 3
        out = torch.empty(N, L, W, device=qkv.device, dtype=torch.float32)
        lse = torch.empty(N, heads, L, device=qkv.device, dtype=torch.float32)
        w_qkv = _h2_amax(qkv) if (h2_on() and cfg.mha_h2 and L >= 32) else None
        h2_mark_next(out)
        if w_qkv is not None:
            _timed("mha_fwd", 4.0 * N * heads * L * L * 64 * (0.5 if causal else 1.0),
                   lambda: call("tris_mha_h2_fwd_f32", P(qkv), P(out), P(lse), w_qkv, N, L, W, heads, int(causal), _stream()))
        else:
            _timed("mha_fwd", 4.0 * N * heads * L * L * 64 * (0.5 if causal else 1.0),
                   lambda: call("tris_mha_mfma_fwd_f32", P(qkv), P(out), P(lse), N, L, W, heads, int(causal), _stream()))
        MHA_STATS["last"] = "h2" if w_qkv is not None else "f32"
        ctx.h2 = w_qkv is not None
        ctx.cfg = (N, L, W, heads, int(causal))
        ctx.save_for_backward(qkv, out, lse)
        return out

    @staticmethod
    def backward(ctx, do):
        qkv, out, lse = ctx.saved_tensors
        N, L, W, heads, causal = ctx.cfg
        do = do.contiguous()
        dqkv = torch.empty_like(qkv)
        delta = torch.empty_like(lse)
        w_qkv = w_do = None
        if ctx.h2 and h2_on():
            w_qkv, w_do = _h2_amax(qkv), _h2_amax(do)
        h2_mark_next(dqkv)
        if w_qkv is not None and w_do is not None:
            call("tris_mha_h2_bwd_f32", P(qkv), P(out), P(do), P(lse), P(delta), P(dqkv), w_qkv, w_do, N, L, W, heads, causal, _stream())
        else:
            call("tris_mha_mfma_bwd_f32", P(qkv), P(out), P(do), P(lse), P(delta), P(dqkv), N, L, W, heads, causal, _stream())
        return dqkv, None, None


def _mha_impl(L):
    import os
    mode = cfg.mha
    if L > 64 or mode == "mfma":
        return "mfma"
    if mode == "valu":
        return "valu"
    return "valu" if L < 40 else "mfma"


def mha(qkv, heads, causal):
    if _mha_impl(qkv.shape[1]) == "valu":
        return MhaFn.apply(qkv, heads, causal)
    return MhaMfmaFn.apply(qkv, heads, causal)


class QGeluFn(torch.autograd.Function):
    @staticmethod
    def forward(ctx, x):
        x = x.contiguous()
        ctx.save_for_backward(x)
        return ew("TRIS_EW_QGELU", x)

    @staticmethod
    def backward(ctx, dy):
        (x,) = ctx.saved_tensors
        return ew("TRIS_EW_QGELU_BWD", dy.contiguous(), x)


def quick_gelu(x):
    return QGeluFn.apply(x)


class EmbedFn(torch.autograd.Function):

    @staticmethod
    def forward(ctx, ids, tok, pos, reducer=None):
        _chk(ids, tok, pos)
        ids = ids.contiguous()
        N, L = ids.shape
        W = tok.shape[1]
        out = torch.empty(N, L, W, device=tok.device, dtype=torch.float32)
        call("tris_embed_fwd_f32", P(ids), P(tok), P(pos), P(out), N, L, W, _stream())
        ctx.params = (tok, pos)
        ctx.reducer = reducer
        ctx.save_for_backward(ids, tok, pos)
        return out

    @staticmethod
    def backward(ctx, dout):
        ids, tok, pos = ctx.saved_tensors
        N, L = ids.shape
        W = tok.shape[1]
        dout = dout.contiguous()
        st = _sink(ctx.params[0]), _sink(ctx.params[1])
        dtok = st[0] if st[0] is not None else torch.empty_like(tok)
        dpos = st[1] if st[1] is not None else torch.empty_like(pos)
        dtok.zero_()
        dpos.zero_()
        call("tris_embed_bwd_f32", P(ids), P(dout), None, P(dpos), N, L, W, _stream())
        red = ctx.reducer
        if red is not None and st[0] is not None and W % 4 == 0 and W <= 2048 and red.take_embedding_rows(ctx.params[0], ids.view(-1), dout.view(N * L, W), dtok):
            pass
        elif W % 4 == 0 and W <= 2048:
            call("tris_embed_rows_bwd_f32", P(ids), P(dout), P(dtok), N * L, W, 1.0, _stream())
        else:
            call("tris_embed_bwd_f32", P(ids), P(dout), P(dtok), None, N, L, W, _stream())
        return None, (None if st[0] is not None else dtok), (None if st[1] is not None else dpos), None


def embed(ids, tok, pos, reducer=None):
    return EmbedFn.apply(ids, tok, pos, reducer)


class EotGatherFn(torch.autograd.Function):
    @staticmethod
    def forward(ctx, ids, x):
        _chk(ids, x)
        ids, x = (None if ids is None else ids.contiguous()), x.contiguous()
        N, L, W = x.shape
        out = torch.empty(N, W, device=x.device, dtype=torch.float32)
        call("tris_eot_gather_fwd_f32", P(ids), P(x), P(out), N, L, W, _stream())
        ctx.save_for_backward(ids)
        ctx.dims = (N, L, W)
        return out

    @staticmethod
    def backward(ctx, dout):
        (ids,) = ctx.saved_tensors
        N, L, W = ctx.dims
        dx = torch.empty(N, L, W, device=dout.device, dtype=torch.float32)
        call("tris_eot_gather_bwd_f32", P(ids), P(dout.contiguous()), P(dx), N, L, W, _stream())
        return None, dx


def eot_gather(ids, x):
    return EotGatherFn.apply(ids, x)


class rows_limit:

    def __init__(self, plan):
        self.ptr = plan.data_ptr() + 4

    def __enter__(self):
        call("tris_rows_limit_thread", self.ptr)
        _TLS.rows_limit = self.ptr

    def __exit__(self, *exc):
        _TLS.rows_limit = None
        call("tris_rows_limit_thread", None)
        return False


def _rows_limit_blind(A, tA, batch):
    return (getattr(_TLS, "rows_limit", None) is not None and batch == 1 and not tA and h2_on() and pl_word(A) is None
            and _h2_tag_slot(A) is None)


def packed_rows(N, L):
    return (N * L + 255) // 256 * 256


def text_packable(L):
    return not _BATCH_INVARIANT and 1 <= L <= 64


def text_pack_plan(ids):
    N, L = ids.shape
    plan = torch.empty(3 + N + packed_rows(N, L), device=ids.device, dtype=torch.int32)
    call("tris_text_pack_plan_i64", P(ids), N, L, plan.data_ptr(), _stream())
    return plan


def embed_packed(ids, tok, pos, plan):
    N, L = ids.shape
    W = tok.shape[1]
    out = torch.empty(packed_rows(N, L), W, device=tok.device, dtype=torch.float32)
    call("tris_embed_packed_fwd_f32", P(ids), P(tok), P(pos), plan.data_ptr(), P(out), N, L, W, _stream())
    return out


def mha_packed(qkv, plan, N, L, heads, causal):
    W = qkv.shape[-1] // 3
    out = torch.empty(qkv.shape[0], W, device=qkv.device, dtype=torch.float32)
    h2_mark_next(out)
    call("tris_mha_packed_fwd_f32", P(qkv), P(out), plan.data_ptr(), N, L, W, heads, int(causal), _stream())
    return out


def eot_gather_packed(x, plan, N):
    out = torch.empty(N, x.shape[-1], device=x.device, dtype=torch.float32)
    call("tris_eot_gather_packed_f32", P(x), plan.data_ptr(), P(out), N, x.shape[-1], _stream())
    return out


def token0(x):
    return EotGatherFn.apply(None, x)


class L2NormFn(torch.autograd.Function):
    @staticmethod
    def forward(ctx, x):
        _chk(x)
        x = x.contiguous()
        C = x.shape[-1]
        rows = x.numel() // C
# ... 1332 lines not shown
```

Before: 1372 img/s.

## Emit f16 split planes directly from LayerNorm and attention in frozen towers

In frozen transformer blocks, such as the aux CLIP ViT, LayerNorm and the h2 attention forward now write their output already split into packed hi/lo f16 planes. The following GEMMs can then consume it without a separate conversion pass, which removes that pass and the extra memory traffic. The older opt-in gemm_convert path, which converted A on the fly, is removed. The GEMM epilogue also gains an extra-output variant so the pipelined glds path can take pre_out. This adds precision-floor bookkeeping and more complex tagging logic, and it risks errors if a plane tensor reaches a weight-gradient path.

```diff
diff --git a/include/tris_hip.h b/include/tris_hip.h
--- a/include/tris_hip.h
+++ b/include/tris_hip.h
@@ -114,6 +114,8 @@
 
 int tris_layernorm_fwd_f32(const float* X, const float* gamma, const float* beta, float* Y, float* mean, float* rstd,
                            long rows, int W, float eps, void* stream);
+int tris_layernorm_fwd_pl_f32(const float* X, const float* gamma, const float* beta, float* Y, unsigned* word, float* mean,
+                              float* rstd, long rows, int W, float eps, void* stream);
 long tris_layernorm_bwd_workspace_bytes(long rows, int W);
 int tris_layernorm_bwd_f32(const float* dY, const float* X, const float* gamma, const float* mean, const float* rstd,
                            float* dX, float* dgamma, float* dbeta, long rows, int W, float* workspace, const float* extra , void* stream);
@@ -153,6 +155,8 @@
                           float* dqkv, int N, int L, int W, int heads, int causal, void* stream);
 int tris_mha_h2_fwd_f32(const float* qkv, float* out, float* lse, const unsigned* amax_qkv, int N, int L, int W, int heads,
                         int causal, void* stream);
+int tris_mha_h2_fwd_pl_f32(const float* qkv, float* out, float* out_pl, float* lse, const unsigned* amax_qkv, int N, int L, int W,
+                           int heads, int causal, void* stream);
 int tris_mha_h2_bwd_f32(const float* qkv, const float* out, const float* dout, const float* lse, float* delta, float* dqkv,
                         const unsigned* amax_qkv, const unsigned* amax_dout, int N, int L, int W, int heads, int causal,
                         void* stream);
diff --git a/tris_amd/CLIP/clip/model.py b/tris_amd/CLIP/clip/model.py
--- a/tris_amd/CLIP/clip/model.py
+++ b/tris_amd/CLIP/clip/model.py
@@ -210,7 +210,9 @@
         self.weight = nn.Parameter(torch.ones(w))
         self.bias = nn.Parameter(torch.zeros(w))
 
-    def forward(self, x, grad_box=None):
+    def forward(self, x, grad_box=None, planes=False):
+        if planes:
+            return ops.layer_norm(x, self.weight, self.bias, self.eps, grad_box, planes=True)
         return ops.layer_norm(x, self.weight, self.bias, self.eps, grad_box)
 
 
@@ -243,15 +245,20 @@
         self.ln_2 = LayerNorm(d_model)
         self.causal = attn_mask is not None
 
+    def _planes_form(self, x):
+        return (cfg.tower_planes and ops.planes_on() and x.shape[-1] % 32 == 0 and x.numel() // x.shape[-1] >= 4
+                and not any(p.requires_grad for p in self.parameters()))
+
     def forward(self, x):
         use_box = torch.is_grad_enabled() and x.requires_grad and cfg.grad_box
         b1 = ops.GradBox() if use_box else None
         b2 = ops.GradBox() if use_box else None
-        h = self.ln_1(x, b1)
+        pl = self._planes_form(x)
+        h = self.ln_1(x, b1, pl)
         qkv = ops.linear(h, self.attn.in_proj_weight, self.attn.in_proj_bias)
-        a = ops.mha(qkv, self.attn.num_heads, self.causal)
+        a = ops.mha(qkv, self.attn.num_heads, self.causal, planes=True) if pl else ops.mha(qkv, self.attn.num_heads, self.causal)
         x = self.attn.out_proj(a, resid=x, grad_box_res=b1)
-        h = self.ln_2(x, b2)
+        h = self.ln_2(x, b2, pl)
         if torch.is_grad_enabled() and cfg.mlp_fuse:
             f = ops.linear_qgelu(h, self.mlp.c_fc.weight, self.mlp.c_fc.bias)
             return ops.linear(f, self.mlp.c_proj.weight, self.mlp.c_proj.bias, x, 0, grad_box_res=b2, act_link=True)
@@ -270,7 +277,7 @@
         return self.mlp.c_proj(self.mlp.c_fc(h, act=2), resid=x)
 
     def forward_token0(self, x):
-        h = self.ln_1(x)
+        h = self.ln_1(x, planes=self._planes_form(x))
         qkv = ops.linear(h, self.attn.in_proj_weight, self.attn.in_proj_bias)
         a = ops.token0(ops.mha(qkv, self.attn.num_heads, self.causal))
         x0 = self.attn.out_proj(a, resid=ops.token0(x))
@@ -312,9 +319,6 @@
         self.positional_embedding = nn.Parameter(scale * torch.randn((input_resolution // patch_size) ** 2 + 1, width))
         self.ln_pre = LayerNorm(width)
         self.transformer = Transformer(width, layers, heads)
-        for blk in self.transformer.resblocks:
-            for w in (blk.attn.in_proj_weight, blk.attn.out_proj.weight, blk.mlp.c_fc.weight, blk.mlp.c_proj.weight):
-                w._tris_linear_w = True
         self.ln_post = LayerNorm(width)
         self.proj = nn.Parameter(scale * torch.randn(width, output_dim))
         self.spacial_dim = 7
diff --git a/tris_amd/config.py b/tris_amd/config.py
--- a/tris_amd/config.py
+++ b/tris_amd/config.py
@@ -49,7 +49,7 @@
         self.aux_text_early = _flag("TRIS_AUX_TEXT_EARLY", True)
         self.text_pack = _flag("TRIS_TEXT_PACK", True)
         self.bn_bitmask = _flag("TRIS_BN_BITMASK", True)
-        self.gemm_convert = int(e("TRIS_GEMM_CONVERT", "0"))
+        self.tower_planes = _flag("TRIS_TOWER_PLANES", True)
         self.step_graph_rerecord = int(e("TRIS_STEP_GRAPH_RERECORD", "3"))
         self.side_param_grads = _flag("TRIS_SIDE_PARAM_GRADS", True)
         self.vit_token0 = _flag("TRIS_VIT_TOKEN0", True)
diff --git a/tris_amd/csrc/attn_h2.hip b/tris_amd/csrc/attn_h2.hip
--- a/tris_amd/csrc/attn_h2.hip
+++ b/tris_amd/csrc/attn_h2.hip
@@ -5,6 +5,7 @@
 namespace {
 
 #include "amax.h"
+#include "planes.h"
 
 constexpr int HD = 64;
 constexpr int RS = 144;
@@ -76,7 +77,7 @@
 
 __global__ __launch_bounds__(256) void mha_h2_fwd_kernel(const float* __restrict__ qkv, float* __restrict__ out, float* __restrict__ lse,
                                                          int L, int W, int causal, float scale, const unsigned* __restrict__ am_qkv,
-                                                         unsigned* __restrict__ amax) {
+                                                         unsigned* __restrict__ amax, float* __restrict__ out_pl = nullptr) {
   __shared__ __attribute__((aligned(16))) char Kp[2 * PLB];
   __shared__ __attribute__((aligned(16))) char Vp[2 * PLB];
   const int tid = threadIdx.x, lane = tid & 63, wave = tid >> 6, r = lane & 15, kg = lane >> 4;
@@ -146,26 +147,40 @@
       }
     }
   }
-  unsigned am = 0u;
+  unsigned am = 0u, below = 0u;
   if (q0 < L) {
     const float linv = 1.f / l;
     float* ob = out + (long)n * L * W + h * HD;
+    unsigned* pb = out_pl != nullptr ? reinterpret_cast<unsigned*>(out_pl + (long)n * L * W + h * HD) : nullptr;
 #pragma unroll
     for (int t = 0; t < 4; ++t) {
       const float li = __shfl(linv, 4 * kg + t, 64) * inv_o;
       const int q = q0 + 4 * kg + t;
-      if (q < L) {
-#pragma unroll
-        for (int j = 0; j < 4; ++j) {
-          const float o = (oc[j][t] + ox[j][t] * (1.0f / 2048.0f)) * li;
+#pragma unroll
+      for (int j = 0; j < 4; ++j) {
+        const float o = (oc[j][t] + ox[j][t] * (1.0f / 2048.0f)) * li;
+        if (q < L) {
           ob[(long)q * W + 16 * j + r] = o;
           am = max(am, __builtin_bit_cast(unsigned, o) & 0x7fffffffu);
         }
+        if (pb != nullptr) {
+          const float xs = o * s;
+          const _Float16 hi = (_Float16)xs;
+          const _Float16 lo = (_Float16)((xs - (float)hi) * 2048.f);
+          const unsigned own = (unsigned)__builtin_bit_cast(unsigned short, hi) | ((unsigned)__builtin_bit_cast(unsigned short, lo) << 16);
+          const unsigned nb = (unsigned)__shfl_xor((int)own, 1, 64);
+          const unsigned word = (r & 1) ? ((nb >> 16) | (own & 0xffff0000u)) : ((own & 0xffffu) | (nb << 16));
+          if (q < L) {
+            below += (o != 0.f && fabsf(o) * s < 6.103515625e-05f) ? 1u : 0u;
+            pb[(long)q * W + 16 * j + (r & 8) + ((r & 1) ? 4 : 0) + ((r & 6) >> 1)] = word;
+          }
+        }
       }
     }
     if (kg == 0 && q0 + r < L) lse[((long)n * H + h) * L + q0 + r] = m + __logf(l);
   }
   if (amax != nullptr) amax_commit(am, amax);
+  if (out_pl != nullptr) pl_floor_commit(below, am_qkv);
 }
 
 __global__ __launch_bounds__(256) void mha_h2_dq_kernel(const float* __restrict__ qkv, const float* __restrict__ out,
@@ -374,6 +389,16 @@
   return 0;
 }
 
+extern "C" int tris_mha_h2_fwd_pl_f32(const float* qkv, float* out, float* out_pl, float* lse, const unsigned* amax_qkv, int N, int L,
+                                      int W, int heads, int causal, void* stream) {
+  if (W != heads * HD || L < 1 || N < 1 || (((uintptr_t)qkv) & 15) || (((uintptr_t)out_pl) & 15) || amax_qkv == nullptr || out_pl == nullptr)
+    return (int)hipErrorInvalidValue;
+  hipLaunchKernelGGL(mha_h2_fwd_kernel, dim3(cdiv(L, 64), heads, N), dim3(256), 0, (hipStream_t)stream, qkv, out, lse, L, W, causal,
+                     1.0f / sqrtf((float)HD), amax_qkv, tris_internal_take_amax_next(), out_pl);
+  TRIS_LAUNCH_CHECK();
+  return 0;
+}
+
 extern "C" int tris_mha_h2_bwd_f32(const float* qkv, const float* out, const float* dout, const float* lse, float* delta, float* dqkv,
                                    const unsigned* amax_qkv, const unsigned* amax_dout, int N, int L, int W, int heads, int causal,
                                    void* stream) {
diff --git a/tris_amd/csrc/gemm_core.h b/tris_amd/csrc/gemm_core.h
--- a/tris_amd/csrc/gemm_core.h
+++ b/tris_amd/csrc/gemm_core.h
@@ -443,7 +443,7 @@
   const bool xtra = p.pre_out != nullptr || p.dact_x != nullptr;
   if (mode == 4 && !fast) return (int)hipErrorInvalidValue;
   const bool pipe = cfg.pipe == 1 && (mode == 1 || mode == 3 || mode == 4) && fast && bn != 32 && !xtra;
-  const bool glds = cfg.pipe >= 2 && mode == 4 && fast && !xtra && bn != 32 && AK == A_ROWK && BKIND == B_NK;
+  const bool glds = cfg.pipe >= 2 && mode == 4 && fast && p.dact_x == nullptr && bn != 32 && AK == A_ROWK && BKIND == B_NK;
   const int gform = glds ? (cfg.pipe >= 4 ? cfg.pipe - 2 : cfg.pipe) : 0;
   if (bm == 256 && !pipe && !glds) bm = 128;
   int tiles_m = cdiv(p.M, bm), tiles_n = cdiv(p.N, bn);
@@ -533,6 +533,8 @@
     if (splitk > 1) {                                                                                                            \
       p.C = ws;                                                                                                                  \
       hipLaunchKernelGGL((gemm_fast_kernel<BM_, BN_, AK, BKIND, EPI_SLAB, 4, NW_, 32, 4, NWM_>), grid, dim3(NW_ * 64), 0, st, p); \
+    } else if (xtra) {                                                                                                           \
+      hipLaunchKernelGGL((gemm_fast_kernel<BM_, BN_, AK, BKIND, EPI_XTRA, 4, NW_, 32, 4, NWM_>), grid, dim3(NW_ * 64), 0, st, p); \
     } else {                                                                                                                     \
       hipLaunchKernelGGL((gemm_fast_kernel<BM_, BN_, AK, BKIND, EPI_STD, 4, NW_, 32, 4, NWM_>), grid, dim3(NW_ * 64), 0, st, p);  \
     }                                                                                                                            \
diff --git a/tris_amd/csrc/norm.hip b/tris_amd/csrc/norm.hip
--- a/tris_amd/csrc/norm.hip
+++ b/tris_amd/csrc/norm.hip
@@ -11,8 +11,13 @@
 namespace {
 
 #include "amax.h"
+#include "x3_split.h"
+#include "planes.h"
 
 __device__ __forceinline__ float4 ld4(const float* p) { return *reinterpret_cast<const float4*>(p); }
+__device__ __forceinline__ unsigned ln_dpp_nb(const unsigned v) {
+  return (unsigned)__builtin_amdgcn_update_dpp(0, (int)v, 0xB1, 0xF, 0xF, true);
+}
 __device__ __forceinline__ void st4(float* p, float4 v) { *reinterpret_cast<float4*>(p) = v; }
 typedef float f32x4_t __attribute__((ext_vector_type(4)));
 __device__ __forceinline__ float4 ld4nt(const float* p) {
@@ -514,16 +519,19 @@
   if (amax != nullptr) amax_commit(am, amax);
 }
 
+template <bool PL>
 __global__ __launch_bounds__(256) void layernorm_fwd_kernel(const float* __restrict__ X, const float* __restrict__ gamma,
                                                             const float* __restrict__ beta, float* __restrict__ Y,
                                                             float* __restrict__ mean_out, float* __restrict__ rstd_out,
                                                             long rows, int W, float eps, unsigned* __restrict__ amax = nullptr,
-                                                            const int* __restrict__ limit = nullptr) {
+                                                            const int* __restrict__ limit = nullptr, float xhat_max = 0.f) {
   const int lane = threadIdx.x & 63;
   const long row = (long)blockIdx.x * 4 + (threadIdx.x >> 6);
   if (row >= rows) return;
   if (limit != nullptr && row >= (long)*limit) return;
   unsigned am = 0u;
+  float pl_s = 1.f;
+  unsigned below = 0u;
   const int W4 = W >> 2;
   float4 v[4];
   float s = 0.f;
@@ -544,6 +552,23 @@
     }
   }
   float rstd = rsqrtf(wave_sum(s2) / (float)W + eps);
+  if constexpr (PL) {
+    float bd = 0.f;
+#pragma unroll
+    for (int q = 0; q < 4; ++q) {
+      const int i = lane + q * 64;
+      if (i < W4) {
+        const float4 g = ld4(gamma + i * 4), b = ld4(beta + i * 4);
+        bd = fmaxf(fmaxf(bd, fmaf(fabsf(g.x), xhat_max, fabsf(b.x))), fmaf(fabsf(g.y), xhat_max, fabsf(b.y)));
+        bd = fmaxf(fmaxf(bd, fmaf(fabsf(g.z), xhat_max, fabsf(b.z))), fmaf(fabsf(g.w), xhat_max, fabsf(b.w)));
+      }
+    }
+    unsigned bits = __builtin_bit_cast(unsigned, bd);
+#pragma unroll
+    for (int sft = 32; sft > 0; sft >>= 1) bits = max(bits, (unsigned)__shfl_xor((int)bits, sft, 64));
+    pl_s = h2_scale_from_bits(bits);
+    if (row == 0 && lane == 0 && bits != 0u) amax_raise(bits, amax);
+  }
 #pragma unroll
   for (int q = 0; q < 4; ++q) {
     int i = lane + q * 64;
@@ -553,11 +578,22 @@
       o.y = (v[q].y - mean) * rstd * g.y + b.y;
       o.z = (v[q].z - mean) * rstd * g.z + b.z;
       o.w = (v[q].w - mean) * rstd * g.w + b.w;
-      st4(Y + row * W + i * 4, o);
-      am = max(am, abits4(o));
-    }
-  }
-  if (amax != nullptr) amax_commit(am, amax);
+      if constexpr (PL) {
+        below += pl_below_floor(o, make_float4(0.f, 0.f, 0.f, 0.f), pl_s);
+        const Split4 sp = split4h(o, pl_s);
+        const bool odd = lane & 1;
+        const uint2 send = odd ? sp.hi : sp.mid;
+        const uint2 recv = make_uint2(ln_dpp_nb(send.x), ln_dpp_nb(send.y));
+        const uint4 w = odd ? make_uint4(recv.x, recv.y, sp.mid.x, sp.mid.y) : make_uint4(sp.hi.x, sp.hi.y, recv.x, recv.y);
+        *reinterpret_cast<uint4*>(Y + row * W + i * 4) = w;
+      } else {
+        st4(Y + row * W + i * 4, o);
+        am = max(am, abits4(o));
+      }
+    }
+  }
+  if constexpr (PL) pl_floor_commit(below, amax);
+  else if (amax != nullptr) amax_commit(am, amax);
   if (lane == 0 && mean_out) { mean_out[row] = mean; rstd_out[row] = rstd; }
 }
 
@@ -1051,8 +1087,19 @@
 extern "C" int tris_layernorm_fwd_f32(const float* X, const float* gamma, const float* beta, float* Y, float* mean,
                                       float* rstd, long rows, int W, float eps, void* stream) {
   if (W % 4 || W > 1024) return (int)hipErrorInvalidValue;
-  hipLaunchKernelGGL(layernorm_fwd_kernel, dim3(cdiv(rows, 4)), dim3(256), 0, (hipStream_t)stream, X, gamma, beta, Y,
-                     mean, rstd, rows, W, eps, take_amax_next(), g_rows_limit);
+  hipLaunchKernelGGL(layernorm_fwd_kernel<false>, dim3(cdiv(rows, 4)), dim3(256), 0, (hipStream_t)stream, X, gamma, beta, Y,
+                     mean, rstd, rows, W, eps, take_amax_next(), g_rows_limit, 0.f);
+  TRIS_LAUNCH_CHECK();
+  return 0;
+}
+
+static float ln_xhat_max(int W) { return sqrtf((float)W) * (1.0f + 1.0f / 65536.0f); }
+extern "C" int tris_layernorm_fwd_pl_f32(const float* X, const float* gamma, const float* beta, float* Y, unsigned* word, float* mean,
+                                         float* rstd, long rows, int W, float eps, void* stream) {
+  if (W % 8 || W > 1024 || W < 8 || word == nullptr || (((uintptr_t)X | (uintptr_t)Y | (uintptr_t)gamma | (uintptr_t)beta) & 15)) return TRIS_DECLINED;
+  if (rows <= 0) return 0;
+  hipLaunchKernelGGL(layernorm_fwd_kernel<true>, dim3(cdiv(rows, 4)), dim3(256), 0, (hipStream_t)stream, X, gamma, beta, Y,
+                     mean, rstd, rows, W, eps, word, g_rows_limit, ln_xhat_max(W));
   TRIS_LAUNCH_CHECK();
   return 0;
 }
diff --git a/tris_amd/ops.py b/tris_amd/ops.py
--- a/tris_amd/ops.py
+++ b/tris_amd/ops.py
@@ -398,16 +398,16 @@
 def gemm(A, B, C, M, N, K, lda, ldb, ldc, tA, tB, batch=1, sA=0, sB=0, sC=0, bias=None, bias_mode=0, resid=None,
          ldr=0, sR=0, act=0, alpha=1.0, use_ws=True, pre_out=None, dact=None, w_a=False, w_b=False, w_bt=False, mark=True):
     _chk(A, B, C, bias, resid)
-    if pre_out is not None or dact is not None or batch != 1 or _BATCH_INVARIANT:
+    if dact is not None or batch != 1 or _BATCH_INVARIANT:
         A, B = unplanes(A), unplanes(B)
     if pre_out is not None or dact is not None:
         if _BATCH_INVARIANT or batch != 1:
             return False
-        h2_arm(A, B)
+        pA, pB = h2_pp(A, B, w_b=w_b, k_red=K)
         h2_mark_next(C)
         call("tris_gemm_epilogue_next", P(pre_out), P(dact))
         return _timed("gemm", 2.0 * M * N * K, lambda: _declinable(
-            "tris_gemm_f32", P(A), P(B), P(C), M, N, K, lda, ldb, ldc, int(tA), int(tB), 1, 0, 0, 0, P(bias), bias_mode, P(resid),
+            "tris_gemm_f32", pA, pB, P(C), M, N, K, lda, ldb, ldc, int(tA), int(tB), 1, 0, 0, 0, P(bias), bias_mode, P(resid),
             ldr, sR, act, float(alpha), None, 0, _stream()),
             nbytes=4.0 * (M * K + K * N + M * N * (2 + int(resid is not None))))
     if _BATCH_INVARIANT and batch == 1 and not tA and M < 4 and lda == K and ldc == N and (resid is None or ldr == N) and bias_mode != 2:
@@ -424,9 +424,6 @@
         return C
     ws = workspace(0) if (use_ws and batch == 1 and not _BATCH_INVARIANT) else None
     blind = _rows_limit_blind(A, tA, batch)
-    if (w_b and batch == 1 and not tA and M >= cfg.gemm_convert and cfg.gemm_convert > 0 and K % 32 == 0 and lda == K and getattr(B, "_tris_linear_w", False)
-            and planes_on() and pl_word(A) is None and A.is_contiguous() and A.data_ptr() % 16 == 0 and _pl_weight_ok(B) and not blind):
-        A = _a_planes(A, M, K)
     if blind:
         PL_STATS["last"] = PL_STATS["last_t"] = False
         pA, pB = P(A), P(unplanes(B))
@@ -577,25 +574,13 @@
 
 
 def _pl_weight_t_ok(p):
-    if p.dim() == 2:
-        return cfg.gemm_convert > 0 and getattr(p, "_tris_linear_w", False) and p.shape[0] % 64 == 0 and p.shape[1] % 64 == 0
     return p.dim() == 4 and p.shape[2] * p.shape[3] == 1 and p.shape[0] % 64 == 0 and p.shape[1] % 64 == 0
 
 
 def _pl_weight_ok(p):
     if p.dim() == 2:
-        return cfg.gemm_convert > 0 and getattr(p, "_tris_linear_w", False) and p.shape[1] % 8 == 0 and p.is_contiguous()
+        return cfg.tower_planes and not p.requires_grad and p.shape[1] % 8 == 0 and p.is_contiguous()
     return p.dim() == 4 and p.shape[1] % 8 == 0 and (p.is_contiguous(memory_format=torch.channels_last) or p.shape[2] * p.shape[3] == 1)
-
-
-def _a_planes(A, M, K):
-    slot = _h2_amax(A)
-    if slot is None:
-        return A
-    t = torch.empty_like(A)
-    call("tris_h2_planes_f32", P(A), P(t), A.numel(), slot, _stream())
-    PL_STATS["converted"] = PL_STATS.get("converted", 0) + 1
-    return pl_tag(t, slot)
 
 
 def _h2_new_step_id():
@@ -821,7 +806,7 @@
     return True
 
 
-PL_STATS = {"unplanes": 0, "dx_planes": 0, "dy_planes": 0, "products": 0, "mixed": 0, "last": False, "last_t": False}
+PL_STATS = {"unplanes": 0, "dx_planes": 0, "dy_planes": 0, "products": 0, "mixed": 0, "tower_planes": 0, "last": False, "last_t": False}
 
 
 _HAS_GPU = None
@@ -1064,7 +1049,7 @@
         _retag(x, ctx.x_pl)
         if pl_word(dy) is not None and (ctx.has_r or ctx.has_b or ctx.act == 1):
             dy = unplanes(dy)
-        if pl_word(dy) is None:
+        if pl_word(dy) is None and ctx.needs_input_grad[1]:
             x = unplanes(x)
         d_res = dy if ctx.has_r and ctx.needs_input_grad[3] else None
         if d_res is not None and ctx.grad_box_res is not None and ctx.grad_box_res.deposit(d_res):
@@ -1155,8 +1140,10 @@
         M = x.numel() // K
         y = torch.empty(*x.shape[:-1], N, device=x.device, dtype=torch.float32)
         pre = torch.empty_like(y)
-        if gemm(x, w, y, M, N, K, K, K, N, False, True, bias=b, bias_mode=1 if b is not None else 0, act=2, pre_out=pre) is False:
-            gemm(x, w, pre, M, N, K, K, K, N, False, True, bias=b, bias_mode=1 if b is not None else 0)
+        if pl_word(x) is not None and w.requires_grad:
+            raise RuntimeError("linear_qgelu: a plane input next to a weight that needs a gradient (the weight gradient would read x)")
+        if gemm(x, w, y, M, N, K, K, K, N, False, True, bias=b, bias_mode=1 if b is not None else 0, act=2, pre_out=pre, w_b=True) is False:
+            gemm(x, w, pre, M, N, K, K, K, N, False, True, bias=b, bias_mode=1 if b is not None else 0, w_b=True)
             ew("TRIS_EW_QGELU", pre, out=y)
         ctx.dims, ctx.has_b, ctx.params = (M, N, K), b is not None, (w, b)
         ctx.link = y._act_link = _ActLink(pre)
@@ -1722,7 +1709,7 @@
 
 class LayerNormFn(torch.autograd.Function):
     @staticmethod
-    def forward(ctx, x, g, b, eps, grad_box=None):
+    def forward(ctx, x, g, b, eps, grad_box=None, planes=False):
         _chk(x, g, b)
         ctx.grad_box = grad_box
         x = x.contiguous()
@@ -1730,8 +1717,14 @@
         rows = x.numel() // W
         y = torch.empty_like(x)
         st = torch.empty(2, rows, device=x.device, dtype=torch.float32)
-        h2_mark_next(y)
-        call("tris_layernorm_fwd_f32", P(x), P(g), P(b), P(y), P(st), P(st, rows), rows, W, eps, _stream())
+        word = _h2_slot() if (planes and planes_on() and W % 8 == 0 and W <= 1024) else None
+        if word is not None and _declinable("tris_layernorm_fwd_pl_f32", P(x), P(g), P(b), P(y), word, P(st), P(st, rows), rows, W,
+                                            eps, _stream()):
+            pl_tag(y, word)
+            PL_STATS["tower_planes"] += 1
+        else:
+            h2_mark_next(y)
+            call("tris_layernorm_fwd_f32", P(x), P(g), P(b), P(y), P(st), P(st, rows), rows, W, eps, _stream())
         ctx.dims = (rows, W)
         ctx.params = (g, b)
         ctx.save_for_backward(x, g, b, st)
@@ -1757,18 +1750,18 @@
             h2_mark_next(dx)
             call("tris_layernorm_bwd_f32", P(dy), P(x), P(g), P(st), P(st, rows), P(dx), P(sg), P(sb), rows, W, P(ws),
                  P(extra), _stream())
-            return dx, None, None, None, None
+            return dx, None, None, None, None, None
         dgb = torch.empty(2, W, device=x.device, dtype=torch.float32) if need_p else None
         h2_mark_next(dx)
         call("tris_layernorm_bwd_f32", P(dy), P(x), P(g), P(st), P(st, rows), P(dx), P(dgb), P(dgb, W),
              rows, W, P(ws), P(extra), _stream())
         dg = _emit(ctx.params[0], lambda o: o.copy_(dgb[0]), ctx.needs_input_grad[1])
         db = _emit(ctx.params[1], lambda o: o.copy_(dgb[1]), ctx.needs_input_grad[2])
-        return dx, dg, db, None, None
-
-
-def layer_norm(x, g, b, eps=1e-5, grad_box=None):
-    return LayerNormFn.apply(x, g, b, eps, grad_box)
+        return dx, dg, db, None, None, None
+
+
+def layer_norm(x, g, b, eps=1e-5, grad_box=None, planes=False):
+    return LayerNormFn.apply(x, g, b, eps, grad_box, planes)
 
 
 class MhaFn(torch.autograd.Function):
@@ -1803,7 +1796,7 @@
 class MhaMfmaFn(torch.autograd.Function):
 
     @staticmethod
-    def forward(ctx, qkv, heads, causal):
+    def forward(ctx, qkv, heads, causal, planes=False):
         _chk(qkv)
         qkv = qkv.contiguous()
         N, L, W3 = qkv.shape
@@ -1811,6 +1804,16 @@
         out = torch.empty(N, L, W, device=qkv.device, dtype=torch.float32)
         lse = torch.empty(N, heads, L, device=qkv.device, dtype=torch.float32)
         w_qkv = _h2_amax(qkv) if (h2_on() and cfg.mha_h2 and L >= 32) else None
+        if planes and w_qkv is not None and planes_on():
+            out_pl = torch.empty_like(out)
+            _timed("mha_fwd", 4.0 * N * heads * L * L * 64 * (0.5 if causal else 1.0),
+                   lambda: call("tris_mha_h2_fwd_pl_f32", P(qkv), P(out), P(out_pl), P(lse), w_qkv, N, L, W, heads, int(causal), _stream()))
+            MHA_STATS["last"] = "h2"
+            ctx.h2 = True
+            ctx.cfg = (N, L, W, heads, int(causal))
+            ctx.save_for_backward(qkv, out, lse)
+            PL_STATS["tower_planes"] += 1
+            return pl_tag(out_pl, w_qkv)
         h2_mark_next(out)
         if w_qkv is not None:
             _timed("mha_fwd", 4.0 * N * heads * L * L * 64 * (0.5 if causal else 1.0),
@@ -1839,7 +1842,7 @@
             call("tris_mha_h2_bwd_f32", P(qkv), P(out), P(do), P(lse), P(delta), P(dqkv), w_qkv, w_do, N, L, W, heads, causal, _stream())
         else:
             call("tris_mha_mfma_bwd_f32", P(qkv), P(out), P(do), P(lse), P(delta), P(dqkv), N, L, W, heads, causal, _stream())
-        return dqkv, None, None
+        return dqkv, None, None, None
 
 
 def _mha_impl(L):
@@ -1852,10 +1855,10 @@
     return "valu" if L < 40 else "mfma"
 
 
-def mha(qkv, heads, causal):
+def mha(qkv, heads, causal, planes=False):
     if _mha_impl(qkv.shape[1]) == "valu":
         return MhaFn.apply(qkv, heads, causal)
-    return MhaMfmaFn.apply(qkv, heads, causal)
+    return MhaMfmaFn.apply(qkv, heads, causal, planes)
 
 
 class QGeluFn(torch.autograd.Function):
```

New measurement: 1388 img/s, median of 6. No clear change (+1.1%).
